# knights-lab/BURST

Measured on AMD Instinct MI355X. Metric: aligned reads/sec (node), 100-bp synthetic reads @0.98 id vs RefSeq stand-in .edx/.acx (DB15), -m BEST; 1 GPU, higher is better.
Workload: dtype u32 bit-vectors (u8 edit distances)

## Files before the change

burst_amd/csrc/bhip_align.hip:

```cpp
#include "bhip_handle.h"
#include "bhip_pf_select.h"

__global__ void k_hit_count(const BhipHit *__restrict__ hits, uint32_t n, const uint32_t *__restrict__ n_dev, uint32_t *__restrict__ cnt, uint32_t *__restrict__ rank) {
	if (n_dev) n = *n_dev < n ? *n_dev : n;
	for (uint32_t i = blockIdx.x * blockDim.x + threadIdx.x; i < n; i += gridDim.x * blockDim.x) rank[i] = atomicAdd(&cnt[hits[i].q], 1u);
}
__global__ void k_hit_scatter(const BhipHit *__restrict__ in, uint32_t n, const uint32_t *__restrict__ n_dev, const uint32_t *__restrict__ off, const uint32_t *__restrict__ rank,
                              BhipHit *__restrict__ out, const uint32_t *__restrict__ qmap) {
	if (n_dev) n = *n_dev < n ? *n_dev : n;
	for (uint32_t i = blockIdx.x * blockDim.x + threadIdx.x; i < n; i += gridDim.x * blockDim.x) {
		BhipHit h = in[i];
		const uint32_t dst = off[h.q] + rank[i];
		if (qmap) h.q = qmap[h.q];
		out[dst] = h;
	}
}
__global__ void k_junk_adjust_raw(BhipRawHit *__restrict__ raw, const uint32_t *__restrict__ n_raw_dev, uint32_t raw_cap, const uint8_t *__restrict__ nx) {
	uint32_t n = *n_raw_dev;
	if (n > raw_cap) n = raw_cap;
	for (uint32_t i = blockIdx.x * blockDim.x + threadIdx.x; i < n; i += gridDim.x * blockDim.x) { const uint32_t x = nx[raw[i].q]; raw[i].ed += x; raw[i].m += x; }
}
__global__ void k_junk_adjust_best(uint32_t *__restrict__ best, const uint8_t *__restrict__ nx_six, uint32_t s0, uint32_t s1) {
	for (uint32_t s = s0 + blockIdx.x * blockDim.x + threadIdx.x; s < s1; s += gridDim.x * blockDim.x)
		if (nx_six[s] && best[s] != 0xFFFFFFFFu) best[s] += nx_six[s];
}

__global__ __launch_bounds__(256) void k_hit_fix(BhipHit *__restrict__ out, const uint32_t *__restrict__ off, const uint32_t *__restrict__ cnt, uint32_t n_q,
                                               BhipHit *__restrict__ scratch, uint32_t scratch_cap) {
	const uint32_t lane = threadIdx.x & 63u;
	const uint32_t wave = (blockIdx.x * blockDim.x + threadIdx.x) >> 6, n_waves = (gridDim.x * blockDim.x) >> 6;
	struct Rec { uint32_t w[5]; };
	static_assert(sizeof(BhipHit) == 20, "BhipHit is five dwords");
	for (uint32_t q0 = wave * 64u; q0 < n_q; q0 += n_waves * 64u) {
		const uint32_t q = q0 + lane;
		const uint32_t n_mine = q < n_q ? cnt[q] : 0u, o_mine = q < n_q ? off[q] : 0u;
		unsigned long long todo = __ballot(n_mine >= 2u);
		while (todo) {
			const int b = __builtin_ctzll(todo);
			todo &= todo - 1ull;
			const uint32_t n = (uint32_t)__builtin_amdgcn_readlane((int)n_mine, b), o = (uint32_t)__builtin_amdgcn_readlane((int)o_mine, b);
			Rec *grp = (Rec *)(out + o);
			if (n <= 64u) {
				Rec r = {};
				if (lane < n) r = grp[lane];
				const uint32_t key = lane < n ? r.w[1] : 0xFFFFFFFFu;
				uint32_t rank = 0;
				for (uint32_t j = 0; j < n; ++j) { const uint32_t kj = (uint32_t)__builtin_amdgcn_readlane((int)key, (int)j); rank += (kj < key || (kj == key && j < lane)) ? 1u : 0u; }
				if (lane < n) grp[rank] = r;
			} else if ((uint64_t)o + n <= scratch_cap) {
				Rec *tmp = (Rec *)(scratch + o);
				for (uint32_t i = lane; i < n; i += 64u) tmp[i] = grp[i];
				__threadfence();
				for (uint32_t i0 = 0; i0 < n; i0 += 64u) {
					const uint32_t i = i0 + lane;
					Rec r = {};
					if (i < n) r = tmp[i];
					const uint32_t key = i < n ? r.w[1] : 0xFFFFFFFFu;
					uint32_t rank = 0;
					for (uint32_t j0 = 0; j0 < n; j0 += 64u) {
						const uint32_t kj = j0 + lane < n ? tmp[j0 + lane].w[1] : 0xFFFFFFFFu;
						const uint32_t m = n - j0 < 64u ? n - j0 : 64u;
						for (uint32_t j = 0; j < m; ++j) { const uint32_t kk = (uint32_t)__builtin_amdgcn_readlane((int)kj, (int)j); rank += (kk < key || (kk == key && j0 + j < i)) ? 1u : 0u; }
					}
					if (i < n) grp[rank] = r;
				}
			} else if (lane == 0) {
				BhipHit *a = out + o;
				uint32_t gap = 1;
				while (gap < n / 3) gap = 3 * gap + 1;
				for (; gap >= 1; gap /= 3)
					for (uint32_t i = gap; i < n; ++i) {
						const BhipHit v = a[i];
						uint32_t j = i;
						for (; j >= gap && a[j - gap].refIx > v.refIx; j -= gap) a[j] = a[j - gap];
						a[j] = v;
					}
			}
		}
	}
}
__global__ void k_set_rank_ptrs(SharedCtr *sc, uint32_t *cnt, uint32_t *rank) { sc->cnt = cnt; sc->rank = rank; }

__device__ __forceinline__ unsigned long long best_key_of(const BhipHit &h, const uint32_t *__restrict__ order) {
	return (unsigned long long)(~__float_as_uint(h.score)) << 32 | order[h.refIx];
}
__global__ void k_best_key(const BhipHit *__restrict__ hits, uint32_t n, const uint32_t *__restrict__ n_dev, const uint32_t *__restrict__ order, const uint32_t *__restrict__ cnt,
                           unsigned long long *__restrict__ key) {
	if (n_dev) n = *n_dev < n ? *n_dev : n;
	for (uint32_t i = blockIdx.x * blockDim.x + threadIdx.x; i < n; i += gridDim.x * blockDim.x) {
		const BhipHit h = hits[i];
		if (cnt[h.q] > 1u) atomicMin(&key[h.q], best_key_of(h, order));
	}
}
__global__ void k_best_flag(const uint32_t *__restrict__ cnt, uint32_t n_q, uint32_t *__restrict__ flag) {
	for (uint32_t i = blockIdx.x * blockDim.x + threadIdx.x; i <= n_q; i += gridDim.x * blockDim.x) flag[i] = i < n_q && cnt[i] ? 1u : 0u;
}
__global__ void k_best_emit(const BhipHit *__restrict__ hits, uint32_t n, const uint32_t *__restrict__ n_dev, const uint32_t *__restrict__ order, const uint32_t *__restrict__ cnt,
                            const unsigned long long *__restrict__ key, const uint32_t *__restrict__ off, BhipHit *__restrict__ out, const uint32_t *__restrict__ qmap) {
	if (n_dev) n = *n_dev < n ? *n_dev : n;
	for (uint32_t i = blockIdx.x * blockDim.x + threadIdx.x; i < n; i += gridDim.x * blockDim.x) {
		BhipHit h = hits[i];
		if (cnt[h.q] > 1u && best_key_of(h, order) != key[h.q]) continue;
		const uint32_t dst = off[h.q];
		if (qmap) h.q = qmap[h.q];
		out[dst] = h;
	}
}
extern "C" int bhip_set_ref_order(void *handle, const uint32_t *order, uint32_t n) {
	Handle *h = (Handle *)handle;
	if (!h) return fail(BHIP_E_ARG, "null handle");
	if (!order) return h->n_order ? 1 : 0;
	if (n < h->tot_refs) return fail(BHIP_E_ARG, "reference order table holds %u entries, the database has %u references", n, h->tot_refs);
	HIPCHK(hipSetDevice(h->device));
	int rc;
	h->n_order = 0;
	if ((rc = h->ref_order.reserve((size_t)h->tot_refs * 4 + 16))) return rc;
	HIPCHK(hipMemcpy(h->ref_order.p, order, (size_t)h->tot_refs * 4, hipMemcpyHostToDevice));
	h->n_order = h->tot_refs;
	return BHIP_OK;
}

static void launch_myers(Handle *h, Lane *L, hipStream_t st, int NW, uint32_t grid, const uint2 *pairs, const uint32_t *n_pairs_dev,
		uint64_t n_pairs_host, uint32_t li_base, const uint32_t *qlist, BhipRawHit *raw, uint32_t *n_raw, uint32_t raw_cap, uint32_t *best,
		uint8_t *mins, Counters *dc) {
	if (NW > 32) {
		hipLaunchKernelGGL(k_myers_long, dim3(grid * 4u), dim3(64), (size_t)NW * 512u, st, pairs, n_pairs_dev, n_pairs_host, h->n_clumps, li_base, qlist,
			L->peq.as<uint32_t>(), h->s_off(), h->s_emac(), (best && h->cur->st_has_six) ? h->cur->qsix.as<uint32_t>() : nullptr,
			h->ref_lane.as<uint4>(), h->ref_off.as<uint64_t>(), h->clump_len.as<uint32_t>(), h->tot_refs, raw, n_raw, raw_cap, best, mins, &dc->col_sum, &dc->qlen_sum, (uint32_t)NW);
		return;
	}
	#define LM(N) hipLaunchKernelGGL(k_myers<N>, dim3(grid), dim3(256), 0, st, pairs, n_pairs_dev, n_pairs_host, h->n_clumps, li_base, qlist, \
		L->peq.as<uint32_t>(), h->s_off(), h->s_emac(), (best && h->cur->st_has_six) ? h->cur->qsix.as<uint32_t>() : nullptr, \
		h->ref_lane.as<uint4>(), h->ref_off.as<uint64_t>(), h->clump_len.as<uint32_t>(), h->tot_refs, raw, n_raw, raw_cap, best, mins, &dc->col_sum, &dc->qlen_sum)
	switch (NW) { case 2: LM(2); break; case 4: LM(4); break; case 6: LM(6); break; case 8: LM(8); break; case 10: LM(10); break;
		case 16: LM(16); break; default: LM(32); break; }
	#undef LM
}
static void launch_prefix(Handle *h, Lane *L, hipStream_t st, int NWP, uint32_t grid, const uint2 *pairs, const uint32_t *n_pairs_dev,
		uint64_t n_pairs_host, uint32_t li_base, const uint32_t *qlist, uint32_t *n_wins, Counters *dc) {
	#define LP(N) hipLaunchKernelGGL(k_myers_prefix<N>, dim3(grid), dim3(256), 0, st, pairs, n_pairs_dev, n_pairs_host, h->n_clumps, li_base, qlist, \
		L->peqp.as<uint32_t>(), h->s_off(), h->s_emac(), h->ref_lane.as<uint4>(), h->ref_off.as<uint64_t>(), h->clump_len.as<uint32_t>(), \
		h->tot_refs, L->wins.as<BhipWin>(), n_wins, (uint32_t)L->win_cap, &dc->col_sum, &dc->qlen_sum, dc->win_class_seen, h->cur->st_has_six ? h->cur->qsix.as<uint32_t>() : nullptr)
	if (NWP == 1) LP(1); else if (NWP == 2) LP(2); else if (NWP == 3) LP(3); else if (NWP == 4) LP(4); else LP(6);
	#undef LP
}
static void launch_prefix_task(Handle *h, Lane *L, hipStream_t st, int NWP, uint32_t grid, const uint2 *tasks, const uint32_t *n_tasks_dev, const uint32_t *qlist,
		BhipWin *wins, uint32_t *n_wins, Counters *dc, const uint4 *qmeta) {
	#define LT(N) hipLaunchKernelGGL(k_myers_prefix_task<N>, dim3(grid), dim3(64), 0, st, tasks, n_tasks_dev, (uint32_t)L->task_cap, qlist, \
		L->peqp.as<uint32_t>(), h->s_off(), h->s_emac(), h->ref_lane.as<uint4>(), h->ref_off.as<uint64_t>(), h->clump_len.as<uint32_t>(), \
		wins, n_wins, (uint32_t)L->win_cap, &dc->tcol_sum, dc->win_class_seen, qmeta, h->cur->st_has_six ? h->cur->qsix.as<uint32_t>() : nullptr)
	if (NWP == 1) LT(1); else if (NWP == 2) LT(2); else if (NWP == 3) LT(3); else if (NWP == 4) LT(4); else LT(6);
	#undef LT
}
static uint32_t blocks_per_cu(const void *fn, uint32_t threads, size_t dyn_lds, hipFuncAttributes *fa_out = nullptr) {
	hipFuncAttributes fa_here, &fa = fa_out ? *fa_out : fa_here;
	memset(&fa, 0, sizeof fa);
	if (hipFuncGetAttributes(&fa, fn) != hipSuccess) return 4;
	const uint32_t waves_per_block = (threads + 63) / 64;
	const uint32_t by_reg = 4u * std::min(8u, 512u / (uint32_t)std::max(8, (fa.numRegs + 7) & ~7)) / waves_per_block;
	const size_t lds = fa.sharedSizeBytes + dyn_lds;
	const uint32_t by_lds = lds ? (uint32_t)((148u * 1024u) / std::max<size_t>(512, (lds + 511) & ~(size_t)511)) : 64u;
	return std::max(1u, std::min(by_reg, by_lds));
}

static void launch_window(Handle *h, Lane *L, hipStream_t wst, int cls, int NWP, uint32_t grid_cap, const BhipWin *wins, const uint32_t *n_wins, Counters *dc) {
	const uint32_t *six = h->cur->st_has_six ? h->cur->qsix.as<uint32_t>() : nullptr;
	const int NWc = kClasses[cls];
	const int min_class = h->opt_no_band ? 0 : NWc >= 8 ? 3 : NWc >= 6 ? 2 : NWc >= 4 ? 1 : 0;
	#define LB(BW) { uint32_t per_cu = blocks_per_cu((const void *)k_myers_window_band<BW>, 64u, 0); \
		if (h->opt_band_blocks > 0) per_cu = (uint32_t)h->opt_band_blocks; \
		const uint32_t grid = (uint32_t)h->n_cu * per_cu * (uint32_t)h->opt_oversub; \
		hipLaunchKernelGGL(k_myers_window_band<BW>, dim3(grid), dim3(64), 0, wst, wins, n_wins, (uint32_t)L->win_cap, NWP, NWc, L->peq.as<uint32_t>(), six, \
			h->ref_lane.as<uint4>(), L->raw.as<BhipRawHit>(), &dc->n_raw, (uint32_t)L->raw_cap, h->best.as<uint32_t>(), &dc->wcol_sum, dc->win_class_seen); }
	if (min_class >= 1) LB(2);
	if (min_class >= 2) LB(3);
	if (min_class >= 3) LB(4);
	#undef LB
	#define LW(N) { const uint32_t thr = (N) <= 8 ? 64u : 256u;       \
		const uint32_t grid = std::min<uint32_t>(grid_cap * (256u / thr), (uint32_t)h->n_cu * blocks_per_cu((const void *)k_myers_window<N>, thr, 0)); \
		hipLaunchKernelGGL(k_myers_window<N>, dim3(grid), dim3(thr), 0, wst, wins, n_wins, (uint32_t)L->win_cap, NWP, min_class, \
		L->peq.as<uint32_t>(), six, h->ref_lane.as<uint4>(), \
		L->raw.as<BhipRawHit>(), &dc->n_raw, (uint32_t)L->raw_cap, h->best.as<uint32_t>(), &dc->wcol_sum, dc->win_class_seen); }
	switch (NWc) { case 2: LW(2); break; case 4: LW(4); break; case 6: LW(6); break; case 8: LW(8); break; case 10: LW(10); break;
		case 16: LW(16); break; default: LW(32); break; }
	#undef LW
}


static int upload_queries(Handle *h, const uint8_t *q_codes, const uint64_t *q_off, const uint16_t *q_emac,
                          const uint32_t *q_six, const uint8_t *q_rc, uint32_t n_q) {
	const uint64_t nb = q_off[n_q];
	int rc;
	h->cur->st_has_junk = false;
	h->cur->st_maxlen = 0; h->cur->st_maxE = 0;
	for (uint32_t i = 0; i < n_q; ++i) {
		h->cur->st_maxlen = std::max<uint32_t>(h->cur->st_maxlen, (uint32_t)(q_off[i + 1] - q_off[i]));
		h->cur->st_maxE = std::max<uint32_t>(h->cur->st_maxE, q_emac[i]);
	}
	if ((rc = h->cur->qcodes.reserve(nb + 16))) return rc;
	if ((rc = h->cur->qoff.reserve((n_q + 1) * sizeof(uint64_t)))) return rc;
	if ((rc = h->cur->qemac.reserve((n_q + 1) * sizeof(uint16_t)))) return rc;
	if ((rc = h->cur->qsix.reserve((n_q + 1) * sizeof(uint32_t)))) return rc;
	if ((rc = h->cur->qrc.reserve(n_q + 1))) return rc;
	HIPCHK(hipMemcpyAsync(h->cur->qcodes.p, q_codes, nb, hipMemcpyHostToDevice, h->stream));
	HIPCHK(hipMemcpyAsync(h->cur->qoff.p, q_off, (n_q + 1) * sizeof(uint64_t), hipMemcpyHostToDevice, h->stream));
	HIPCHK(hipMemcpyAsync(h->cur->qemac.p, q_emac, n_q * sizeof(uint16_t), hipMemcpyHostToDevice, h->stream));
	if (q_six) HIPCHK(hipMemcpyAsync(h->cur->qsix.p, q_six, n_q * sizeof(uint32_t), hipMemcpyHostToDevice, h->stream));
	if (q_rc) HIPCHK(hipMemcpyAsync(h->cur->qrc.p, q_rc, n_q, hipMemcpyHostToDevice, h->stream));
	return 0;
}

static int upload_plan(Handle *h, const uint8_t *q_codes, const uint64_t *q_off, const uint16_t *q_emac, uint32_t n_q, std::vector<uint32_t> &plan) {
	int rc;
	if ((rc = h->cur->plan.reserve((size_t)n_q * 4 + 16))) return rc;
	(void)q_codes; (void)q_off; (void)q_emac;
	HIPCHK(hipMemcpyAsync(h->cur->plan.p, plan.data(), (size_t)n_q * 4, hipMemcpyHostToDevice, h->stream));
	HIPCHK(hipStreamSynchronize(h->stream));
	return 0;
}

struct PfOverflow {
	uint32_t *fb1 = nullptr, *n_fb1 = nullptr;
	uint32_t *fb2 = nullptr, *n_fb2 = nullptr;
	int begin(Lane *L, Counters *dc, hipStream_t st, uint32_t n_list, bool lane_resolved) {
		int rc;
		if ((rc = L->fb_list.reserve(lane_resolved ? (size_t)n_list * 8 + 64 : (size_t)n_list * 4 + 16))) return rc;
		fb1 = L->fb_list.as<uint32_t>(); n_fb1 = &dc->n_fb;
		if (lane_resolved) {
			fb2 = fb1 + n_list + 8; n_fb2 = &dc->n_fb2;
			if (L->pf_launches || L->fb_dirty) HIPCHK(hipMemsetAsync(&dc->n_fb, 0, 8, st));
			L->fb_dirty = false;
		} else {
			HIPCHK(hipMemsetAsync(&dc->n_fb, 0, 4, st));
			L->fb_dirty = true;
		}
		return 0;
	}
};

static int launch_dense_fallback(Handle *h, Lane *L, hipStream_t st, const uint32_t *d_qlist, uint32_t n_list, const uint32_t *bad, uint32_t n_bad,
                                 uint2 *cand, uint32_t *candcnt, uint32_t *n_cand_dev, uint32_t cand_cap, Counters *dc, const uint32_t *fb, const uint32_t *n_fb) {
	const uint32_t *plan = h->cur->plan.as<uint32_t>();
	const bool narrow = h->cur->st_maxlen < 255u + (uint32_t)h->K;
	const size_t lds_w = ((size_t)(h->n_clumps + (narrow ? 3 : 1)) / (narrow ? 4 : 2)) * 4 + 1536u * 4 + 512u * 8 + 512u * 4 + 16;
	const uint32_t nw32 = (h->n_clumps + 1) / 2;
	if (lds_w <= 64 * 1024) {
		const uint32_t per_cu = (uint32_t)std::max<size_t>(1, std::min<size_t>(16, (160 * 1024) / lds_w));
		const uint32_t grid = std::min<uint32_t>(n_list, (uint32_t)h->n_cu * per_cu);
		if (narrow) hipLaunchKernelGGL(k_prefilter_wave<uint8_t>, dim3(grid), dim3(64), lds_w, st, h->s_codes(), h->s_off(),
			h->s_emac(), d_qlist, n_list, h->acx_view(), h->K, h->n_clumps, bad, n_bad, cand, candcnt,
			n_cand_dev, cand_cap, &dc->ent_read, plan, fb, n_fb);
		else hipLaunchKernelGGL(k_prefilter_wave<uint16_t>, dim3(grid), dim3(64), lds_w, st, h->s_codes(), h->s_off(),
			h->s_emac(), d_qlist, n_list, h->acx_view(), h->K, h->n_clumps, bad, n_bad, cand, candcnt,
			n_cand_dev, cand_cap, &dc->ent_read, plan, fb, n_fb);
	} else {
		int rc;
		const uint32_t grid = std::min<uint32_t>(n_list, (uint32_t)h->n_cu * 2);
		if ((rc = L->gcnt.reserve((size_t)grid * nw32 * 4))) return rc;
		hipLaunchKernelGGL(k_prefilter<false>, dim3(grid), dim3(256), 0, st, h->s_codes(), h->s_off(),
			h->s_emac(), d_qlist, n_list, h->acx_view(), h->K, h->n_clumps,
			L->gcnt.as<uint32_t>(), bad, n_bad, cand, candcnt, n_cand_dev, cand_cap, &dc->ent_read, fb, n_fb, plan);
	}
	HIPCHK(hipGetLastError());
	return 0;
}

static int launch_prefilter(Handle *h, Lane *L, hipStream_t st, const uint32_t *d_qlist, uint32_t n_list, uint2 *cand, uint32_t *candcnt, uint32_t cand_cap,
                            bool with_bad, uint32_t *n_cand_dev, Counters *dc) {
	const uint32_t *bad = with_bad ? h->bad.as<uint32_t>() : nullptr;
	const uint32_t n_bad = with_bad ? h->n_bad : 0;
	int rc;
	PfOverflow ov;
	if ((rc = ov.begin(L, dc, st, n_list, false))) return rc;
	{
		const uint32_t n_quads = (n_list + 3) / 4;
		const uint32_t grid = std::min<uint32_t>(n_quads, (uint32_t)h->n_cu * 6);
		hipLaunchKernelGGL(k_prefilter_hash, dim3(grid), dim3(64), 0, st, h->s_codes(), h->s_off(), h->s_emac(),
			d_qlist, n_list, h->acx_view(), h->K, bad, n_bad, cand, candcnt, n_cand_dev, cand_cap, &dc->ent_read,
			h->cur->plan.as<uint32_t>(), ov.fb1, ov.n_fb1);
		HIPCHK(hipGetLastError());
	}
	return launch_dense_fallback(h, L, st, d_qlist, n_list, bad, n_bad, cand, candcnt, n_cand_dev, cand_cap, dc, ov.fb1, ov.n_fb1);
}

static uint32_t seed_row_words(uint32_t maxwords) { return maxwords <= 8 ? 8u : std::max<uint32_t>(16u, (maxwords + 15u) & ~15u); }
static int class_prefix_words(const Handle *h, uint32_t maxE, int NW) {
	if (!h->opt_two_stage || NW > 32) return 0;
	const uint32_t want = (6 * maxE + 31) / 32;
	int NWP = want <= 1 ? 1 : (want <= 2 ? 2 : (want <= 3 ? 3 : (want <= 4 ? 4 : (want <= 6 ? 6 : 0))));
	if (NWP >= NW) NWP = 0;
	return NWP;
}
static int launch_peq(Handle *h, hipStream_t st, StageSlot *S, const uint32_t *d_qlist, uint32_t n_list, int NW, int NWP, DBuf &peq, DBuf &peqp, uint32_t blocks_per_cu = 16) {
	int rc;
	if ((rc = peq.reserve((size_t)n_list * 16 * NW * 4))) return rc;
	if ((rc = peqp.reserve((size_t)n_list * 16 * 6 * 4))) return rc;
	const bool junk = S->st_has_junk;
	const uint8_t *codes = junk ? S->qcodes_s.as<uint8_t>() : S->qcodes.as<uint8_t>();
	const uint64_t *off = junk ? S->qoff_s.as<uint64_t>() : S->qoff.as<uint64_t>();
	const uint32_t *pack = junk ? S->qpack_s.as<uint32_t>() : S->qpack.as<uint32_t>();
	{
		const uint32_t qb = 256u / (uint32_t)NW;
		const uint32_t grid = (uint32_t)std::min<uint64_t>(((uint64_t)n_list + qb - 1) / qb, (uint64_t)h->n_cu * blocks_per_cu);
		hipLaunchKernelGGL(k_build_peq, dim3(grid), dim3(256), 0, st, codes, off, d_qlist, n_list, NW, 0, h->mm, peq.as<uint32_t>(), pack, (S->st_maxlen + 7) / 8, h->peq_rows);
		HIPCHK(hipGetLastError());
	}
	if (NWP) {
		const uint32_t qb = 256u / (uint32_t)NWP;
		const uint32_t grid = (uint32_t)std::min<uint64_t>(((uint64_t)n_list + qb - 1) / qb, (uint64_t)h->n_cu * blocks_per_cu);
		hipLaunchKernelGGL(k_build_peq, dim3(grid), dim3(256), 0, st, codes, off, d_qlist, n_list, NWP, 32 * NWP, h->mm, peqp.as<uint32_t>(), pack, (S->st_maxlen + 7) / 8, h->peq_rows);
		HIPCHK(hipGetLastError());
	}
	return 0;
}
static uint32_t seed_min_need_for(const Handle *h, double mean_words, uint32_t W16) {
	return bhip_seed_min_need(h->opt_seed_min_need, h->opt_pf_cw, h->opt_pf_table, h->opt_pf_bytes, h->acx_wmean, mean_words, W16);
}
static int launch_seed(Handle *h, Lane *L, hipStream_t st, StageSlot *S, int cls, const uint32_t *d_qlist, uint32_t n_list, uint32_t maxwords, double mean_words, bool ahead = false) {
	int rc;
	const uint32_t W16 = seed_row_words(maxwords);
	L->seeded_ok[cls] = false;
	if ((rc = L->ranges_c[cls].reserve((size_t)n_list * W16 * 8 + 16))) return rc;
	if ((rc = L->hdr_c[cls].reserve((size_t)n_list * 8 + 16))) return rc;
	DBuf &qm = L->qmeta_c[S->seq & 1][cls];
	if ((rc = qm.reserve((size_t)n_list * 16 + 16))) return rc;
	L->qmeta_seq[S->seq & 1][cls] = 0;
	const uint64_t n_thr = (uint64_t)n_list * W16;
	hipEvent_t *ev = L->ev_seed[S->seq & 1][cls];
	const bool junk = S->st_has_junk;
	HIPCHK(hipEventRecord(ev[0], st));
	const uint64_t full = (n_thr + 255) / 256;
	const uint32_t grid = (uint32_t)(ahead && h->opt_seed_ahead_blocks > 0 ? std::min<uint64_t>(full, (uint64_t)h->n_cu * (uint64_t)h->opt_seed_ahead_blocks) : full);
	hipLaunchKernelGGL(k_seed_ranges, dim3(grid), dim3(256), 0, st,
		junk ? S->qcodes_s.as<uint8_t>() : S->qcodes.as<uint8_t>(), junk ? S->qoff_s.as<uint64_t>() : S->qoff.as<uint64_t>(), d_qlist, n_list,
		h->acx_view(), h->K, S->plan.as<uint32_t>(), W16, L->ranges_c[cls].as<uint2>(), L->hdr_c[cls].as<uint2>(),
		junk ? S->qpack_s.as<uint32_t>() : S->qpack.as<uint32_t>(), (S->st_maxlen + 7) / 8, junk ? S->qemac_s.as<uint16_t>() : S->qemac.as<uint16_t>(), qm.as<uint4>(), S->st_has_six ? S->qsix.as<uint32_t>() : nullptr,
		seed_min_need_for(h, mean_words, W16), (uint32_t)h->opt_seed_drop_len, h->alt);
	HIPCHK(hipGetLastError());
	HIPCHK(hipEventRecord(ev[1], st));
	L->qmeta_seq[S->seq & 1][cls] = S->seq + 1;
	L->seeded_ok[cls] = true; L->seeded_seq[cls] = S->seq; L->seeded_n[cls] = n_list; L->seeded_W16[cls] = W16;
	return 0;
}

static bhip_pf_kernel_t pf_kernel(const BhipPfChoice &c, int big) {
	if (c.legacy) return bhip_legacy_pf_kernel ? bhip_legacy_pf_kernel(c.kind, big ? 11 : c.htb, big ? 4 : c.rb, c.cw_mode, big) : nullptr;
	if (c.kind == BHIP_PF_CQ) return c.cw_mode == 0 ? (big ? k_prefilter_cq<0, 1> : k_prefilter_cq<0, 0>) : (big ? k_prefilter_cq<1, 1> : k_prefilter_cq<1, 0>);
	return big ? k_prefilter_cw<2, 1> : k_prefilter_cw<2, 0>;
}

static int launch_prefilter_mask(Handle *h, Lane *L, hipStream_t st, int cls, const uint32_t *d_qlist, uint32_t n_list, uint32_t maxwords, uint32_t *n_tasks_dev,
                                 uint32_t *n_cand_dev, Counters *dc, int algo, int prune) {
	int rc;
	PfOverflow ov;
	if ((rc = ov.begin(L, dc, st, n_list, true))) return rc;
	const uint32_t W16 = seed_row_words(maxwords);
	const double mean_words = n_list ? (double)L->seed_words[cls] / (double)n_list : (double)maxwords;
	if (!(L->seeded_ok[cls] && L->seeded_seq[cls] == h->cur->seq && L->seeded_n[cls] == n_list && L->seeded_W16[cls] == W16))
		if ((rc = launch_seed(h, L, st, h->cur, cls, d_qlist, n_list, maxwords, mean_words))) return rc;
	const BhipPfChoice c = bhip_pf_choose(algo, h->opt_pf_cw, h->opt_pf_table, h->opt_pf_rb, W16, mean_words * h->acx_wmean);
	const bool filter = c.kind != BHIP_PF_MASK, cw = c.kind == BHIP_PF_CW || c.kind == BHIP_PF_CQ;
	const bhip_pf_kernel_t fp = filter ? pf_kernel(c, 0) : nullptr, fp2 = filter && c.two_pass ? pf_kernel(c, 1) : nullptr;
	if (filter && (!fp || (c.two_pass && !fp2)))
		return fail(BHIP_E_ARG, "option prefilter_cw = %d selects a superseded prefilter kernel that is not part of libburst_hip.so (tests: libburst_hip_legacy.so is loaded first)", h->opt_pf_cw);
	hipFuncAttributes fa;
	const void *fn = filter ? (const void *)fp : c.htb == 9 ? (const void *)k_prefilter_mask<9> : c.htb == 10 ? (const void *)k_prefilter_mask<10> : (const void *)k_prefilter_mask<11>;
	const uint32_t fit = std::min<uint32_t>(cw ? 32u : 12u, blocks_per_cu(fn, 64u, 0, &fa));
	if (getenv("BHIP_DEBUG")) {
		if (cw) fprintf(stderr, "[bhip] prefilter kernel: %s, slot mode %d, %zu B LDS, %d VGPRs -> %u blocks per CU\n", c.kind == BHIP_PF_CQ ? "four queries per wave, streams by the whole wave" : "one query per wave", c.cw_mode, fa.sharedSizeBytes, fa.numRegs, fit);
		else fprintf(stderr, "[bhip] prefilter kernel: table 2^%d, %d record blocks in registers, %zu B LDS, %d VGPRs -> %u blocks per CU\n", c.htb, c.rb, fa.sharedSizeBytes, fa.numRegs, fit);
	}
	const uint32_t waves = h->opt_pf_waves ? std::min<uint32_t>((uint32_t)h->opt_pf_waves, fit) : fit;
	const uint32_t grid = std::min<uint32_t>(c.kind == BHIP_PF_CW ? n_list : (n_list + 3) / 4, (uint32_t)h->n_cu * waves);
	HIPCHK(hipEventRecord(L->ev_pf[cls][1], st));
	const uint32_t *fb_dense = ov.fb1, *n_fb_dense = ov.n_fb1;
	if (filter) {
		auto launch = [&](bhip_pf_kernel_t k, uint32_t g, uint32_t *fb, uint32_t *n_fb, const uint32_t *sel, const uint32_t *n_sel) {
			hipLaunchKernelGGL(k, dim3(g), dim3(64), 0, st, L->ranges_c[cls].as<uint2>(), L->hdr_c[cls].as<uint2>(), W16, n_list,
				h->acx_view().rec, h->bad.as<uint32_t>(), h->n_bad,
				h->clump_len.as<uint32_t>(), h->tot_refs, L->tasks.as<uint2>(), n_tasks_dev, (uint32_t)L->task_cap, &dc->ent_read,
				fb, n_fb, &dc->unit_sum, &dc->col_sum, &dc->qlen_sum, &dc->surv_sum,
				L->tasks2.as<uint2>(), &dc->n_tasks2_cls[cls], prune, sel, n_sel, c.kind == BHIP_PF_CF ? h->opt_pf_bytes : 0);
		};
		launch(fp, grid, ov.fb1, ov.n_fb1, nullptr, nullptr);
		if (c.two_pass) {
			HIPCHK(hipGetLastError());
			const uint32_t g2 = (uint32_t)h->n_cu * (c.kind == BHIP_PF_CQ ? std::min<uint32_t>(4u, blocks_per_cu((const void *)fp2, 64u, 0)) : 1u);
			launch(fp2, g2, ov.fb2, ov.n_fb2, ov.fb1, ov.n_fb1);
			fb_dense = ov.fb2; n_fb_dense = ov.n_fb2;
		}
	} else {
#define PFM_LAUNCH(B) hipLaunchKernelGGL(k_prefilter_mask<B>, dim3(grid), dim3(64), 0, st, L->ranges_c[cls].as<uint2>(), L->hdr_c[cls].as<uint2>(), W16, n_list, \
		h->acx_view().rec, h->bad.as<uint32_t>(), h->n_bad, \
		h->clump_len.as<uint32_t>(), h->tot_refs, L->tasks.as<uint2>(), n_tasks_dev, (uint32_t)L->task_cap, &dc->ent_read, \
		ov.fb1, ov.n_fb1, &dc->unit_sum, &dc->col_sum, &dc->qlen_sum, L->cand.as<uint2>(), n_cand_dev, (uint32_t)L->cand_cap)
		if (c.htb == 9) PFM_LAUNCH(9); else if (c.htb == 10) PFM_LAUNCH(10); else PFM_LAUNCH(11);
#undef PFM_LAUNCH
	}
	HIPCHK(hipGetLastError());
	HIPCHK(hipEventRecord(L->ev_pf[cls][2], st));
	++L->pf_launches;
	L->pf_algo_used = c.kind;
	return launch_dense_fallback(h, L, st, d_qlist, n_list, h->bad.as<uint32_t>(), h->n_bad, L->cand.as<uint2>(), nullptr, n_cand_dev, (uint32_t)L->cand_cap, dc, fb_dense, n_fb_dense);
}

static int lane_reserve_work(Lane *L) {
	int rc;
	if ((rc = L->cand.reserve(L->cand_cap * sizeof(uint2))) || (rc = L->raw.reserve(L->raw_cap * sizeof(BhipRawHit))) || (rc = L->wide.reserve(L->raw_cap * sizeof(uint32_t))) ||
	    (rc = L->rs_lists.reserve(L->raw_cap * sizeof(uint32_t) * 10)) || (rc = L->scratch.reserve(L->scratch_cap * sizeof(uint32_t))) || (rc = L->wins.reserve(L->win_cap * sizeof(BhipWin))) ||
	    (rc = L->tasks.reserve(L->task_cap * sizeof(uint2))) || (rc = L->tasks2.reserve(L->task_cap * sizeof(uint2))) || (rc = L->tasks2k.reserve(L->task_cap * sizeof(uint2))) ||
	    (rc = L->wins2.reserve(L->win_cap * sizeof(BhipWin)))) return rc;
	return 0;
}
extern "C" int bhip_reserve(void *handle, uint32_t n_entries, uint32_t max_len) { return bhip_reserve_symbols(handle, n_entries, max_len, 0); }
extern "C" int bhip_reserve_symbols(void *handle, uint32_t n_entries, uint32_t max_len, uint64_t total_symbols) {
	Handle *h = (Handle *)handle;
	if (!h) return fail(BHIP_E_ARG, "null handle");
	if (!n_entries) return BHIP_OK;
	if (!max_len || max_len > BHIP_MAX_QLEN) max_len = BHIP_MAX_QLEN;
	HIPCHK(hipSetDevice(h->device));
	int rc;
	if (getenv("BHIP_DEBUG")) { size_t f_ = 0, t_ = 0; if (hipMemGetInfo(&f_, &t_) == hipSuccess) fprintf(stderr, "[bhip] reserve for %u entries of up to %u symbols: %.2f GB of the device's %.2f free\n", n_entries, max_len, f_ / 1e9, t_ / 1e9); }
	const size_t n = n_entries, nb = total_symbols ? (size_t)std::min<uint64_t>(total_symbols + 64, (uint64_t)n * max_len) : n * max_len, qw = (max_len + 7) / 8;
	const size_t cw = (size_t)class_words(class_of_len(max_len), max_len);
	const size_t peq_words = total_symbols ? std::min<size_t>(n * cw, 2 * (nb / 32 + n)) : n * cw;
	for (StageSlot &S : h->slots) {
		if ((rc = slot_init(&S))) return rc;
		if ((rc = S.qcodes4.reserve(nb / 2 + 128)) || (rc = S.qcodes.reserve(nb + 128)) || (rc = S.qoff.reserve((n + 1) * 8)) || (rc = S.qemac.reserve((n + 1) * 2)) ||
		    (rc = S.qsix.reserve((n + 1) * 4)) || (rc = S.qrc.reserve(n + 1)) || (rc = S.qflags.reserve(n + 1)) || (rc = S.qmap.reserve((n + 1) * 4)) ||
		    (rc = S.off_raw.reserve((n + 8) * 8)) || (rc = S.plan.reserve(n * 4 + 16)) || (rc = S.qpack.reserve(n * qw * 4 + 64)) || (rc = S.key.reserve(n + 16)) ||
		    (rc = S.key_sorted.reserve(n + 16)) || (rc = S.idx.reserve(n * 4 + 16)) || (rc = S.idx_sorted.reserve(n * 4 + 16))) return rc;
		size_t tb = 0;
		HIPCHK(hipcub::DeviceRadixSort::SortPairs(nullptr, tb, S.key.as<uint8_t>(), S.key_sorted.as<uint8_t>(), S.idx.as<uint32_t>(), S.idx_sorted.as<uint32_t>(), (int)n, 0, 8, h->stage_stream));
		if ((rc = S.sort_tmp.reserve(tb + 16))) return rc;
	}
	if (getenv("BHIP_DEBUG")) { size_t f_ = 0, t_ = 0; if (hipMemGetInfo(&f_, &t_) == hipSuccess) fprintf(stderr, "[bhip] ... staging slots reserved: %.2f GB free\n", f_ / 1e9); }
	if ((rc = ensure_lanes(h, 1))) return rc;
	Lane *L = h->lanes[0];
	lane_capacity_floor(h, L, n);
	const int cls = class_of_len(max_len);
	if ((rc = lane_reserve_work(L)) || (rc = L->peq.reserve(peq_words * 16 * 4)) || (rc = L->peqp.reserve(n * 16 * 6 * 4)) ||
	    (rc = L->peq_alt.reserve(peq_words * 16 * 4)) || (rc = L->peqp_alt.reserve(n * 16 * 6 * 4)) ||
	    (rc = L->fb_list.reserve(n * 8 + 64)) || (rc = L->ranges_c[cls].reserve(n * 16 * 8 + 16)) || (rc = L->hdr_c[cls].reserve(n * 8 + 16))) return rc;
	if (h->n_order) { if ((rc = h->best_key.reserve((n + 1) * 8)) || (rc = h->sort_idx.reserve(std::max<size_t>((size_t)h->out_cap, n + 1) * 4))) return rc; if (!h->nsel_pinned) HIPCHK(hipHostMalloc((void **)&h->nsel_pinned, 64, hipHostMallocDefault)); }
	if ((rc = h->best.reserve((n + 1) * 4)) || (rc = h->out.reserve(h->out_cap * sizeof(BhipHit))) || (rc = h->shared_ctr.reserve(sizeof(SharedCtr))) ||
	    (rc = h->sort_idx.reserve(h->out_cap * 4)) || (rc = h->sort_keys.reserve((n + 1) * 4)) || (rc = h->sort_keys2.reserve((n + 1) * 4)) ||
	    (rc = h->out_sorted.reserve(h->out_cap * sizeof(BhipHit))) || (rc = h->out_sorted2.reserve(h->out_cap * sizeof(BhipHit)))) return rc;
	{
		size_t tb = 0;
		HIPCHK(hipcub::DeviceScan::ExclusiveSum(nullptr, tb, h->sort_keys.as<uint32_t>(), h->sort_keys2.as<uint32_t>(), (int)(n + 1), h->stream));
		if ((rc = h->sort_tmp.reserve(tb))) return rc;
	}
	if (getenv("BHIP_DEBUG")) { size_t f_ = 0, t_ = 0; if (hipMemGetInfo(&f_, &t_) == hipSuccess) fprintf(stderr, "[bhip] ... lane and record buffers reserved: %.2f GB free\n", f_ / 1e9); }
	if (!h->copy_stream) { HIPCHK(hipStreamCreateWithFlags(&h->copy_stream, hipStreamNonBlocking)); HIPCHK(hipEventCreateWithFlags(&h->ev_sorted, hipEventDisableTiming));
		for (auto &e : h->ev_copied) HIPCHK(hipEventCreateWithFlags(&e, hipEventDisableTiming)); }
	{
		const uint32_t nw = std::min<uint32_t>(n_entries, 1u << 17), len = std::min<uint32_t>(max_len, 100u);
		const size_t nb_w = (size_t)nw * len + 16;
		uint8_t *pin = nullptr;
		const size_t bytes = nb_w + nb_w / 2 + 16 + ((size_t)nw + 1) * 8 + (size_t)nw * 2 + 64 + (size_t)nw * 4 * sizeof(BhipHit);
		HIPCHK(hipHostMalloc((void **)&pin, bytes, hipHostMallocPortable));
		uint8_t *codes = pin, *codes4 = pin + nb_w;
		uint64_t *off = (uint64_t *)(pin + ((nb_w + nb_w / 2 + 16 + 7) & ~(size_t)7));
		uint16_t *emac = (uint16_t *)(off + nw + 1);
		BhipHit *hbuf = (BhipHit *)(((uintptr_t)(emac + nw) + 63) & ~(uintptr_t)63);
		uint64_t x = 88172645463325252ull;
		for (size_t i = 0; i < nb_w; ++i) { x ^= x << 13; x ^= x >> 7; x ^= x << 17; codes[i] = (uint8_t)(1 + (x & 3)); }
		for (size_t i = 0; i < nb_w / 2; ++i) codes4[i] = (uint8_t)(codes[2 * i] | codes[2 * i + 1] << 4);
		for (uint32_t i = 0; i <= nw; ++i) off[i] = (uint64_t)i * len;
		for (uint32_t i = 0; i < nw; ++i) emac[i] = (uint16_t)(len / 40);
		BhipQuerySpan sp;
		memset(&sp, 0, sizeof sp);
		sp.codes = codes; sp.codes4 = codes4; sp.off = off; sp.emac = emac; sp.n = nw;
		uint64_t n_out = 0;
		const int async = h->opt_async_d2h;
		h->opt_async_d2h = 1;
		for (StageSlot &S : h->slots) { S.state = 0; S.st_valid = false; }
		rc = 0;
		for (int rep = 0; rep < 4 && !rc; ++rep) {
			rc = bhip_stage_spans(h, &sp, 1, nw, len);
			if (!rc) rc = bhip_align_staged(h, 0, hbuf, (uint64_t)nw * 4, &n_out);
		}
		(void)bhip_sync_hits(h);
		{
			const size_t big = std::min<size_t>(64u << 20, std::min(h->out_sorted.cap, h->out_sorted2.cap));
			void *tmp = nullptr;
			if (big && hipHostMalloc(&tmp, 2 * big, hipHostMallocPortable) == hipSuccess) {
				(void)hipMemcpyAsync(tmp, h->out_sorted.p, big, hipMemcpyDeviceToHost, h->copy_stream);
				(void)hipMemcpyAsync((char *)tmp + big, h->out_sorted2.p, big, hipMemcpyDeviceToHost, h->copy_stream);
				(void)hipMemcpyAsync(tmp, h->out_sorted.p, big, hipMemcpyDeviceToHost, h->copy_stream);
				(void)hipStreamSynchronize(h->copy_stream);
				(void)hipMemcpyAsync(h->out_sorted.p, tmp, big, hipMemcpyHostToDevice, h->stage_stream);
				(void)hipMemcpyAsync(h->out_sorted2.p, (char *)tmp + big, big, hipMemcpyHostToDevice, h->stage_stream);
				(void)hipMemcpyAsync(h->out_sorted.p, tmp, big, hipMemcpyHostToDevice, h->stage_stream);
				(void)hipStreamSynchronize(h->stage_stream);
				const size_t piece = big / 16;
				if (piece) {
					for (int i = 0; i < 12; ++i) (void)hipMemcpyAsync((char *)h->out_sorted.p + (size_t)i * piece, (char *)tmp + (size_t)i * piece, piece, hipMemcpyHostToDevice, h->stage_stream);
					(void)hipMemcpyAsync((char *)tmp + big, h->out_sorted2.p, big, hipMemcpyDeviceToHost, h->copy_stream);
					(void)hipStreamSynchronize(h->copy_stream);
					(void)hipStreamSynchronize(h->stage_stream);
				}
				(void)hipHostFree(tmp);
			}
			(void)hipGetLastError();
		}
		h->opt_async_d2h = async;
		for (StageSlot &S : h->slots) { S.state = 0; S.st_valid = false; S.spans.clear(); }
		h->res_valid = false;
		(void)hipHostFree(pin);
		if (rc) return rc;
	}
	return BHIP_OK;
}
static int enqueue_lane(Handle *h, Lane *L, int all_hits, hipEvent_t start, uint32_t band_rows, uint32_t qw, uint32_t rw) {
	int rc;
	if ((rc = lane_reserve_work(L))) return rc;
	hipStream_t pf = h->pf_stream, sw = h->sweep_stream, po = h->post_stream;
	HIPCHK(hipMemsetAsync(L->counters.p, 0, sizeof(Counters), pf));
	Counters *dc = L->counters.as<Counters>();
	SharedCtr *sc = h->shared_ctr.as<SharedCtr>();
	L->launches = 0; L->prefix_words = 0; L->n_pairs_ex = 0; L->pf_launches = 0; L->fb_dirty = false;
	for (int c = 0; c < kNumClasses; ++c) { L->pf_masked[c] = false; L->pruned[c] = false; }
	const uint32_t grid_my = (uint32_t)h->n_cu * (uint32_t)h->opt_sweep_blocks;
	(void)start;
	for (int cls = 0; cls < kNumClasses; ++cls) {
		const uint32_t n_pf = L->npf[cls], n_ex = L->nex[cls], n_list = n_pf + n_ex;
		if (!n_list) continue;
		const int NW = class_words(cls, L->maxlen);
		const uint32_t *qlist = L->qlist[cls];
		hipEvent_t *ce = L->ev_cls[cls];
		if (L->launches) { HIPCHK(hipStreamWaitEvent(pf, L->ev_rs[0], 0)); HIPCHK(hipStreamWaitEvent(sw, L->ev_rs[0], 0)); }
		const int NWP = class_prefix_words(h, L->maxE[cls], NW);
		HIPCHK(hipEventRecord(ce[0], sw));
		L->peq_ahead[cls] = false;
		if (L->alt_ok && L->alt_seq == h->cur->seq && L->alt_cls == cls && L->alt_n == n_list && L->alt_nwp == NWP && !L->launches) {
			std::swap(L->peq, L->peq_alt); std::swap(L->peqp, L->peqp_alt);
			std::swap(L->ev_peq_cur[0], L->ev_peq_alt[0]); std::swap(L->ev_peq_cur[1], L->ev_peq_alt[1]);
			L->alt_ok = false; L->peq_ahead[cls] = true;
		} else if ((rc = launch_peq(h, sw, h->cur, qlist, n_list, NW, NWP, L->peq, L->peqp))) return rc;
		L->prefix_words = (uint32_t)NWP;
		HIPCHK(hipEventRecord(ce[1], sw));
		HIPCHK(hipEventRecord(ce[7], pf));
		const bool masked = NWP && n_pf && h->has_masks && h->opt_lane_masks;
		const int pf_algo = bhip_pf_algo(h->opt_pf_algo, L->pf_algo);
		const int prune = masked && !all_hits && h->opt_prune && n_list < (1u << 24) && pf_algo == 0;
		if (n_pf) {
			if (masked) { if ((rc = launch_prefilter_mask(h, L, pf, cls, qlist, n_pf, L->maxwords[cls], &dc->n_tasks_cls[cls], &dc->n_cand_cls[cls], dc, pf_algo, prune))) return rc; }
			else if ((rc = launch_prefilter(h, L, pf, qlist, n_pf, L->cand.as<uint2>(), nullptr, (uint32_t)L->cand_cap, true, &dc->n_cand_cls[cls], dc))) return rc;
		}
		const uint4 *qmeta_cls = (masked && L->qmeta_seq[h->cur->seq & 1][cls] == h->cur->seq + 1) ? L->qmeta_c[h->cur->seq & 1][cls].as<uint4>() : nullptr;
		L->masked = masked;
		L->pf_masked[cls] = masked && n_pf;
		HIPCHK(hipEventRecord(ce[2], pf));
		HIPCHK(hipStreamWaitEvent(sw, ce[2], 0));
		HIPCHK(hipEventRecord(ce[6], sw));
		if (n_pf) {
			if (masked) launch_prefix_task(h, L, sw, NWP, (uint32_t)h->n_cu * 4u * (uint32_t)h->opt_sweep_blocks * (uint32_t)h->opt_oversub, L->tasks.as<uint2>(), &dc->n_tasks_cls[cls], qlist, L->wins.as<BhipWin>(), &dc->n_wins_cls[cls], dc, qmeta_cls);
			if (NWP) launch_prefix(h, L, sw, NWP, masked ? std::min<uint32_t>(grid_my, (uint32_t)h->n_cu) : grid_my, L->cand.as<uint2>(), &dc->n_cand_cls[cls], L->cand_cap, 0, qlist, &dc->n_wins_cls[cls], dc);
			else launch_myers(h, L, sw, NW, grid_my, L->cand.as<uint2>(), &dc->n_cand_cls[cls], L->cand_cap, 0, qlist, L->raw.as<BhipRawHit>(),
				&dc->n_raw, (uint32_t)L->raw_cap, h->best.as<uint32_t>(), nullptr, dc);
			HIPCHK(hipGetLastError());
			++L->launches;
		}
		HIPCHK(hipEventRecord(ce[3], sw));
		if (n_ex) {
			const uint64_t np = (uint64_t)n_ex * h->n_clumps;
			const uint32_t g = (uint32_t)std::min<uint64_t>((np + 15) / 16, grid_my);
			if (NWP) launch_prefix(h, L, sw, NWP, g, nullptr, nullptr, np, n_pf, qlist, &dc->n_wins_cls[cls], dc);
			else launch_myers(h, L, sw, NW, g, nullptr, nullptr, np, n_pf, qlist, L->raw.as<BhipRawHit>(), &dc->n_raw, (uint32_t)L->raw_cap,
				h->best.as<uint32_t>(), nullptr, dc);
			HIPCHK(hipGetLastError());
			++L->launches;
			L->n_pairs_ex += np;
		}
		HIPCHK(hipEventRecord(ce[4], sw));
		HIPCHK(hipStreamWaitEvent(po, ce[4], 0));
		if (NWP) { launch_window(h, L, po, cls, NWP, grid_my, L->wins.as<BhipWin>(), &dc->n_wins_cls[cls], dc); HIPCHK(hipGetLastError()); }
		L->pruned[cls] = masked && prune && n_pf;
		if (masked && prune && n_pf) {
			HIPCHK(hipEventRecord(L->ev_ph[cls][0], po));
			HIPCHK(hipStreamWaitEvent(sw, L->ev_ph[cls][0], 0));
			hipLaunchKernelGGL(k_task_filter, dim3((uint32_t)h->n_cu * 8), dim3(256), 0, sw, L->tasks2.as<uint2>(), &dc->n_tasks2_cls[cls], (uint32_t)L->task_cap, qlist,
				h->cur->st_has_six ? h->cur->qsix.as<uint32_t>() : nullptr, h->best.as<uint32_t>(), L->tasks2k.as<uint2>(), &dc->n_tasks2k_cls[cls]);
			launch_prefix_task(h, L, sw, NWP, (uint32_t)h->n_cu * 4u * (uint32_t)h->opt_sweep_blocks * (uint32_t)h->opt_oversub, L->tasks2k.as<uint2>(), &dc->n_tasks2k_cls[cls], qlist, L->wins2.as<BhipWin>(), &dc->n_wins2_cls[cls], dc, qmeta_cls);
			HIPCHK(hipGetLastError());
			HIPCHK(hipEventRecord(L->ev_ph[cls][1], sw));
			HIPCHK(hipStreamWaitEvent(po, L->ev_ph[cls][1], 0));
			launch_window(h, L, po, cls, NWP, grid_my, L->wins2.as<BhipWin>(), &dc->n_wins2_cls[cls], dc);
			HIPCHK(hipGetLastError());
		}
		HIPCHK(hipEventRecord(ce[5], po));
		HIPCHK(hipEventRecord(L->ev_rs[0], po));
	}
	HIPCHK(hipEventRecord(L->ev_rs[0], po));
	if (h->cur->st_has_junk) {
		const uint32_t nl_ = h->cur->st_lanes, nsh_ = h->cur->st_nshared;
		uint32_t li_ = 0;
		for (uint32_t l = 0; l < nl_; ++l) if (h->lanes[l] == L) li_ = l;
		const uint32_t s0 = (uint32_t)(((uint64_t)li_ * nsh_ + nl_ - 1) / nl_), s1 = (uint32_t)(((uint64_t)(li_ + 1) * nsh_ + nl_ - 1) / nl_);
		hipLaunchKernelGGL(k_junk_adjust_raw, dim3((uint32_t)h->n_cu * 4), dim3(256), 0, po, L->raw.as<BhipRawHit>(), &dc->n_raw, (uint32_t)L->raw_cap, h->cur->nx.as<uint8_t>());
		if (s1 > s0) hipLaunchKernelGGL(k_junk_adjust_best, dim3(std::min<uint32_t>((s1 - s0 + 255) / 256, (uint32_t)h->n_cu * 4)), dim3(256), 0, po, h->best.as<uint32_t>(), h->cur->nx_six.as<uint8_t>(), s0, s1);
		HIPCHK(hipGetLastError());
	}
	const uint32_t qw_g = (h->cur->st_maxlen + 7) / 8;
	hipLaunchKernelGGL(k_rescore_classify, dim3((uint32_t)h->n_cu * 8), dim3(256), 0, po, L->raw.as<BhipRawHit>(), &dc->n_raw, (uint32_t)L->raw_cap,
		h->best.as<uint32_t>(), all_hits, h->cur->qoff.as<uint64_t>(), h->cur->st_has_six ? h->cur->qsix.as<uint32_t>() : nullptr, h->cur->st_has_rc ? h->cur->qrc.as<uint8_t>() : nullptr,
		h->clump_len.as<uint32_t>(), h->out.as<BhipHit>(), &sc->n_out, (uint32_t)h->out_cap, L->rs_lists.as<uint32_t>(), dc->n_rs, L->wide.as<uint32_t>(), &dc->n_wide,
		band_rows, h->opt_rescore_reg);
	HIPCHK(hipGetLastError());
	if (h->opt_rescore_reg) {
#define RS_LAUNCH(SET, BLOCKS) hipLaunchKernelGGL(k_rescore_reg<SET>, dim3((uint32_t)h->n_cu * std::min<uint32_t>(32u, blocks_per_cu((const void *)k_rescore_reg<SET>, 64, 0)) * (uint32_t)h->opt_oversub), dim3(64), 0, po, L->raw.as<BhipRawHit>(), L->rs_lists.as<uint32_t>(), dc->n_rs, (uint32_t)L->raw_cap, \
			h->cur->qoff.as<uint64_t>(), h->cur->st_has_rc ? h->cur->qrc.as<uint8_t>() : nullptr, h->cur->qpack.as<uint32_t>(), qw_g, \
			h->ref_lane.as<uint8_t>(), h->ref_off.as<uint64_t>(), h->clump_len.as<uint32_t>(), h->lut.as<uint8_t>(), h->out.as<BhipHit>(), &sc->n_out, (uint32_t)h->out_cap, &sc->err)
		RS_LAUNCH(0, 16);
		HIPCHK(hipGetLastError());
		RS_LAUNCH(3, 16);
		HIPCHK(hipGetLastError());
		RS_LAUNCH(1, 12);
		HIPCHK(hipGetLastError());
		RS_LAUNCH(2, 8);
		HIPCHK(hipGetLastError());
#undef RS_LAUNCH
	}
	const uint32_t grid_rs = (uint32_t)h->n_cu * (h->opt_rescore_reg ? 4 : 16);
	const size_t lds_rs = (size_t)(band_rows + 1 + qw + rw) * 256;
	hipLaunchKernelGGL(k_rescore<false>, dim3(grid_rs), dim3(64), lds_rs, po, L->raw.as<BhipRawHit>(), &dc->n_raw, (uint32_t)L->raw_cap,
		L->rs_lists.as<uint32_t>() + (size_t)9 * L->raw_cap, &dc->n_rs[9], h->best.as<uint32_t>(), all_hits, h->cur->qcodes.as<uint8_t>(), h->cur->qoff.as<uint64_t>(),
		h->cur->st_has_six ? h->cur->qsix.as<uint32_t>() : nullptr, h->cur->st_has_rc ? h->cur->qrc.as<uint8_t>() : nullptr, h->ref_lane.as<uint8_t>(), h->ref_off.as<uint64_t>(),
		h->clump_len.as<uint32_t>(), h->lut.as<uint8_t>(), h->out.as<BhipHit>(), &sc->n_out, (uint32_t)h->out_cap, L->wide.as<uint32_t>(),
		&dc->n_wide, (uint32_t *)nullptr, &dc->scratch_used, 0ull, &sc->err, qw ? h->cur->qpack.as<uint32_t>() : nullptr, band_rows, qw, rw);
	HIPCHK(hipGetLastError());
	HIPCHK(hipEventRecord(L->ev_rs[1], po));
	HIPCHK(hipMemcpyAsync(L->hc_pinned, dc, sizeof(Counters), hipMemcpyDeviceToHost, po));
	return 0;
}

static void seed_next_batch(Handle *h, StageSlot *cur, hipEvent_t cur_done) {
	if (!h->opt_seed_ahead || !h->has_acx || !h->has_masks || !h->opt_lane_masks || h->opt_host_routing) return;
	StageSlot *N = nullptr;
	for (StageSlot &S : h->slots) if (&S != cur && S.state == 1 && (!N || S.seq < N->seq)) N = &S;
	if (!N || !N->st_nq) return;
	if (!N->resolved) {
		for (;;) {
			const hipError_t e = hipEventQuery(N->ev_done);
			if (e == hipSuccess) break;
			if (e != hipErrorNotReady) { (void)hipGetLastError(); return; }
			if (hipEventQuery(cur_done) != hipErrorNotReady) { (void)hipGetLastError(); return; }
			std::this_thread::yield();
		}
		(void)hipGetLastError();
		const BhipStageInfo &I = *N->info_pinned;
		if (I.err || I.junk) return;
		if (resolve_slot(h, N)) return;
	}
	if (N->st_has_junk || ensure_lanes(h, N->st_lanes)) return;
	for (uint32_t l = 0; l < N->st_lanes && l < h->lanes.size(); ++l) {
		Lane *L = h->lanes[l];
		for (int cls = 0; cls < kNumClasses; ++cls) {
			const uint32_t n_pf = N->npf[l][cls];
			if (!n_pf || !class_prefix_words(h, N->maxE[l][cls], class_words(cls, N->maxlen_lane[l]))) continue;
			if (L->seeded_ok[cls] && L->seeded_seq[cls] == N->seq) continue;
			if (launch_seed(h, L, h->pf_stream, N, cls, N->idx_sorted.as<uint32_t>() + N->qlist_off[l][cls], n_pf, N->maxwords[l][cls], (double)N->seed_words[l][cls] / (double)n_pf, true)) { (void)hipGetLastError(); return; }
		}
		int only = -1, n_cls = 0;
		for (int cls = 0; cls < kNumClasses; ++cls) if (N->npf[l][cls] + N->nex[l][cls]) { only = cls; ++n_cls; }
		if (n_cls == 1 && !(L->alt_ok && L->alt_seq == N->seq)) {
			const uint32_t n_list = N->npf[l][only] + N->nex[l][only];
			const int NW = class_words(only, N->maxlen_lane[l]), NWP = class_prefix_words(h, N->maxE[l][only], NW);
			L->alt_ok = false;
			if (hipEventRecord(L->ev_peq_alt[0], h->pf_stream) != hipSuccess ||
			    launch_peq(h, h->pf_stream, N, N->idx_sorted.as<uint32_t>() + N->qlist_off[l][only], n_list, NW, NWP, L->peq_alt, L->peqp_alt, (uint32_t)h->opt_peq_ahead_blocks) ||
			    hipEventRecord(L->ev_peq_alt[1], h->pf_stream) != hipSuccess) { (void)hipGetLastError(); return; }
			L->alt_ok = true; L->alt_seq = N->seq; L->alt_cls = only; L->alt_nwp = NWP; L->alt_n = n_list;
		}
	}
}

extern "C" int bhip_set_enqueued_hook(void *handle, void (*fn)(void *), void *ctx) {
	Handle *h = (Handle *)handle;
	if (!h) return fail(BHIP_E_ARG, "null handle");
	h->enqueued_hook = fn; h->enqueued_ctx = ctx;
	return BHIP_OK;
}

extern "C" int bhip_align_staged(void *handle, int all_hits_arg, BhipHit *hits, uint64_t cap, uint64_t *n_hits) {
	Handle *h = (Handle *)handle;
	if (!h || !n_hits) return fail(BHIP_E_ARG, "null argument");
	*n_hits = 0;
	if (all_hits_arg < 0 || all_hits_arg > BHIP_HITS_BEST) return fail(BHIP_E_ARG, "all_hits must be 0, 1 or 2 (BHIP_HITS_BEST)");
	const int all_hits = all_hits_arg == BHIP_HITS_ALL ? 1 : 0;
	const bool sel_best = all_hits_arg == BHIP_HITS_BEST;
	if (sel_best && !h->n_order) return fail(BHIP_E_ARG, "BHIP_HITS_BEST needs the reference order table (bhip_set_ref_order)");
	memset(&h->stats, 0, sizeof h->stats);
	HIPCHK(hipSetDevice(h->device));
	StageSlot *slot = nullptr;
	for (StageSlot &S : h->slots) if (S.state == 1 && (!slot || S.seq < slot->seq)) slot = &S;
	if (!slot) for (StageSlot &S : h->slots) if (S.state == 2 && (!slot || S.seq > slot->seq)) slot = &S;
	if (!slot) return fail(BHIP_E_ARG, "no staged queries (call bhip_stage_queries first)");
	{ int rcs = resolve_slot(h, slot); if (rcs) { slot->state = 0; return rcs; } }
	apply_slot(h, slot);
	const uint32_t n_q = h->cur->st_nq, n_shared = h->cur->st_nshared, nl = h->cur->st_lanes;
	if (!n_q) { slot->state = 2; return BHIP_OK; }
	const uint32_t band_rows = std::min<uint32_t>(BHIP_RESCORE_WMAX, 2 * h->cur->st_maxE + 1 + 9);
	uint32_t qw = (h->cur->st_maxlen + 7) / 8, rw = (h->cur->st_maxlen + band_rows + 24) / 8 + 2;
	if ((size_t)(band_rows + 1 + qw + rw) * 256 > 40 * 1024) { qw = 0; rw = 0; }
	SharedCtr hsc;
	uint32_t n_deliver = 0;
	bool sorted_ahead = false; int o_ahead = 0;
	if (sel_best) { int rcs; if ((rcs = h->best_key.reserve((size_t)(n_q + 1) * 8)) || (rcs = h->sort_idx.reserve(std::max<size_t>((size_t)h->out_cap, (size_t)n_q + 1) * 4))) return rcs;
		if (!h->nsel_pinned) HIPCHK(hipHostMalloc((void **)&h->nsel_pinned, 64, hipHostMallocDefault)); }
	auto enqueue_grouping = [&](hipStream_t st, uint32_t n_host, const uint32_t *n_dev, DBuf &sorted, uint32_t *cnt, uint32_t *off, uint32_t *rank, size_t tmp_bytes) -> int {
		const uint32_t g = (uint32_t)h->n_cu * 8;
		const uint32_t *qmap = h->cur->has_qmap ? h->cur->qmap.as<uint32_t>() : (const uint32_t *)nullptr;
		if (sel_best) {
			hipLaunchKernelGGL(k_best_key, dim3(g), dim3(256), 0, st, h->out.as<BhipHit>(), n_host, n_dev, h->ref_order.as<uint32_t>(), cnt, h->best_key.as<unsigned long long>());
			hipLaunchKernelGGL(k_best_flag, dim3(std::min<uint32_t>((n_q + 256) / 256, g)), dim3(256), 0, st, cnt, n_q, rank);
			HIPCHK(hipcub::DeviceScan::ExclusiveSum(h->sort_tmp.p, tmp_bytes, rank, off, (int)(n_q + 1), st));
			hipLaunchKernelGGL(k_best_emit, dim3(g), dim3(256), 0, st, h->out.as<BhipHit>(), n_host, n_dev, h->ref_order.as<uint32_t>(), cnt, h->best_key.as<unsigned long long>(), off, sorted.as<BhipHit>(), qmap);
			HIPCHK(hipGetLastError());
			HIPCHK(hipMemcpyAsync(h->nsel_pinned, off + n_q, 4, hipMemcpyDeviceToHost, st));
			return 0;
		}
		HIPCHK(hipcub::DeviceScan::ExclusiveSum(h->sort_tmp.p, tmp_bytes, cnt, off, (int)(n_q + 1), st));
		hipLaunchKernelGGL(k_hit_scatter, dim3(g), dim3(256), 0, st, h->out.as<BhipHit>(), n_host, n_dev, off, rank, sorted.as<BhipHit>(), qmap);
		hipLaunchKernelGGL(k_hit_fix, dim3(std::min<uint32_t>((n_q + 255) / 256, (uint32_t)h->n_cu * 8)), dim3(256), 0, st, sorted.as<BhipHit>(), off, cnt, n_q, h->sort_scratch.as<BhipHit>(), (uint32_t)(h->sort_scratch.cap / sizeof(BhipHit)));
		HIPCHK(hipGetLastError());
		return 0;
	};
	for (int attempt = 0; attempt < 24; ++attempt) {
		int rc;
		sorted_ahead = false;
		if (h->res_valid && h->res_seq == slot->seq && h->res_all_hits == all_hits_arg) { hsc.n_out = h->res_n_raw; hsc.err = 0; h->stats = h->res_stats; n_deliver = h->res_n; *n_hits = n_deliver; }
		else {
		h->res_valid = false;
		if ((rc = h->best.reserve((size_t)(n_shared + 1) * 4))) return rc;
		if ((rc = h->out.reserve(h->out_cap * sizeof(BhipHit)))) return rc;
		if ((rc = h->shared_ctr.reserve(sizeof(SharedCtr)))) return rc;
		HIPCHK(hipEventRecord(h->ev[0], h->stream));
		HIPCHK(hipMemsetAsync(h->best.p, 0xFF, (size_t)n_shared * 4, h->stream));
		HIPCHK(hipMemsetAsync(h->shared_ctr.p, 0, 2 * sizeof(uint32_t), h->stream));
		{
			if ((rc = h->sort_idx.reserve((size_t)h->out_cap * 4)) || (rc = h->sort_keys.reserve((size_t)(n_q + 1) * 4))) return rc;
			HIPCHK(hipMemsetAsync(h->sort_keys.p, 0, (size_t)(n_q + 1) * 4, h->stream));
			if (sel_best) HIPCHK(hipMemsetAsync(h->best_key.p, 0xFF, (size_t)(n_q + 1) * 8, h->stream));
			hipLaunchKernelGGL(k_set_rank_ptrs, dim3(1), dim3(1), 0, h->stream, h->shared_ctr.as<SharedCtr>(), h->sort_keys.as<uint32_t>(), h->sort_idx.as<uint32_t>());
		}
		HIPCHK(hipEventRecord(h->ev[1], h->stream));
		HIPCHK(hipStreamWaitEvent(h->sweep_stream, h->ev[1], 0));
		HIPCHK(hipStreamWaitEvent(h->post_stream, h->ev[1], 0));
		for (uint32_t l = 0; l < nl; ++l) if (h->lanes[l]->n_entries) if ((rc = enqueue_lane(h, h->lanes[l], all_hits, h->ev[1], band_rows, qw, rw))) return rc;
		HIPCHK(hipEventRecord(h->ev[2], h->pf_stream));
		sorted_ahead = false;
		{
			const bool async = h->opt_async_d2h && hits;
			o_ahead = async ? (h->out_idx ^ 1) : 0;
			DBuf &sorted = o_ahead ? h->out_sorted2 : h->out_sorted;
			size_t tmp_bytes = 0;
			uint32_t *cnt = nullptr, *off = nullptr, *rank = nullptr;
			if ((rc = h->sort_idx.reserve((size_t)h->out_cap * 4)) || (rc = h->sort_keys.reserve((size_t)(n_q + 1) * 4)) || (rc = h->sort_keys2.reserve((size_t)(n_q + 1) * 4)) ||
			    (rc = sorted.reserve((size_t)h->out_cap * sizeof(BhipHit))) || (rc = h->sort_scratch.reserve((size_t)h->out_cap * sizeof(BhipHit)))) return rc;
			cnt = h->sort_keys.as<uint32_t>(); off = h->sort_keys2.as<uint32_t>(); rank = h->sort_idx.as<uint32_t>();
			HIPCHK(hipcub::DeviceScan::ExclusiveSum(nullptr, tmp_bytes, cnt, off, (int)(n_q + 1), h->post_stream));
			if ((rc = h->sort_tmp.reserve(tmp_bytes))) return rc;
			SharedCtr *sc = h->shared_ctr.as<SharedCtr>();
			if (h->copy_pending[o_ahead]) HIPCHK(hipStreamWaitEvent(h->post_stream, h->ev_copied[o_ahead], 0));
			HIPCHK(hipEventRecord(h->ev[4], h->post_stream));
			if ((rc = enqueue_grouping(h->post_stream, (uint32_t)h->out_cap, &sc->n_out, sorted, cnt, off, rank, tmp_bytes))) return rc;
			HIPCHK(hipEventRecord(h->ev[5], h->post_stream));
			sorted_ahead = true;
		}
		if (!h->hsc_pinned) HIPCHK(hipHostMalloc((void **)&h->hsc_pinned, sizeof(SharedCtr), hipHostMallocDefault));
		HIPCHK(hipMemcpyAsync(h->hsc_pinned, h->shared_ctr.p, 2 * sizeof(uint32_t), hipMemcpyDeviceToHost, h->post_stream));
		HIPCHK(hipEventRecord(h->ev[3], h->post_stream));
		seed_next_batch(h, slot, h->ev[3]);
		if (h->enqueued_hook && attempt == 0) h->enqueued_hook(h->enqueued_ctx);
		HIPCHK(hipEventSynchronize(h->ev[2]));
		HIPCHK(hipStreamSynchronize(h->sweep_stream));
		HIPCHK(hipStreamSynchronize(h->post_stream));
		for (uint32_t l = 0; l < nl; ++l) if (h->lanes[l]->n_entries) h->lanes[l]->hc = *h->lanes[l]->hc_pinned;
		for (uint32_t l = 0; l < nl; ++l) {
			Lane *L = h->lanes[l];
			const bool cq_min_only = !all_hits && h->opt_pf_cw == 2 && L->pf_algo_used == 3;
			if (L->n_entries && L->pf_algo == 0 && !cq_min_only && L->hc.ent_read > 100000 && (double)L->hc.surv_sum > (all_hits ? 0.20 : 0.50) * (double)L->hc.ent_read) L->pf_algo = 1;
		}
		if (getenv("BHIP_DEBUG")) for (uint32_t l = 0; l < nl; ++l) {
			const Lane *L = h->lanes[l];
			if (!L->n_entries) continue;
			fprintf(stderr, "[bhip] lane %u: %llu list records, %llu survived the counting filter, next prefilter algorithm %d\n", l, (unsigned long long)L->hc.ent_read, (unsigned long long)L->hc.surv_sum, L->pf_algo);
			for (int cls = 0; cls < kNumClasses; ++cls) if (L->npf[cls] + L->nex[cls])
				fprintf(stderr, "[bhip] lane %u class NW=%d: prefiltered %u exhaustive %u maxE %u maxwords %u | tasks %u + deferred %u (kept %u) clump pairs %u windows %u + %u | fallback queries(last class) %u raw %u\n",
					l, kClasses[cls], L->npf[cls], L->nex[cls], L->maxE[cls], L->maxwords[cls], L->hc.n_tasks_cls[cls], L->hc.n_tasks2_cls[cls], L->hc.n_tasks2k_cls[cls], L->hc.n_cand_cls[cls], L->hc.n_wins_cls[cls], L->hc.n_wins2_cls[cls], L->hc.n_fb, L->hc.n_raw);
			if (L->hc.n_fb) fprintf(stderr, "[bhip] lane %u: %u queries overflowed the first prefilter pass, %u the second (dense fallback)\n", l, L->hc.n_fb, L->hc.n_fb2);
		}
		bool retry = false;
		for (uint32_t l = 0; l < nl; ++l) {
			Lane *L = h->lanes[l];
			if (!L->n_entries) continue;
			const Counters &c = L->hc;
			for (int cls = 0; cls < kNumClasses; ++cls) {
				if (c.n_cand_cls[cls] > L->cand_cap) { L->cand_cap = (uint64_t)c.n_cand_cls[cls] + c.n_cand_cls[cls] / 8 + 1024; retry = true; }
				if (c.n_tasks_cls[cls] > L->task_cap) { L->task_cap = (uint64_t)c.n_tasks_cls[cls] + c.n_tasks_cls[cls] / 8 + 1024; retry = true; }
				if (c.n_tasks2_cls[cls] > L->task_cap) { L->task_cap = (uint64_t)c.n_tasks2_cls[cls] + c.n_tasks2_cls[cls] / 8 + 1024; retry = true; }
				if (c.n_wins2_cls[cls] > L->win_cap) { L->win_cap = (uint64_t)c.n_wins2_cls[cls] + c.n_wins2_cls[cls] / 8 + 1024; retry = true; }
				if (c.n_wins_cls[cls] > L->win_cap) { L->win_cap = (uint64_t)c.n_wins_cls[cls] + c.n_wins_cls[cls] / 8 + 1024; retry = true; }
			}
			if (c.n_raw > L->raw_cap) { L->raw_cap = (uint64_t)c.n_raw + c.n_raw / 8 + 1024; retry = true; }
		}
		if (retry) continue;
		bool scratch_retry = false;
		for (uint32_t l = 0; l < nl; ++l) {
			Lane *L = h->lanes[l];
			if (!L->n_entries || !L->hc.n_wide) continue;
			sorted_ahead = false;
			Counters *dc = L->counters.as<Counters>();
			SharedCtr *sc = h->shared_ctr.as<SharedCtr>();
			hipLaunchKernelGGL(k_rescore<true>, dim3(std::min<uint32_t>((L->hc.n_wide + 63) / 64, (uint32_t)h->n_cu * 16)), dim3(64), 256, h->post_stream,
				L->raw.as<BhipRawHit>(), &dc->n_raw, (uint32_t)L->raw_cap, L->wide.as<uint32_t>(), &dc->n_wide, h->best.as<uint32_t>(), all_hits,
				h->cur->qcodes.as<uint8_t>(), h->cur->qoff.as<uint64_t>(), h->cur->st_has_six ? h->cur->qsix.as<uint32_t>() : nullptr, h->cur->st_has_rc ? h->cur->qrc.as<uint8_t>() : nullptr,
				h->ref_lane.as<uint8_t>(), h->ref_off.as<uint64_t>(), h->clump_len.as<uint32_t>(), h->lut.as<uint8_t>(), h->out.as<BhipHit>(),
				&sc->n_out, (uint32_t)h->out_cap, (uint32_t *)nullptr, (uint32_t *)nullptr, L->scratch.as<uint32_t>(), &dc->scratch_used,
				(unsigned long long)L->scratch_cap, &sc->err, (const uint32_t *)nullptr, 0u, 0u, 0u);
			HIPCHK(hipGetLastError());
			HIPCHK(hipMemcpyAsync(&L->hc, dc, sizeof(Counters), hipMemcpyDeviceToHost, h->post_stream));
			HIPCHK(hipStreamSynchronize(h->post_stream));
			if (L->hc.scratch_used > L->scratch_cap) { L->scratch_cap = (uint64_t)L->hc.scratch_used + 1024; scratch_retry = true; }
		}
		if (sorted_ahead) hsc = *h->hsc_pinned;
		else HIPCHK(hipMemcpy(&hsc, h->shared_ctr.p, 2 * sizeof(uint32_t), hipMemcpyDeviceToHost));
		if (scratch_retry || (hsc.err & 2u)) continue;
		if (hsc.err & 1u) return fail(BHIP_E_RESCORE, "re-scoring could not reproduce a hit found by the edit-distance kernel (a query starting with a symbol outside the alphabet? the reference stops here as well: CRITICAL ERROR: Truncation within known good path, burst.c:812-816)");
		if (hsc.n_out > h->out_cap) { h->out_cap = (uint64_t)hsc.n_out + hsc.n_out / 8 + 1024; continue; }
		n_deliver = sel_best ? (sorted_ahead ? *h->nsel_pinned : std::min<uint32_t>(hsc.n_out, n_q)) : hsc.n_out;
		*n_hits = n_deliver;
		h->last_n_out = 0;
		BhipStats &S = h->stats;
		S.n_queries = n_q; S.n_hits = n_deliver;
		uint64_t qlen_sum = 0;
		for (uint32_t l = 0; l < nl; ++l) {
			Lane *L = h->lanes[l];
			if (!L->n_entries) continue;
			const Counters &c = L->hc;
			S.n_pairs += L->n_pairs_ex + c.unit_sum; S.n_columns += c.col_sum; S.n_task_columns += c.tcol_sum; S.n_raw_hits += c.n_raw; S.acx_entries_read += c.ent_read;
			S.myers_launches += L->launches; S.prefilter_launches += L->pf_launches; if (L->pf_launches) S.prefilter_algo = (uint32_t)L->pf_algo_used; S.n_window_columns += c.wcol_sum; qlen_sum += c.qlen_sum;
			if (L->prefix_words) S.prefix_words = L->prefix_words;
			for (int cls = 0; cls < kNumClasses; ++cls) {
				S.n_pairs += c.n_cand_cls[cls]; S.n_windows += c.n_wins_cls[cls] + c.n_wins2_cls[cls]; S.n_lane_tasks += c.n_tasks_cls[cls] + c.n_tasks2k_cls[cls];
				if (!(L->npf[cls] + L->nex[cls])) continue;
				hipEvent_t *ce = L->ev_cls[cls];
				S.ms_peq += L->peq_ahead[cls] ? ev_ms(L->ev_peq_cur[0], L->ev_peq_cur[1]) : ev_ms(ce[0], ce[1]);
				if (L->npf[cls]) S.ms_prefilter += ev_ms(ce[7], ce[2]);
				if (L->npf[cls] && L->pf_masked[cls]) { { hipEvent_t *es = L->ev_seed[h->cur->seq & 1][cls]; S.ms_seed += ev_ms(es[0], es[1]); } S.ms_prefilter_hash += ev_ms(L->ev_pf[cls][1], L->ev_pf[cls][2]); S.n_seed_words += L->seed_words[cls]; }
				float sweep = ev_ms(ce[6], ce[4]), win = ev_ms(ce[4], ce[5]);
				if (L->pruned[cls]) { const float second = ev_ms(L->ev_ph[cls][0], L->ev_ph[cls][1]); sweep += second; win -= second; }
				S.ms_myers += sweep + win;
				if (L->prefix_words) { S.ms_myers_prefix += sweep; S.ms_myers_window += win; }
			}
			S.ms_rescore += ev_ms(L->ev_rs[0], L->ev_rs[1]);
		}
		S.bytes_algorithmic = 8ull * S.n_columns + qlen_sum / 2 + 192ull * S.n_pairs;
		h->res_valid = true; h->res_seq = slot->seq; h->res_all_hits = all_hits_arg; h->res_n = n_deliver; h->res_n_raw = hsc.n_out; h->res_stats = h->stats;
		}
		BhipStats &S = h->stats;
		if (hits && n_deliver > cap) return fail(BHIP_E_CAPACITY, "hit buffer holds %llu records, %u needed", (unsigned long long)cap, n_deliver);
		HIPCHK(hipEventRecord(h->ev[8], h->stream));
		const bool dbg_t = getenv("BHIP_DEBUG_TIMES") != nullptr;
		const auto tq0 = std::chrono::steady_clock::now();
		auto tq = [&]() { return std::chrono::duration<double, std::milli>(std::chrono::steady_clock::now() - tq0).count(); };
		double tq1 = 0, tq2 = 0, tq3 = 0, tq4 = 0;
		if (hsc.n_out) {
			const uint32_t n = hsc.n_out;
			if ((rc = h->sort_idx.reserve(std::max<size_t>((size_t)n, sel_best ? (size_t)n_q + 1 : 0) * 4)) || (rc = h->sort_keys.reserve((size_t)(n_q + 1) * 4)) || (rc = h->sort_keys2.reserve((size_t)(n_q + 1) * 4)) ||
			    0) return rc;
			const bool async = h->opt_async_d2h && hits;
			const int o = async ? (h->out_idx ^= 1) : 0;
			DBuf &sorted = o ? h->out_sorted2 : h->out_sorted;
			if (sorted_ahead && o == o_ahead) tq1 = tq();
			else {
			if (h->copy_pending[o]) { HIPCHK(hipEventSynchronize(h->ev_copied[o])); h->copy_pending[o] = false; }
			if ((rc = sorted.reserve((size_t)n * sizeof(BhipHit))) || (rc = h->sort_scratch.reserve((size_t)n * sizeof(BhipHit)))) return rc;
			uint32_t *cnt = h->sort_keys.as<uint32_t>(), *off = h->sort_keys2.as<uint32_t>(), *rank = h->sort_idx.as<uint32_t>();
			const uint32_t g = std::min<uint32_t>((n + 255) / 256, (uint32_t)h->n_cu * 8);
			HIPCHK(hipMemsetAsync(cnt, 0, (size_t)(n_q + 1) * 4, h->stream));
			if (sel_best) HIPCHK(hipMemsetAsync(h->best_key.p, 0xFF, (size_t)(n_q + 1) * 8, h->stream));
			tq1 = tq();
			hipLaunchKernelGGL(k_hit_count, dim3(g), dim3(256), 0, h->stream, h->out.as<BhipHit>(), n, (const uint32_t *)nullptr, cnt, rank);
			size_t tmp_bytes = 0;
			HIPCHK(hipcub::DeviceScan::ExclusiveSum(nullptr, tmp_bytes, cnt, off, (int)(n_q + 1), h->stream));
			if ((rc = h->sort_tmp.reserve(tmp_bytes))) return rc;
			if ((rc = enqueue_grouping(h->stream, n, (const uint32_t *)nullptr, sorted, cnt, off, rank, tmp_bytes))) return rc;
			if (sel_best) {
				HIPCHK(hipStreamSynchronize(h->stream));
				n_deliver = *h->nsel_pinned; *n_hits = n_deliver; S.n_hits = n_deliver; h->res_n = n_deliver;
				if (hits && n_deliver > cap) return fail(BHIP_E_CAPACITY, "hit buffer holds %llu records, %u needed", (unsigned long long)cap, n_deliver);
			}
			}
			tq2 = tq();
			const size_t bytes = (size_t)n_deliver * sizeof(BhipHit);
			bool queued = false;
			if (async) {
				if (!h->copy_stream) { HIPCHK(hipStreamCreateWithFlags(&h->copy_stream, hipStreamNonBlocking)); HIPCHK(hipEventCreateWithFlags(&h->ev_sorted, hipEventDisableTiming));
					for (auto &e : h->ev_copied) HIPCHK(hipEventCreateWithFlags(&e, hipEventDisableTiming)); }
				const size_t want = (size_t)cap * sizeof(BhipHit);
				bool reg_ok = h->reg_ptr[o] == (void *)hits && h->reg_bytes[o] >= bytes;
				if (!reg_ok) {
					hipPointerAttribute_t at;
					memset(&at, 0, sizeof at);
					if (hipPointerGetAttributes(&at, (const void *)hits) == hipSuccess && at.type == hipMemoryTypeHost) reg_ok = true;
					else (void)hipGetLastError();
				}
				if (!reg_ok) {
					if (h->reg_ptr[o]) { (void)hipHostUnregister(h->reg_ptr[o]); h->reg_ptr[o] = nullptr; }
					if (h->reg_ptr[o ^ 1] == (void *)hits) { if (h->copy_pending[o ^ 1]) { HIPCHK(hipEventSynchronize(h->ev_copied[o ^ 1])); h->copy_pending[o ^ 1] = false; }
						(void)hipHostUnregister(h->reg_ptr[o ^ 1]); h->reg_ptr[o ^ 1] = nullptr; }
					if (hipHostRegister((void *)hits, want, hipHostRegisterDefault) == hipSuccess) { h->reg_ptr[o] = (void *)hits; h->reg_bytes[o] = want; reg_ok = true; }
					else (void)hipGetLastError();
				}
				tq3 = tq();
				if (reg_ok) {
					HIPCHK(hipEventRecord(h->ev_sorted, h->stream));
					HIPCHK(hipStreamWaitEvent(h->copy_stream, h->ev_sorted, 0));
					HIPCHK(hipMemcpyAsync(hits, sorted.p, bytes, hipMemcpyDeviceToHost, h->copy_stream));
					HIPCHK(hipEventRecord(h->ev_copied[o], h->copy_stream));
					h->copy_pending[o] = true;
					queued = true;
				}
			}
			if (hits && !queued) HIPCHK(hipMemcpyAsync(hits, sorted.p, bytes, hipMemcpyDeviceToHost, h->stream));
			h->last_n_out = n_deliver; h->last_out = o;
		}
		tq4 = tq();
		HIPCHK(hipEventRecord(h->ev[9], h->stream));
		HIPCHK(hipStreamSynchronize(h->stream));
		if (dbg_t) fprintf(stderr, "[bhip] delivery host ms: reserve+memset %.3f, sort launches %.3f, pointer check %.3f, copy enqueue %.3f, sync %.3f\n", tq1, tq2 - tq1, tq3 - tq2, tq4 - tq3, tq() - tq4);
		S.ms_h2d = h->cur->st_ms_h2d; S.ms_stage_copy = h->cur->st_ms_copy; S.ms_stage_route = h->cur->st_ms_route; S.ms_d2h = ev_ms(h->ev[8], h->ev[9]) + (sorted_ahead ? ev_ms(h->ev[4], h->ev[5]) : 0.0f); S.ms_total = ev_ms(h->ev[0], h->ev[9]);
		slot->state = 2;
		h->res_valid = false;
		return BHIP_OK;
	}
	return fail(BHIP_E_INTERNAL, "buffers kept overflowing");
}

extern "C" int bhip_align_batch(void *handle, const uint8_t *q_codes, const uint64_t *q_off, const uint16_t *q_emac,
                                const uint32_t *q_six, const uint8_t *q_rc, const uint8_t *q_flags,
                                uint32_t n_q, uint32_t n_shared, int all_hits,
                                BhipHit *hits, uint64_t cap, uint64_t *n_hits) {
	if (!n_hits) return fail(BHIP_E_ARG, "null argument");
	*n_hits = 0;
	int rc = bhip_stage_queries(handle, q_codes, q_off, q_emac, q_six, q_rc, q_flags, n_q, n_shared);
	if (rc) return rc;
	return bhip_align_staged(handle, all_hits, hits, cap, n_hits);
}

extern "C" int bhip_align_pairs(void *handle, const uint8_t *q_codes, const uint64_t *q_off, const uint16_t *q_emac,
                                uint32_t n_q, const uint32_t *pair_q, const uint32_t *pair_clump, uint64_t n_pairs, uint8_t *mins) {
	Handle *h = (Handle *)handle;
	if (!h || !q_codes || !q_off || !q_emac || !pair_q || !pair_clump || !mins) return fail(BHIP_E_ARG, "null argument");
	memset(&h->stats, 0, sizeof h->stats);
	for (StageSlot &S : h->slots) { S.state = 0; S.st_valid = false; }
	h->cur = &h->slots[0];
	if (!n_pairs || !n_q) return BHIP_OK;
	HIPCHK(hipSetDevice(h->device));
	int rc;
	if ((rc = ensure_lanes(h, 1))) return rc;
	Lane *L = h->lanes[0];
	uint32_t maxlen = 0;
	for (uint32_t i = 0; i < n_q; ++i) maxlen = std::max<uint32_t>(maxlen, (uint32_t)(q_off[i + 1] - q_off[i]));
	if (maxlen > BHIP_MAX_QLEN) return fail(BHIP_E_QUERYLEN, "query longer than %d", BHIP_MAX_QLEN);
	const int cls = class_of_len(std::max<uint32_t>(maxlen, 1)), NW = class_words(cls, maxlen);
	std::vector<uint2> pr(n_pairs);
	for (uint64_t p = 0; p < n_pairs; ++p) {
		if (pair_q[p] >= n_q || pair_clump[p] >= h->n_clumps) return fail(BHIP_E_ARG, "pair %llu out of range", (unsigned long long)p);
		pr[p] = make_uint2(pair_q[p], pair_clump[p]);
	}
	h->cur->st_has_six = false; h->cur->st_has_rc = false;
	if ((rc = upload_queries(h, q_codes, q_off, q_emac, nullptr, nullptr, n_q))) return rc;
	if ((rc = L->peq.reserve((size_t)n_q * 16 * NW * 4))) return rc;
	if ((rc = h->pairs.reserve(n_pairs * sizeof(uint2)))) return rc;
	if ((rc = h->mins.reserve(n_pairs * 16))) return rc;
	hipStream_t st = h->stream;
	HIPCHK(hipMemcpyAsync(h->pairs.p, pr.data(), n_pairs * sizeof(uint2), hipMemcpyHostToDevice, st));
	HIPCHK(hipMemsetAsync(L->counters.p, 0, sizeof(Counters), st));
	Counters *dc = L->counters.as<Counters>();
	const uint32_t qb = 256u / (uint32_t)NW;
	hipLaunchKernelGGL(k_build_peq, dim3((uint32_t)std::min<uint64_t>(((uint64_t)n_q + qb - 1) / qb, (uint64_t)h->n_cu * 16)), dim3(256), 0, st,
		h->cur->qcodes.as<uint8_t>(), h->cur->qoff.as<uint64_t>(), (const uint32_t *)nullptr, n_q, NW, 0, h->mm, L->peq.as<uint32_t>(), (const uint32_t *)nullptr, 0u, h->peq_rows);
	HIPCHK(hipGetLastError());
	HIPCHK(hipEventRecord(h->ev[0], st));
	launch_myers(h, L, st, NW, (uint32_t)std::min<uint64_t>((n_pairs + 15) / 16, (uint64_t)h->n_cu * 8), h->pairs.as<uint2>(), nullptr, n_pairs, 0, nullptr,
		nullptr, nullptr, 0, nullptr, h->mins.as<uint8_t>(), dc);
	HIPCHK(hipGetLastError());
	HIPCHK(hipEventRecord(h->ev[1], st));
	HIPCHK(hipMemcpyAsync(mins, h->mins.p, n_pairs * 16, hipMemcpyDeviceToHost, st));
	Counters hc;
	HIPCHK(hipMemcpyAsync(&hc, dc, sizeof hc, hipMemcpyDeviceToHost, st));
	HIPCHK(hipStreamSynchronize(st));
	h->stats.n_queries = n_q; h->stats.n_pairs = n_pairs; h->stats.n_columns = hc.col_sum; h->stats.myers_launches = 1;
	h->stats.bytes_algorithmic = 8ull * hc.col_sum + hc.qlen_sum / 2 + 192ull * n_pairs;
	h->stats.ms_myers = ev_ms(h->ev[0], h->ev[1]); h->stats.ms_total = h->stats.ms_myers;
	return BHIP_OK;
}

extern "C" int bhip_prefilter(void *handle, const uint8_t *q_codes, const uint64_t *q_off, const uint16_t *q_emac, uint32_t n_q,
                              uint32_t *out_q, uint32_t *out_clump, uint32_t *out_count, uint64_t cap, uint64_t *n_out) {
	Handle *h = (Handle *)handle;
	if (!h || !q_codes || !q_off || !q_emac || !n_out) return fail(BHIP_E_ARG, "null argument");
	if (!h->has_acx) return fail(BHIP_E_ARG, "handle has no accelerator");
	*n_out = 0;
	for (StageSlot &S : h->slots) { S.state = 0; S.st_valid = false; }
	h->cur = &h->slots[0];
	if (!n_q) return BHIP_OK;
	HIPCHK(hipSetDevice(h->device));
	int rc;
	if ((rc = ensure_lanes(h, 1))) return rc;
	Lane *L = h->lanes[0];
	for (int attempt = 0; attempt < 4; ++attempt) {
		if ((rc = upload_queries(h, q_codes, q_off, q_emac, nullptr, nullptr, n_q))) return rc;
		{
			std::vector<uint32_t> plan(n_q, 1u);
			for (uint32_t i = 0; i < n_q; ++i) plan[i] = make_seed_plan(q_codes + q_off[i], (uint32_t)(q_off[i + 1] - q_off[i]), q_emac[i], (uint32_t)h->K, h->opt_prefilter_stride, h->alt);
			if ((rc = upload_plan(h, q_codes, q_off, q_emac, n_q, plan))) return rc;
	{
		const uint32_t qw_g = (h->cur->st_maxlen + 7) / 8;
		if ((rc = h->cur->qpack.reserve((size_t)n_q * qw_g * 4 + 16))) return rc;
		const uint64_t total = (uint64_t)n_q * qw_g;
		if (total) hipLaunchKernelGGL(k_pack_queries, dim3((uint32_t)std::min<uint64_t>((total + 255) / 256, (uint64_t)h->n_cu * 16)), dim3(256), 0, h->stream,
			h->cur->qcodes.as<uint8_t>(), h->cur->qoff.as<uint64_t>(), n_q, qw_g, h->cur->qpack.as<uint32_t>());
		HIPCHK(hipGetLastError());
	}
		}
		if ((rc = L->cand.reserve(L->cand_cap * sizeof(uint2)))) return rc;
		if ((rc = L->candcnt.reserve(L->cand_cap * sizeof(uint32_t)))) return rc;
		HIPCHK(hipStreamSynchronize(h->stream));
		HIPCHK(hipMemsetAsync(L->counters.p, 0, sizeof(Counters), L->stream));
		Counters *dc = L->counters.as<Counters>();
		HIPCHK(hipEventRecord(h->ev[0], L->stream));
		if ((rc = launch_prefilter(h, L, L->stream, nullptr, n_q, L->cand.as<uint2>(), L->candcnt.as<uint32_t>(), (uint32_t)L->cand_cap, false, &dc->n_cand, dc))) return rc;
		HIPCHK(hipEventRecord(h->ev[1], L->stream));
		Counters hc;
		HIPCHK(hipMemcpyAsync(&hc, dc, sizeof hc, hipMemcpyDeviceToHost, L->stream));
		HIPCHK(hipStreamSynchronize(L->stream));
		if (hc.n_cand > L->cand_cap) { L->cand_cap = (uint64_t)hc.n_cand + 1024; continue; }
		*n_out = hc.n_cand;
		memset(&h->stats, 0, sizeof h->stats);
		h->stats.n_queries = n_q; h->stats.n_pairs = hc.n_cand; h->stats.acx_entries_read = hc.ent_read; h->stats.ms_prefilter = ev_ms(h->ev[0], h->ev[1]);
		if (hc.n_cand > cap) return fail(BHIP_E_CAPACITY, "candidate buffer holds %llu, %u needed", (unsigned long long)cap, hc.n_cand);
		std::vector<uint2> c(hc.n_cand); std::vector<uint32_t> cc(hc.n_cand);
		if (hc.n_cand) {
			HIPCHK(hipMemcpy(c.data(), L->cand.p, hc.n_cand * sizeof(uint2), hipMemcpyDeviceToHost));
			HIPCHK(hipMemcpy(cc.data(), L->candcnt.p, hc.n_cand * sizeof(uint32_t), hipMemcpyDeviceToHost));
		}
		std::vector<uint32_t> ord(hc.n_cand);
		for (uint32_t i = 0; i < hc.n_cand; ++i) ord[i] = i;
		std::sort(ord.begin(), ord.end(), [&](uint32_t a, uint32_t b) { return c[a].x != c[b].x ? c[a].x < c[b].x : c[a].y < c[b].y; });
		for (uint32_t i = 0; i < hc.n_cand; ++i) {
			if (out_q) out_q[i] = c[ord[i]].x;
			if (out_clump) out_clump[i] = c[ord[i]].y;
			if (out_count) out_count[i] = cc[ord[i]];
		}
		return BHIP_OK;
	}
	return fail(BHIP_E_INTERNAL, "candidate buffer kept overflowing");
}

extern "C" int bhip_copy_hits_device(void *handle, void *dst_device, uint64_t cap_records, uint64_t *n_records) {
	Handle *h = (Handle *)handle;
	if (!h || !n_records) return fail(BHIP_E_ARG, "null argument");
	*n_records = h->last_n_out;
	if (!h->last_n_out) return BHIP_OK;
	if (!dst_device && cap_records) return fail(BHIP_E_ARG, "null destination");
	if (h->last_n_out > cap_records) return fail(BHIP_E_CAPACITY, "device buffer holds %llu records, %llu needed", (unsigned long long)cap_records, (unsigned long long)h->last_n_out);
	HIPCHK(hipSetDevice(h->device));
	HIPCHK(hipMemcpyAsync(dst_device, (h->last_out ? h->out_sorted2 : h->out_sorted).p, (size_t)h->last_n_out * sizeof(BhipHit), hipMemcpyDeviceToDevice, h->stream));
	HIPCHK(hipStreamSynchronize(h->stream));
	return BHIP_OK;
}

extern "C" int bhip_sync_hits(void *handle) {
	Handle *h = (Handle *)handle;
	if (!h) return fail(BHIP_E_ARG, "null handle");
	HIPCHK(hipSetDevice(h->device));
	for (int o = 0; o < 2; ++o) if (h->copy_pending[o]) { HIPCHK(hipEventSynchronize(h->ev_copied[o])); h->copy_pending[o] = false; }
	return BHIP_OK;
}
```

burst_amd/csrc/bhip_handle.h:

```cpp
#ifndef BHIP_HANDLE_H
#define BHIP_HANDLE_H
#include <hip/hip_runtime.h>
#include <hipcub/hipcub.hpp>
#include <string>
#include <stdint.h>
#include <stdio.h>
#include <stdarg.h>
#include <stdlib.h>
#include <string.h>
#include <algorithm>
#include <vector>
#include <mutex>
#include <atomic>
#include <chrono>
#include <thread>
#include "burst_hip.h"
#include "bhip_internal.h"

__global__ void k_acx_offsets(const uint32_t *, uint64_t, int, uint32_t *, unsigned long long *);
__global__ void k_acx_lines(const uint32_t *, uint64_t, int, unsigned long long *, uint4 *);
__global__ void k_acx_decode(const uint8_t *, const unsigned long long *, const uint32_t *, BhipAcxView, uint64_t, int, uint32_t, uint32_t *, uint32_t *);
__global__ void k_transpose_refs(const uint8_t *, const uint64_t *, const uint32_t *, const uint64_t *, uint32_t, uint4 *);
__global__ void k_build_peq(const uint8_t *, const uint64_t *, const uint32_t *, uint32_t, int, int, BhipMatchMask, uint32_t *, const uint32_t *, uint32_t, uint32_t);
template <bool LDS_CNT> __global__ void k_prefilter(const uint8_t *, const uint64_t *, const uint16_t *, const uint32_t *, uint32_t,
	BhipAcxView, int, uint32_t, uint32_t *, const uint32_t *, uint32_t, uint2 *, uint32_t *, uint32_t *, uint32_t,
	unsigned long long *, const uint32_t *, const uint32_t *, const uint32_t *);
__global__ void k_prefilter_hash(const uint8_t *, const uint64_t *, const uint16_t *, const uint32_t *, uint32_t, BhipAcxView, int,
	const uint32_t *, uint32_t, uint2 *, uint32_t *, uint32_t *, uint32_t, unsigned long long *, const uint32_t *, uint32_t *, uint32_t *);
template <typename CNT> __global__ void k_prefilter_wave(const uint8_t *, const uint64_t *, const uint16_t *, const uint32_t *, uint32_t,
	BhipAcxView, int, uint32_t, const uint32_t *, uint32_t, uint2 *, uint32_t *, uint32_t *, uint32_t, unsigned long long *, const uint32_t *,
	const uint32_t *, const uint32_t *);
template <int NW> __global__ void k_myers(const uint2 *, const uint32_t *, uint64_t, uint32_t, uint32_t, const uint32_t *, const uint32_t *,
	const uint64_t *, const uint16_t *, const uint32_t *, const uint4 *, const uint64_t *, const uint32_t *, uint32_t,
	BhipRawHit *, uint32_t *, uint32_t, uint32_t *, uint8_t *, unsigned long long *, unsigned long long *);
__global__ void k_myers_long(const uint2 *, const uint32_t *, uint64_t, uint32_t, uint32_t, const uint32_t *, const uint32_t *,
	const uint64_t *, const uint16_t *, const uint32_t *, const uint4 *, const uint64_t *, const uint32_t *, uint32_t,
	BhipRawHit *, uint32_t *, uint32_t, uint32_t *, uint8_t *, unsigned long long *, unsigned long long *, uint32_t);
template <int NWP> __global__ void k_myers_prefix(const uint2 *, const uint32_t *, uint64_t, uint32_t, uint32_t, const uint32_t *, const uint32_t *,
	const uint64_t *, const uint16_t *, const uint4 *, const uint64_t *, const uint32_t *, uint32_t, BhipWin *, uint32_t *, uint32_t,
	unsigned long long *, unsigned long long *, uint32_t *, const uint32_t *);
template <int NW> __global__ void k_myers_window(const BhipWin *, const uint32_t *, uint32_t, int, int, const uint32_t *, const uint32_t *,
	const uint4 *, BhipRawHit *, uint32_t *, uint32_t, uint32_t *, unsigned long long *, const uint32_t *);
template <int BW> __global__ void k_myers_window_band(const BhipWin *, const uint32_t *, uint32_t, int, int, const uint32_t *, const uint32_t *,
	const uint4 *, BhipRawHit *, uint32_t *, uint32_t, uint32_t *, unsigned long long *, const uint32_t *);
__global__ void k_extract_kmers(const uint4 *, const uint64_t *, const uint32_t *, const uint64_t *, uint32_t, uint32_t, int, unsigned long long *, uint16_t *, uint32_t *);
__global__ void k_attach_masks(BhipAcxView, uint64_t, const unsigned long long *, const uint16_t *, uint32_t, const uint32_t *, uint32_t *, uint32_t, uint32_t);
template <int HTB> __global__ void k_prefilter_mask(const uint2 *, const uint2 *, uint32_t, uint32_t, const uint32_t *, const uint32_t *, uint32_t, const uint32_t *, uint32_t,
	uint2 *, uint32_t *, uint32_t, unsigned long long *, uint32_t *, uint32_t *, unsigned long long *, unsigned long long *, unsigned long long *,
	uint2 *, uint32_t *, uint32_t);
template <int MODE, int BIG> __global__ void k_prefilter_cq(const uint2 *, const uint2 *, uint32_t, uint32_t, const uint32_t *, const uint32_t *, uint32_t, const uint32_t *, uint32_t,
	uint2 *, uint32_t *, uint32_t, unsigned long long *, uint32_t *, uint32_t *, unsigned long long *, unsigned long long *, unsigned long long *, unsigned long long *,
	uint2 *, uint32_t *, int, const uint32_t *, const uint32_t *, int);
template <int MODE, int BIG> __global__ void k_prefilter_cw(const uint2 *, const uint2 *, uint32_t, uint32_t, const uint32_t *, const uint32_t *, uint32_t, const uint32_t *, uint32_t,
	uint2 *, uint32_t *, uint32_t, unsigned long long *, uint32_t *, uint32_t *, unsigned long long *, unsigned long long *, unsigned long long *, unsigned long long *,
	uint2 *, uint32_t *, int, const uint32_t *, const uint32_t *, int);
__global__ void k_task_filter(const uint2 *, const uint32_t *, uint32_t, const uint32_t *, const uint32_t *, const uint32_t *, uint2 *, uint32_t *);
__global__ void k_seed_ranges(const uint8_t *, const uint64_t *, const uint32_t *, uint32_t, BhipAcxView, int, const uint32_t *, uint32_t, uint2 *, uint2 *, const uint32_t *, uint32_t, const uint16_t *, uint4 *, const uint32_t *, uint32_t, uint32_t, BhipAlt);
template <int NWP> __global__ void k_myers_prefix_task(const uint2 *, const uint32_t *, uint32_t, const uint32_t *, const uint32_t *, const uint64_t *,
	const uint16_t *, const uint4 *, const uint64_t *, const uint32_t *, BhipWin *, uint32_t *, uint32_t, unsigned long long *, uint32_t *, const uint4 *, const uint32_t *);
template <bool WIDE> __global__ void k_rescore(const BhipRawHit *, const uint32_t *, uint32_t, const uint32_t *, const uint32_t *,
	const uint32_t *, int, const uint8_t *, const uint64_t *, const uint32_t *, const uint8_t *, const uint8_t *, const uint64_t *,
	const uint32_t *, const uint8_t *, BhipHit *, uint32_t *, uint32_t, uint32_t *, uint32_t *, uint32_t *, unsigned long long *,
	unsigned long long, uint32_t *, const uint32_t *, uint32_t, uint32_t, uint32_t);
__global__ void k_pack_queries(const uint8_t *, const uint64_t *, uint32_t, uint32_t, uint32_t *);
__global__ void k_unpack4(const uint8_t *, uint64_t, uint64_t, uint8_t *);
__global__ void k_unpack2(const uint8_t *, uint64_t, uint64_t, uint8_t *);
__global__ void k_span_fill(const uint64_t *, uint32_t, uint32_t, uint64_t, uint32_t, uint64_t *, uint32_t *, uint32_t *);
__global__ void k_route(const uint64_t *, const uint32_t *, uint32_t, const uint16_t *, const uint32_t *, const uint8_t *, uint32_t, uint32_t, uint32_t, int, int, int,
	uint32_t *, uint8_t *, uint32_t *, BhipStageInfo *, BhipAlt);
__global__ void k_rescore_classify(const BhipRawHit *, const uint32_t *, uint32_t, const uint32_t *, int, const uint64_t *, const uint32_t *, const uint8_t *,
	const uint32_t *, BhipHit *, uint32_t *, uint32_t, uint32_t *, uint32_t *, uint32_t *, uint32_t *, uint32_t, int);
template <int SET> __global__ void k_rescore_reg(const BhipRawHit *, const uint32_t *, const uint32_t *, uint32_t, const uint64_t *, const uint8_t *, const uint32_t *, uint32_t,
	const uint8_t *, const uint64_t *, const uint32_t *, const uint8_t *, BhipHit *, uint32_t *, uint32_t, uint32_t *);
int bhip_fail_msg(int code, const char *fmt, ...) __attribute__((format(printf, 2, 3)));
#define fail(...) bhip_fail_msg(__VA_ARGS__)
inline bool bhip_trace_sync() { static const bool on = getenv("BHIP_TRACE_SYNC") != nullptr; return on; }
#define HIPCHK(x) do { hipError_t e_ = (x); if (e_ != hipSuccess) \
	return fail(BHIP_E_DEVICE, "%s:%d %s: %s", __FILE__, __LINE__, #x, hipGetErrorString(e_)); \
	if (bhip_trace_sync()) { fprintf(stderr, "[bhip sync] %s:%d\n", __FILE__, __LINE__); (void)hipDeviceSynchronize(); } } while (0)

inline std::mutex &bhip_vmm_mutex() { static std::mutex m; return m; }
inline std::atomic<int> &bhip_vmm_peer_access() { static std::atomic<int> f(0); return f; }
struct DBuf {
	void *p = nullptr; size_t cap = 0;
	bool vmm = false; size_t va_size = 0; int vmm_device = 0;
	std::vector<hipMemGenericAllocationHandle_t> chunks;
	size_t n_mapped = 0;
	static constexpr size_t kChunk = 1ull << 30;
	static hipError_t malloc_patiently(void **q, size_t want) {
		hipError_t e = hipMalloc(q, want);
		if (e != hipErrorOutOfMemory) return e;
		(void)hipGetLastError();
		size_t last_free = 0, total = 0;
		(void)hipMemGetInfo(&last_free, &total);
		const bool dbg = getenv("BHIP_DEBUG") != nullptr;
		if (dbg) fprintf(stderr, "[bhip] hipMalloc(%zu) found no memory with %.2f GB reported free: waiting for memory that is on its way back\n", want, last_free / 1e9);
		for (int tries = 0; tries < 80; ++tries) {
			std::this_thread::sleep_for(std::chrono::milliseconds(100));
			e = hipMalloc(q, want);
			if (e != hipErrorOutOfMemory) { if (dbg) fprintf(stderr, "[bhip] ... there after %d ms\n", 100 * (tries + 1)); return e; }
			(void)hipGetLastError();
			if (dbg && tries % 10 == 9) { size_t f = 0; (void)hipMemGetInfo(&f, &total); fprintf(stderr, "[bhip] ... %d ms: %.2f GB reported free\n", 100 * (tries + 1), f / 1e9); }
		}
		return e;
	}
	static void poison(void *q, size_t n) {
		static const char *ev = getenv("BHIP_POISON");
		if (ev && q) { (void)hipMemset(q, atoi(ev) & 255, n); (void)hipDeviceSynchronize(); if (getenv("BHIP_DEBUG")) fprintf(stderr, "[bhip] buffer %p .. %p (%zu bytes)\n", q, (void *)((char *)q + n), n); }
	}
	int reserve(size_t bytes) {
		if (bytes <= cap) return 0;
		release();
		size_t want = bytes + bytes / 4 + 256;
		hipError_t e = malloc_patiently(&p, want);
		if (e != hipSuccess) { p = nullptr; return fail(BHIP_E_DEVICE, "hipMalloc(%zu): %s", want, hipGetErrorString(e)); }
		poison(p, want);
		cap = want; return 0;
	}
	int reserve_exact(size_t bytes) {
		if (bytes <= cap) return 0;
		release();
		hipError_t e = malloc_patiently(&p, bytes);
		if (e != hipSuccess) { p = nullptr; return fail(BHIP_E_DEVICE, "hipMalloc(%zu): %s", bytes, hipGetErrorString(e)); }
		poison(p, bytes);
		cap = bytes; return 0;
	}
	int reserve_growable(size_t max_bytes, int device) {
		release();
		std::lock_guard<std::mutex> lk(bhip_vmm_mutex());
		int ok = 0;
		if (hipDeviceGetAttribute(&ok, hipDeviceAttributeVirtualMemoryManagementSupported, device) != hipSuccess || !ok) { (void)hipGetLastError(); return 1; }
		const size_t sz = ((max_bytes + kChunk - 1) / kChunk + 1) * kChunk;
		if (hipMemAddressReserve(&p, sz, kChunk, nullptr, 0) != hipSuccess) { (void)hipGetLastError(); p = nullptr; return 1; }
		vmm = true; va_size = sz; vmm_device = device; cap = 0; n_mapped = 0;
		chunks.assign(sz / kChunk, nullptr);
		peers.clear();
		int n_dev = 0;
		if (bhip_vmm_peer_access().load() && hipGetDeviceCount(&n_dev) == hipSuccess) for (int d = 0; d < n_dev; ++d) { int can = 0; if (d != device && hipDeviceCanAccessPeer(&can, d, device) == hipSuccess && can) peers.push_back(d); }
		(void)hipGetLastError();
		return 0;
	}
	std::vector<int> peers;
	int map_chunks(size_t c0, size_t c1) {
		if (!vmm) return fail(BHIP_E_INTERNAL, "map_chunks on a fixed buffer");
		if (c1 > chunks.size()) return fail(BHIP_E_DEVICE, "record area: chunk %zu wanted, %zu reserved", c1, chunks.size());
		hipMemAllocationProp prop = {};
		prop.type = hipMemAllocationTypePinned; prop.location.type = hipMemLocationTypeDevice; prop.location.id = vmm_device;
		hipMemAccessDesc acc = {};
		acc.location.type = hipMemLocationTypeDevice; acc.location.id = vmm_device; acc.flags = hipMemAccessFlagsProtReadWrite;
		for (size_t c = c0; c < c1; ++c) {
			if (chunks[c]) continue;
			std::lock_guard<std::mutex> lk(bhip_vmm_mutex());
			hipMemGenericAllocationHandle_t hnd;
			hipError_t e = hipMemCreate(&hnd, kChunk, &prop, 0);
			if (e != hipSuccess) return fail(BHIP_E_DEVICE, "hipMemCreate(%zu) with %zu chunks mapped: %s", kChunk, n_mapped, hipGetErrorString(e));
			e = hipMemMap((char *)p + c * kChunk, kChunk, 0, hnd, 0);
			if (e == hipSuccess && !peers.empty()) {
				std::vector<hipMemAccessDesc> all(1 + peers.size(), acc);
				for (size_t k = 0; k < peers.size(); ++k) all[1 + k].location.id = peers[k];
				if (hipMemSetAccess((char *)p + c * kChunk, kChunk, all.data(), all.size()) != hipSuccess) { (void)hipGetLastError(); peers.clear(); }
			}
			if (e == hipSuccess && peers.empty()) e = hipMemSetAccess((char *)p + c * kChunk, kChunk, &acc, 1);
			if (e != hipSuccess) { (void)hipMemRelease(hnd); return fail(BHIP_E_DEVICE, "hipMemMap with %zu chunks mapped: %s", n_mapped, hipGetErrorString(e)); }
			chunks[c] = hnd; ++n_mapped;
		}
		size_t pre = cap / kChunk;
		while (pre < chunks.size() && chunks[pre]) ++pre;
		cap = pre * kChunk;
		return 0;
	}
	int grow_to(size_t bytes) {
		if (!vmm) return fail(BHIP_E_INTERNAL, "grow_to on a fixed buffer");
		if (bytes > va_size) return fail(BHIP_E_DEVICE, "record area: %zu bytes wanted, %zu reserved", bytes, va_size);
		return map_chunks(0, (bytes + kChunk - 1) / kChunk);
	}
	int grow_top_to(size_t bytes) {
		if (!vmm) return fail(BHIP_E_INTERNAL, "grow_top_to on a fixed buffer");
		if (bytes > va_size) return fail(BHIP_E_DEVICE, "record area: %zu bytes wanted at its top, %zu reserved", bytes, va_size);
		return map_chunks(chunks.size() - (bytes + kChunk - 1) / kChunk, chunks.size());
	}
	void shrink_to(size_t bytes) {
		if (!vmm) return;
		const size_t keep = (bytes + kChunk - 1) / kChunk;
		std::lock_guard<std::mutex> lk(bhip_vmm_mutex());
		for (size_t c = keep; c < chunks.size(); ++c) if (chunks[c]) {
			(void)hipMemUnmap((char *)p + c * kChunk, kChunk); (void)hipMemRelease(chunks[c]);
			chunks[c] = nullptr; --n_mapped;
		}
		if (cap > keep * kChunk) cap = keep * kChunk;
	}
	void release() {
		if (vmm) {
			std::lock_guard<std::mutex> lk(bhip_vmm_mutex());
			for (size_t c = 0; c < chunks.size(); ++c) if (chunks[c]) { (void)hipMemUnmap((char *)p + c * kChunk, kChunk); (void)hipMemRelease(chunks[c]); }
			chunks.clear(); n_mapped = 0;
			if (p) (void)hipMemAddressFree(p, va_size);
			vmm = false; va_size = 0;
		} else if (p) (void)hipFree(p);
		p = nullptr; cap = 0;
	}
	template <class T> T *as() const { return (T *)p; }
};

static const int kClasses[] = {2, 4, 6, 8, 10, 16, 32, 128};
static const int kNumClasses = BHIP_N_CLASSES;
static inline int class_of_len(uint32_t len) {
	for (int i = 0; i < kNumClasses - 1; ++i) if (len <= 32u * kClasses[i]) return i;
	return kNumClasses - 1;
}
static inline int class_words(int cls, uint32_t maxlen) { return cls == kNumClasses - 1 ? (int)((std::max<uint32_t>(maxlen, 1025u) + 31u) / 32u) : kClasses[cls]; }

struct Counters {
	uint32_t n_cand, n_raw, n_out, n_wide, err, pad0;
	uint32_t n_cand_cls[8];
	uint32_t n_wins_cls[8];
	uint32_t n_fb, n_fb2;
	uint32_t n_tasks_cls[8];
	uint32_t n_tasks2_cls[8];
	uint32_t n_tasks2k_cls[8];
	uint32_t n_wins2_cls[8];
	uint32_t n_rs[12];
	unsigned long long wcol_sum, tcol_sum, unit_sum;
	unsigned long long col_sum, qlen_sum, ent_read, scratch_used;
	unsigned long long surv_sum;
	uint32_t win_class_seen[4];
};

struct StageSlot {
	DBuf qcodes, qcodes4, qlen16, qoff, qemac, qsix, qrc, qflags, qmap, off_raw, plan, qpack, key, key_sorted, idx, idx_sorted, sort_tmp, info;
	DBuf qcodes_s, qoff_s, qemac_s, qpack_s, nx, nx_six;
	BhipStageInfo *info_pinned = nullptr;
	hipEvent_t ev_begin = nullptr, ev_done = nullptr, ev_copied = nullptr;
	int state = 0;
	uint64_t seq = 0;
	bool resolved = false;
	bool st_valid = false, st_has_six = false, st_has_rc = false, st_has_junk = false, has_flags = false, has_qmap = false;
	uint32_t st_nq = 0, st_nshared = 0, st_maxlen = 0, st_maxE = 0, st_lanes = 1;
	float st_ms_h2d = 0, st_ms_copy = 0, st_ms_route = 0;
	std::vector<BhipQuerySpan> spans;
	const uint32_t *six_explicit = nullptr;
	uint32_t npf[16][BHIP_N_CLASSES], nex[16][BHIP_N_CLASSES], maxE[16][BHIP_N_CLASSES], maxwords[16][BHIP_N_CLASSES], qlist_off[16][BHIP_N_CLASSES], maxlen_lane[16], n_entries_lane[16];
	uint64_t seed_words[16][BHIP_N_CLASSES];
	void release_all() {
		DBuf *b[] = {&qcodes, &qcodes4, &qlen16, &qoff, &qemac, &qsix, &qrc, &qflags, &qmap, &off_raw, &plan, &qpack, &key, &key_sorted, &idx, &idx_sorted,
			&sort_tmp, &info, &qcodes_s, &qoff_s, &qemac_s, &qpack_s, &nx, &nx_six};
		for (DBuf *x : b) x->release();
		if (info_pinned) { (void)hipHostFree(info_pinned); info_pinned = nullptr; }
		if (ev_begin) { (void)hipEventDestroy(ev_begin); ev_begin = nullptr; }
		if (ev_done) { (void)hipEventDestroy(ev_done); ev_done = nullptr; }
		if (ev_copied) { (void)hipEventDestroy(ev_copied); ev_copied = nullptr; }
	}
};

struct Lane {
	hipStream_t stream = nullptr;
	hipEvent_t ev_cls[kNumClasses][8];
	hipEvent_t ev_rs[2];
	hipEvent_t ev_ph[kNumClasses][2];
	hipEvent_t ev_pf[kNumClasses][3];
	uint64_t seed_words[kNumClasses] = {0};
	uint32_t pf_launches = 0;
	bool fb_dirty = false;
	bool pf_masked[kNumClasses] = {false};
	bool pruned[kNumClasses] = {false};
	int pf_algo_used = 0;
	int pf_algo = 0;
	const uint32_t *qlist[kNumClasses] = {nullptr};
	DBuf peq, peqp, cand, candcnt, wins, raw, wide, scratch, fb_list, gcnt, counters, tasks, tasks2, tasks2k, wins2, rs_lists;
	DBuf ranges_c[kNumClasses], hdr_c[kNumClasses];
	DBuf qmeta_c[2][kNumClasses];
	uint64_t qmeta_seq[2][kNumClasses] = {};
	bool seeded_ok[kNumClasses] = {false};
	uint64_t seeded_seq[kNumClasses] = {0};
	uint32_t seeded_n[kNumClasses] = {0}, seeded_W16[kNumClasses] = {0};
	hipEvent_t ev_seed[2][kNumClasses][2];
	DBuf peq_alt, peqp_alt;
	bool alt_ok = false; uint64_t alt_seq = 0; int alt_cls = 0, alt_nwp = 0; uint32_t alt_n = 0;
	hipEvent_t ev_peq_alt[2], ev_peq_cur[2];
	bool peq_ahead[kNumClasses] = {false};
	uint64_t task_cap = 1 << 20;
	uint64_t cand_cap = 1 << 18, raw_cap = 1 << 18, win_cap = 1 << 20, scratch_cap = 1 << 18;
	uint32_t npf[kNumClasses] = {0}, nex[kNumClasses] = {0}, maxE[kNumClasses] = {0}, maxwords[kNumClasses] = {0}, maxlen = 0, n_entries = 0;
	Counters *hc_pinned = nullptr;
	Counters hc;
	uint32_t launches = 0, prefix_words = 0;
	uint64_t n_pairs_ex = 0;
	bool masked = false;
};

struct SharedCtr { uint32_t n_out, err; uint32_t *cnt; uint32_t *rank; };
__global__ void k_set_rank_ptrs(SharedCtr *sc, uint32_t *cnt, uint32_t *rank);
struct Handle {
	int device = 0, n_cu = 0;
	char dev_name[256];
	uint64_t hbm = 0;
	hipStream_t stream = nullptr;
	hipStream_t pf_stream = nullptr;
	hipStream_t sweep_stream = nullptr;
	hipStream_t post_stream = nullptr;
	hipEvent_t ev[10];
	uint32_t n_clumps = 0, tot_refs = 0, max_clump_len = 0;
	DBuf ref_lane, ref_off, clump_len, lut;
	BhipMatchMask mm;
	BhipAlt alt;
	bool has_acx = false; int K = 0;
	int acx_z = 0;
	DBuf acx_lines, acx_rec, bad; uint32_t n_bad = 0; uint64_t n_ent = 0, acx_bias = 0;
	BhipAcxView acx_view() const {
		BhipAcxView v; v.lines = acx_lines.as<uint4>();
		v.rec = acx_rec.as<uint32_t>() - acx_bias; return v;
	}
	bool has_masks = false;
	int opt_lane_masks = 1;
	StageSlot slots[3];
	StageSlot *cur = &slots[0];
	uint64_t stage_seq = 0;
	hipStream_t stage_stream = nullptr;
	bool res_valid = false; uint64_t res_seq = 0; int res_all_hits = 0; uint32_t res_n = 0; BhipStats res_stats;
	int opt_host_routing = 0;
	DBuf best, out, shared_ctr, mins, pairs;
	DBuf ref_order, best_key; uint32_t n_order = 0;
	uint32_t *nsel_pinned = nullptr;
	bool res_sel = false; uint32_t res_n_raw = 0;
	SharedCtr *hsc_pinned = nullptr;
	const uint8_t *s_codes() const { return cur->st_has_junk ? cur->qcodes_s.as<uint8_t>() : cur->qcodes.as<uint8_t>(); }
	const uint64_t *s_off() const { return cur->st_has_junk ? cur->qoff_s.as<uint64_t>() : cur->qoff.as<uint64_t>(); }
	const uint16_t *s_emac() const { return cur->st_has_junk ? cur->qemac_s.as<uint16_t>() : cur->qemac.as<uint16_t>(); }
	const uint32_t *s_pack() const { return cur->st_has_junk ? cur->qpack_s.as<uint32_t>() : cur->qpack.as<uint32_t>(); }
	DBuf sort_keys, sort_keys2, sort_idx, sort_tmp, out_sorted, out_sorted2, sort_scratch;
	uint64_t out_cap = 1 << 20;
	std::vector<uint32_t> h_clump_len;
	BhipStats stats;
	std::vector<Lane *> lanes;
	int opt_two_stage = 1;
	int opt_prefilter_stride = 0;
	int opt_lanes = 1;
	int opt_sweep_blocks = 8;
	uint32_t peq_rows = 16;
	int opt_oversub = 2;
	int opt_band_blocks = 0;
	int opt_no_band = 0;
	int opt_async_d2h = 0, out_idx = 0;
	hipStream_t copy_stream = nullptr;
	hipEvent_t ev_sorted = nullptr, ev_copied[2] = {nullptr, nullptr};
	bool copy_pending[2] = {false, false};
	void *reg_ptr[2] = {nullptr, nullptr}; size_t reg_bytes[2] = {0, 0};
	int last_out = 0;
	uint64_t last_n_out = 0;
	int opt_prune = 1;
	int opt_lane_min = 32768;
	int opt_rescore_reg = 1;
	int opt_pf_waves = 0;
	int opt_pf_algo = -1;
	int opt_pf_table = 0;
	int opt_pf_cw = 2;
	int opt_pf_bytes = 1;
	int opt_pf_rb = 0;
	int opt_seed_ahead = 1;
	int opt_seed_ahead_blocks = 2;
	int opt_peq_ahead_blocks = 16;
	void (*enqueued_hook)(void *) = nullptr; void *enqueued_ctx = nullptr;
	int opt_seed_min_need = -1;
	int opt_seed_drop_len = 8;
	double acx_wmean = 0.0;
};

static inline float ev_ms(hipEvent_t a, hipEvent_t b) { float ms = 0; (void)hipEventElapsedTime(&ms, a, b); return ms; }

int  ensure_lanes(Handle *h, uint32_t n);
uint32_t make_seed_plan(const uint8_t *s, uint32_t len, uint32_t E, uint32_t K, int stride_opt, const BhipAlt &A);
int  slot_init(StageSlot *S);
int  resolve_slot(Handle *h, StageSlot *S);
void apply_slot(Handle *h, StageSlot *S);
void lane_capacity_floor(Handle *h, Lane *L, uint64_t n);
int  bhip_load_accelerator(Handle *h, const uint32_t *acx_lens, const void *acx_lists, int acx_fmt, int K, const uint32_t *badlist, uint32_t n_bad);
int  bhip_build_accelerator(Handle *h, int K, int z);
#endif
```

burst_amd/csrc/bhip_init.hip:

```cpp
#include "bhip_handle.h"

static thread_local char g_err[512] = "";

__global__ void k_ref_symbol_scan(const uint32_t *__restrict__ w, uint64_t n_words, uint32_t *__restrict__ flag) {
	uint32_t any = 0;
	for (uint64_t i = blockIdx.x * (uint64_t)blockDim.x + threadIdx.x; i < n_words; i += (uint64_t)gridDim.x * blockDim.x) {
		const uint32_t d = w[i];
		any |= (d | ((d << 1) & ((d << 2) | (d << 3)))) & 0x88888888u;
	}
	if (any) *flag = 1u;
}
int bhip_fail_msg(int code, const char *fmt, ...) {
	va_list ap; va_start(ap, fmt); vsnprintf(g_err, sizeof g_err, fmt, ap); va_end(ap);
	return code;
}

extern "C" const char *bhip_last_error(void) { return g_err; }
extern "C" int bhip_abi_version(void) { return BHIP_ABI_VERSION; }
std::atomic<int> &bhip_vmm_peer_access_flag() { return bhip_vmm_peer_access(); }

static void lane_destroy(Lane *L) {
	if (!L) return;
	DBuf *all[] = {&L->peq, &L->peqp, &L->cand, &L->candcnt, &L->wins, &L->raw, &L->wide, &L->scratch, &L->fb_list, &L->gcnt, &L->counters, &L->tasks, &L->tasks2, &L->tasks2k, &L->wins2, &L->rs_lists};
	for (DBuf *b : all) b->release();
	L->peq_alt.release(); L->peqp_alt.release();
	for (auto &e : L->ev_peq_alt) if (e) (void)hipEventDestroy(e);
	for (auto &e : L->ev_peq_cur) if (e) (void)hipEventDestroy(e);
	for (DBuf &b : L->ranges_c) b.release();
	for (DBuf &b : L->hdr_c) b.release();
	for (auto &pb : L->qmeta_c) for (DBuf &b : pb) b.release();
	for (auto &pe : L->ev_seed) for (auto &ce : pe) for (auto &e : ce) if (e) (void)hipEventDestroy(e);
	for (auto &ce : L->ev_cls) for (auto &e : ce) if (e) (void)hipEventDestroy(e);
	for (auto &e : L->ev_rs) if (e) (void)hipEventDestroy(e);
	for (auto &ce : L->ev_pf) for (auto &e : ce) if (e) (void)hipEventDestroy(e);
	for (auto &ce : L->ev_ph) for (auto &e : ce) if (e) (void)hipEventDestroy(e);
	if (L->hc_pinned) (void)hipHostFree(L->hc_pinned);
	delete L;
}

static int lane_create(Handle *h, Lane **out) {
	Lane *L = new Lane();
	memset(L->ev_cls, 0, sizeof L->ev_cls); memset(L->ev_rs, 0, sizeof L->ev_rs); memset(L->ev_pf, 0, sizeof L->ev_pf); memset(L->ev_ph, 0, sizeof L->ev_ph); memset(L->ev_seed, 0, sizeof L->ev_seed); memset(L->ev_peq_alt, 0, sizeof L->ev_peq_alt); memset(L->ev_peq_cur, 0, sizeof L->ev_peq_cur);
	L->stream = h->stream;
	for (auto &ce : L->ev_cls) for (auto &e : ce) if (hipEventCreate(&e) != hipSuccess) { lane_destroy(L); return fail(BHIP_E_DEVICE, "hipEventCreate failed"); }
	for (auto &e : L->ev_rs) if (hipEventCreate(&e) != hipSuccess) { lane_destroy(L); return fail(BHIP_E_DEVICE, "hipEventCreate failed"); }
	for (auto &ce : L->ev_pf) for (auto &e : ce) if (hipEventCreate(&e) != hipSuccess) { lane_destroy(L); return fail(BHIP_E_DEVICE, "hipEventCreate failed"); }
	for (auto &ce : L->ev_ph) for (auto &e : ce) if (hipEventCreate(&e) != hipSuccess) { lane_destroy(L); return fail(BHIP_E_DEVICE, "hipEventCreate failed"); }
	for (auto &pe : L->ev_seed) for (auto &ce : pe) for (auto &e : ce) if (hipEventCreate(&e) != hipSuccess) { lane_destroy(L); return fail(BHIP_E_DEVICE, "hipEventCreate failed"); }
	for (auto &e : L->ev_peq_alt) if (hipEventCreate(&e) != hipSuccess) { lane_destroy(L); return fail(BHIP_E_DEVICE, "hipEventCreate failed"); }
	for (auto &e : L->ev_peq_cur) if (hipEventCreate(&e) != hipSuccess) { lane_destroy(L); return fail(BHIP_E_DEVICE, "hipEventCreate failed"); }
	int rc = L->counters.reserve(sizeof(Counters));
	if (rc) { lane_destroy(L); return rc; }
	if (hipHostMalloc((void **)&L->hc_pinned, sizeof(Counters), hipHostMallocDefault) != hipSuccess) { lane_destroy(L); return fail(BHIP_E_DEVICE, "hipHostMalloc failed"); }
	(void)h;
	*out = L;
	return 0;
}

extern "C" void bhip_destroy(void *handle) {
	Handle *h = (Handle *)handle;
	if (!h) return;
	(void)hipSetDevice(h->device);
	if (h->stream) (void)hipStreamSynchronize(h->stream);
	if (h->sweep_stream) (void)hipStreamSynchronize(h->sweep_stream);
	if (h->pf_stream) (void)hipStreamSynchronize(h->pf_stream);
	if (h->post_stream) (void)hipStreamSynchronize(h->post_stream);
	if (h->stage_stream) (void)hipStreamSynchronize(h->stage_stream);
	for (StageSlot &S : h->slots) S.release_all();
	if (h->hsc_pinned) (void)hipHostFree(h->hsc_pinned);
	if (h->nsel_pinned) (void)hipHostFree(h->nsel_pinned);
	for (Lane *L : h->lanes) lane_destroy(L);
	DBuf *all[] = {&h->ref_lane, &h->ref_off, &h->clump_len, &h->lut, &h->acx_lines, &h->acx_rec, &h->bad,
		&h->best, &h->out, &h->shared_ctr, &h->mins, &h->pairs, &h->sort_keys, &h->sort_keys2, &h->sort_idx,
		&h->sort_tmp, &h->out_sorted, &h->out_sorted2, &h->sort_scratch, &h->ref_order, &h->best_key};
	for (int o = 0; o < 2; ++o) {
		if (h->copy_pending[o] && h->ev_copied[o]) (void)hipEventSynchronize(h->ev_copied[o]);
		if (h->reg_ptr[o]) (void)hipHostUnregister(h->reg_ptr[o]);
		if (h->ev_copied[o]) (void)hipEventDestroy(h->ev_copied[o]);
	}
	if (h->ev_sorted) (void)hipEventDestroy(h->ev_sorted);
	if (h->copy_stream) (void)hipStreamDestroy(h->copy_stream);
	for (DBuf *b : all) b->release();
	for (auto &e : h->ev) if (e) (void)hipEventDestroy(e);
	if (h->stream) (void)hipStreamDestroy(h->stream);
	if (h->pf_stream) (void)hipStreamDestroy(h->pf_stream);
	if (h->stage_stream) (void)hipStreamDestroy(h->stage_stream);
	delete h;
}


extern "C" int bhip_init(int device, const void *edx_packed, const uint32_t *clump_len, uint32_t n_clumps, uint32_t tot_refs,
                         const uint32_t *acx_lens, const void *acx_lists, int acx_fmt, int K,
                         const uint32_t *badlist, uint32_t n_bad, const uint8_t score_lut[256], int xalpha, void **handle) {
	if (!handle) return fail(BHIP_E_ARG, "handle is NULL");
	*handle = nullptr;
	if (xalpha) return fail(BHIP_E_ARG, "xalpha (-x) databases are not supported on the device");
	if (!edx_packed || !clump_len || !n_clumps || !score_lut) return fail(BHIP_E_ARG, "empty database");
	if (acx_lens && (K < 4 || K > 15 || !acx_lists || (acx_fmt != 0 && acx_fmt != 1)))
		return fail(BHIP_E_ARG, "bad accelerator arguments (K=%d fmt=%d)", K, acx_fmt);
	if (!acx_lens && K && (K < 4 || K > 15)) return fail(BHIP_E_ARG, "bad accelerator word length K=%d", K);
	int ndev = 0;
	HIPCHK(hipGetDeviceCount(&ndev));
	if (device < 0 || device >= ndev) return fail(BHIP_E_DEVICE, "device %d not present (%d visible)", device, ndev);
	HIPCHK(hipSetDevice(device));
	Handle *h = new Handle();
	memset(h->ev, 0, sizeof h->ev);
	memset(&h->stats, 0, sizeof h->stats);
	h->device = device;
	hipDeviceProp_t prop;
	if (hipGetDeviceProperties(&prop, device) == hipSuccess) {
		h->n_cu = prop.multiProcessorCount; h->hbm = prop.totalGlobalMem;
		snprintf(h->dev_name, sizeof h->dev_name, "%s (%s)", prop.name, prop.gcnArchName);
	}
	if (h->n_cu <= 0) h->n_cu = 256;
	#define INITCHK(x) do { hipError_t e_ = (x); if (e_ != hipSuccess) { \
		fail(BHIP_E_DEVICE, "%s:%d %s: %s", __FILE__, __LINE__, #x, hipGetErrorString(e_)); bhip_destroy(h); return BHIP_E_DEVICE; } } while (0)
	#define INITRC(x) do { int rc_ = (x); if (rc_) { bhip_destroy(h); return rc_; } } while (0)
	INITCHK(hipStreamCreateWithFlags(&h->stream, hipStreamNonBlocking));
	h->sweep_stream = h->stream; h->post_stream = h->stream;
	INITCHK(hipStreamCreateWithFlags(&h->pf_stream, hipStreamNonBlocking));
	INITCHK(hipStreamCreateWithFlags(&h->stage_stream, hipStreamNonBlocking));
	for (auto &e : h->ev) INITCHK(hipEventCreate(&e));
	h->n_clumps = n_clumps; h->tot_refs = tot_refs;
	h->h_clump_len.assign(clump_len, clump_len + n_clumps);
	for (int a = 0; a < 16; ++a) {
		uint16_t m = 0;
		for (int b = 0; b < 16; ++b) if (score_lut[16 * a + b] == 0) m |= (uint16_t)(1u << b);
		h->mm.m[a] = m;
		uint8_t n = 0, bases = 0;
		for (int b = 1; b <= 4; ++b) if (m & (1u << b)) { bases |= (uint8_t)((b - 1) << (2 * n)); ++n; }
		h->alt.n[a] = n; h->alt.base[a] = bases;
	}
	std::vector<uint64_t> src_off(n_clumps + 1), dst_off(n_clumps + 1);
	src_off[0] = dst_off[0] = 0;
	for (uint32_t c = 0; c < n_clumps; ++c) {
		src_off[c + 1] = src_off[c] + clump_len[c] / 2u + (clump_len[c] & 1);
		dst_off[c + 1] = dst_off[c] + (clump_len[c] + 31) / 32u;
		if (clump_len[c] > h->max_clump_len) h->max_clump_len = clump_len[c];
	}
	{
		DBuf d_src, d_srcoff;
		INITRC(d_src.reserve(src_off[n_clumps] * 16 + 16));
		INITRC(d_srcoff.reserve((n_clumps + 1) * sizeof(uint64_t)));
		INITRC(h->ref_lane.reserve_exact(dst_off[n_clumps] * 256 + 256));
		INITRC(h->ref_off.reserve((n_clumps + 1) * sizeof(uint64_t)));
		INITRC(h->clump_len.reserve(n_clumps * sizeof(uint32_t)));
		INITRC(h->lut.reserve(256));
		INITCHK(hipMemcpyAsync(d_src.p, edx_packed, src_off[n_clumps] * 16, hipMemcpyHostToDevice, h->stream));
		INITCHK(hipMemcpyAsync(d_srcoff.p, src_off.data(), (n_clumps + 1) * sizeof(uint64_t), hipMemcpyHostToDevice, h->stream));
		INITCHK(hipMemcpyAsync(h->ref_off.p, dst_off.data(), (n_clumps + 1) * sizeof(uint64_t), hipMemcpyHostToDevice, h->stream));
		INITCHK(hipMemcpyAsync(h->clump_len.p, clump_len, n_clumps * sizeof(uint32_t), hipMemcpyHostToDevice, h->stream));
		INITCHK(hipMemcpyAsync(h->lut.p, score_lut, 256, hipMemcpyHostToDevice, h->stream));
		const uint32_t grid = std::min<uint32_t>(n_clumps, (uint32_t)h->n_cu * 8);
		hipLaunchKernelGGL(k_transpose_refs, dim3(grid), dim3(256), 0, h->stream, d_src.as<uint8_t>(), d_srcoff.as<uint64_t>(),
			h->clump_len.as<uint32_t>(), h->ref_off.as<uint64_t>(), n_clumps, h->ref_lane.as<uint4>());
		INITCHK(hipGetLastError());
		DBuf d_flag;
		INITRC(d_flag.reserve(sizeof(uint32_t)));
		INITCHK(hipMemsetAsync(d_flag.p, 0, sizeof(uint32_t), h->stream));
		hipLaunchKernelGGL(k_ref_symbol_scan, dim3((uint32_t)h->n_cu * 8), dim3(256), 0, h->stream, d_src.as<uint32_t>(), src_off[n_clumps] * 4, d_flag.as<uint32_t>());
		INITCHK(hipGetLastError());
		uint32_t any_other = 1;
		INITCHK(hipMemcpyAsync(&any_other, d_flag.p, sizeof(uint32_t), hipMemcpyDeviceToHost, h->stream));
		INITCHK(hipStreamSynchronize(h->stream));
		h->peq_rows = any_other ? 16u : 5u;
		d_src.release(); d_srcoff.release(); d_flag.release();
	}
	if (getenv("BHIP_DEBUG")) { size_t f_ = 0, t_ = 0; if (hipMemGetInfo(&f_, &t_) == hipSuccess) fprintf(stderr, "[bhip] references on the device (%.2f GB, upload buffer released): %.2f GB of the device's %.2f free\n", h->ref_lane.cap / 1e9, f_ / 1e9, t_ / 1e9); }
	h->acx_z = score_lut[16 * 5 + 5] != 0;
	if (acx_lens) INITRC(bhip_load_accelerator(h, acx_lens, acx_lists, acx_fmt, K, badlist, n_bad));
	else if (K) INITRC(bhip_build_accelerator(h, K, h->acx_z));
	INITRC(ensure_lanes(h, 1));
	if (const char *ev = getenv("BHIP_OPTS")) {
		std::string all(ev);
		for (size_t a = 0; a < all.size();) {
			size_t b = all.find(',', a); if (b == std::string::npos) b = all.size();
			const std::string kv = all.substr(a, b - a); a = b + 1;
			const size_t eq = kv.find('=');
			char *end = nullptr;
			const long long v = eq == std::string::npos ? 0 : strtoll(kv.c_str() + eq + 1, &end, 0);
			if (eq == std::string::npos || eq == 0 || !end || end == kv.c_str() + eq + 1 || *end) { fprintf(stderr, "[bhip] BHIP_OPTS: '%s' is not name=<integer>: ignored\n", kv.c_str()); continue; }
			if (bhip_set_option(h, kv.substr(0, eq).c_str(), v)) fprintf(stderr, "[bhip] BHIP_OPTS: %s: ignored\n", bhip_last_error());
		}
	}
	*handle = h;
	return BHIP_OK;
}


extern "C" int bhip_device_info(void *handle, char *name, int name_cap, int *n_cu, uint64_t *hbm_bytes) {
	Handle *h = (Handle *)handle;
	if (!h) return fail(BHIP_E_ARG, "null handle");
	if (name && name_cap > 0) snprintf(name, (size_t)name_cap, "%s", h->dev_name);
	if (n_cu) *n_cu = h->n_cu;
	if (hbm_bytes) *hbm_bytes = h->hbm;
	return BHIP_OK;
}

extern "C" int bhip_set_option(void *handle, const char *name, long long value) {
	Handle *h = (Handle *)handle;
	if (!h || !name) return fail(BHIP_E_ARG, "null argument");
	if (!strcmp(name, "prefilter_stride")) {
		if (value < 0 || value > 64) return fail(BHIP_E_ARG, "prefilter_stride must be 0 (auto) .. 64");
		h->opt_prefilter_stride = (int)value; return BHIP_OK;
	}
	if (!strcmp(name, "two_stage")) { h->opt_two_stage = value != 0; return BHIP_OK; }
	if (!strcmp(name, "host_routing")) { h->opt_host_routing = value != 0; return BHIP_OK; }
	if (!strcmp(name, "discard_staged")) { for (StageSlot &S : h->slots) if (S.state == 1) S.state = 0; h->res_valid = false; return BHIP_OK; }
	if (!strcmp(name, "lane_masks")) { h->opt_lane_masks = value != 0; return BHIP_OK; }
	if (!strcmp(name, "sweep_blocks")) { if (value < 1 || value > 8) return fail(BHIP_E_ARG, "sweep_blocks must be 1 .. 8"); h->opt_sweep_blocks = (int)value; return BHIP_OK; }
	if (!strcmp(name, "lane_min_entries")) { if (value < 1) return fail(BHIP_E_ARG, "lane_min_entries must be >= 1"); h->opt_lane_min = (int)value; return BHIP_OK; }
	if (!strcmp(name, "async_d2h")) { h->opt_async_d2h = value != 0; return BHIP_OK; }
	if (!strcmp(name, "seed_ahead")) { h->opt_seed_ahead = value != 0; return BHIP_OK; }
	if (!strcmp(name, "peq_ahead_blocks")) { if (value < 1 || value > 16) return fail(BHIP_E_ARG, "peq_ahead_blocks must be 1 .. 16"); h->opt_peq_ahead_blocks = (int)value; return BHIP_OK; }
	if (!strcmp(name, "seed_ahead_blocks")) { if (value < 0 || value > 64) return fail(BHIP_E_ARG, "seed_ahead_blocks must be 0 .. 64"); h->opt_seed_ahead_blocks = (int)value; return BHIP_OK; }
	if (!strcmp(name, "band_blocks")) { if (value < 0 || value > 1024) return fail(BHIP_E_ARG, "band_blocks must be 0 .. 1024"); h->opt_band_blocks = (int)value; return BHIP_OK; }
	if (!strcmp(name, "oversub")) { if (value < 1 || value > 16) return fail(BHIP_E_ARG, "oversub must be 1 .. 16"); h->opt_oversub = (int)value; return BHIP_OK; }
	if (!strcmp(name, "band")) { h->opt_no_band = value == 0; return BHIP_OK; }
	if (!strcmp(name, "prune")) { h->opt_prune = value != 0; return BHIP_OK; }
	if (!strcmp(name, "rescore_reg")) { h->opt_rescore_reg = value != 0; return BHIP_OK; }
	if (!strcmp(name, "seed_min_need")) { if (value < -1 || value > 255) return fail(BHIP_E_ARG, "seed_min_need must be -1 (by rule) or 0 .. 255"); h->opt_seed_min_need = (int)value; return BHIP_OK; }
	if (!strcmp(name, "seed_drop_len")) { if (value < 0 || value > (1 << 24)) return fail(BHIP_E_ARG, "seed_drop_len must be 0 .. 2^24"); h->opt_seed_drop_len = (int)value; return BHIP_OK; }
	if (!strcmp(name, "prefilter_waves")) { if (value < 0 || value > 16) return fail(BHIP_E_ARG, "prefilter_waves must be 0 .. 16"); h->opt_pf_waves = (int)value; return BHIP_OK; }
	if (!strcmp(name, "prefilter_algo")) { if (value < -1 || value > 1) return fail(BHIP_E_ARG, "prefilter_algo must be -1, 0 or 1"); h->opt_pf_algo = (int)value; return BHIP_OK; }
	if (!strcmp(name, "prefilter_table")) { if (value != 0 && (value < 9 || value > 11)) return fail(BHIP_E_ARG, "prefilter_table must be 0, 9, 10 or 11"); h->opt_pf_table = (int)value; return BHIP_OK; }
	if (!strcmp(name, "prefilter_cw")) { if (value < 0 || value > 2) return fail(BHIP_E_ARG, "prefilter_cw must be 0, 1 or 2"); h->opt_pf_cw = (int)value; return BHIP_OK; }
	if (!strcmp(name, "prefilter_bytes")) { h->opt_pf_bytes = value != 0; return BHIP_OK; }
	if (!strcmp(name, "prefilter_rb")) { if (value != 0 && (value < 2 || value > 4)) return fail(BHIP_E_ARG, "prefilter_rb must be 0, 2, 3 or 4"); h->opt_pf_rb = (int)value; return BHIP_OK; }
	if (!strcmp(name, "lanes")) {
		if (value < 1 || value > BHIP_MAX_LANES) return fail(BHIP_E_ARG, "lanes must be 1 .. %d", BHIP_MAX_LANES);
		h->opt_lanes = (int)value; for (StageSlot &S : h->slots) { S.state = 0; S.st_valid = false; } return BHIP_OK;
	}
	return fail(BHIP_E_ARG, "unknown option '%s'", name);
}

extern "C" int bhip_get_stats(void *handle, BhipStats *out) {
	Handle *h = (Handle *)handle;
	if (!h || !out) return fail(BHIP_E_ARG, "null argument");
	*out = h->stats;
	return BHIP_OK;
}

int ensure_lanes(Handle *h, uint32_t n) {
	while (h->lanes.size() < n) { Lane *L = nullptr; int rc = lane_create(h, &L); if (rc) return rc; h->lanes.push_back(L); }
	return 0;
}
```

burst_amd/csrc/bhip_stage.hip:

```cpp
#include "bhip_handle.h"

uint32_t make_seed_plan(const uint8_t *s, uint32_t len, uint32_t E, uint32_t K, int stride_opt, const BhipAlt &A) {
	if (len < K) return 1u;
	const uint32_t npos = len - K + 1;
	bool clean = true;
	for (uint32_t i = 0; i < len; ++i) if ((uint32_t)(s[i] - 1u) >= 4u) { clean = false; break; }
	std::vector<uint8_t> valid;
	if (!clean) {
		valid.assign(npos, 0);
		uint32_t run = 0;
		for (uint32_t i = 0; i < len; ++i) { run = ((uint32_t)(s[i] - 1u) < 4u) ? run + 1 : 0; if (i + 1 >= K && run >= K) valid[i + 1 - K] = 1; }
	}
	uint32_t xk = 0, usedk = 0;
	auto sym = [&](uint32_t i) -> uint32_t { return s[i]; };
	auto need_of = [&](uint32_t st) -> int {
		uint32_t W = 0;
		if (clean) W = (len - K) / st + 1;
		else if (st == K) { uint32_t ws; bhip_expand_walk(sym, K, (len - K) / K + 1, A, ws, xk, usedk); W = ws + xk; }
		else for (uint32_t p = 0; p < npos; p += st) W += valid[p];
		return (int)W - (int)(E * ((K + st - 1) / st));
	};
	const uint32_t smin = (len - K) / 254 + 1;
	uint32_t best_s = 0; int best_n = 0;
	if (stride_opt > 0) { best_s = std::max<uint32_t>((uint32_t)stride_opt, smin); best_n = need_of(best_s); }
// ... 162 lines not shown
	for (uint32_t k = 0; k < S->spans.size(); ++k) if (S->spans[k].n) { if (!n_live) first = k; ++n_live; }
	const bool share_by_position = S->st_has_six && !S->six_explicit;
	if (n_live == 1 && S->spans[first].off[0] == 0 && !share_by_position) {
		q_codes = S->spans[first].codes; q_off = S->spans[first].off; q_emac = S->spans[first].emac; q_flags = S->spans[first].flags;
	} else {
		f_off.assign(1, 0);
		for (const BhipQuerySpan &sp : S->spans) {
			if (!sp.n) continue;
			f_codes.insert(f_codes.end(), sp.codes + sp.off[0], sp.codes + sp.off[sp.n]);
			const uint64_t base = f_off.back() - sp.off[0];
			for (uint32_t j = 0; j < sp.n; ++j) { f_off.push_back(sp.off[j + 1] + base); if (share_by_position) f_six.push_back(j); }
			f_emac.insert(f_emac.end(), sp.emac, sp.emac + sp.n);
			if (S->has_flags) f_flags.insert(f_flags.end(), sp.flags, sp.flags + sp.n);
		}
		f_codes.resize(f_codes.size() + 16, 0);
		q_codes = f_codes.data(); q_off = f_off.data(); q_emac = f_emac.data();
		if (share_by_position) q_six = f_six.data();
		if (S->has_flags) q_flags = f_flags.data();
	}
	const size_t n_keys = (size_t)nl * kNumClasses * 2;
	std::vector<uint32_t> plan(n_q, 1u);
	std::vector<uint8_t> nxv(n_q, 0);
	struct Part {
		std::vector<std::vector<uint32_t>> lists;
		std::vector<uint32_t> maxE, maxwords, maxlen, n_entries;
		std::vector<uint64_t> seed_words;
		int err = 0; uint32_t err_i = 0; uint64_t err_len = 0;
		bool junk = false;
	};
	uint32_t n_thr = n_q < 65536 ? 1u : std::max(1u, std::min(32u, std::thread::hardware_concurrency()));
	if (const char *ev = getenv("BHIP_STAGE_THREADS")) { const int v = atoi(ev); if (v > 0 && n_q >= 65536) n_thr = (uint32_t)std::min(v, 64); }
	std::vector<Part> parts(n_thr);
	auto work = [&](uint32_t t) {
		Part &P = parts[t];
		P.lists.resize(n_keys); P.maxE.assign((size_t)nl * kNumClasses, 0); P.maxwords.assign((size_t)nl * kNumClasses, 0);
		P.seed_words.assign((size_t)nl * kNumClasses, 0); P.maxlen.assign(nl, 0); P.n_entries.assign(nl, 0);
		const uint32_t i0 = (uint32_t)((uint64_t)n_q * t / n_thr), i1 = (uint32_t)((uint64_t)n_q * (t + 1) / n_thr);
		std::vector<uint8_t> clean;
		for (uint32_t i = i0; i < i1; ++i) {
			const uint64_t len_all = q_off[i + 1] - q_off[i];
			if (len_all == 0) continue;
			if (len_all > BHIP_MAX_QLEN) { P.err = 1; P.err_i = i; P.err_len = len_all; return; }
			if (q_six && q_six[i] >= nsh) { P.err = 2; P.err_i = i; return; }
			const uint8_t *codes_i = q_codes + q_off[i];
			uint64_t len = len_all;
			uint32_t E_i = q_emac[i];
			if (memchr(codes_i, 0, len_all)) {
				clean.clear();
				for (uint64_t k = 0; k < len_all; ++k) if (codes_i[k]) clean.push_back(codes_i[k]);
				const uint64_t nx_i = len_all - clean.size();
				P.junk = true;
				nxv[i] = (uint8_t)std::min<uint64_t>(nx_i, 255);
				if (nx_i > E_i || clean.empty()) { nxv[i] = 255; continue; }
				E_i -= (uint32_t)nx_i; len = clean.size(); codes_i = clean.data();
			}
			const uint32_t six = q_six ? q_six[i] : i;
			const uint32_t l = (uint32_t)(((uint64_t)six * nl) / nsh);
			const int cls = class_of_len((uint32_t)len);
			int ex = q_flags ? (q_flags[i] == BHIP_Q_EXHAUSTIVE) : !h->has_acx;
			if (!h->has_acx) ex = 1;
			if (!ex) {
				plan[i] = make_seed_plan(codes_i, (uint32_t)len, E_i, (uint32_t)h->K, h->opt_prefilter_stride, h->alt);
				if (BHIP_PLAN_NEED(plan[i]) == 0) ex = 1;
			}
			const size_t lc = (size_t)l * kNumClasses + cls;
			P.lists[lc * 2 + ex].push_back(i);
			P.maxE[lc] = std::max<uint32_t>(P.maxE[lc], E_i);
			if (!ex && len >= (uint64_t)h->K) {
				const uint32_t nwd = (uint32_t)((len - h->K) / (plan[i] & 255u) + 1) + BHIP_PLAN_USED(plan[i]);
				P.maxwords[lc] = std::max<uint32_t>(P.maxwords[lc], nwd);
				P.seed_words[lc] += nwd;
			}
			P.maxlen[l] = std::max<uint32_t>(P.maxlen[l], (uint32_t)len_all);
			++P.n_entries[l];
		}
	};
	if (n_thr == 1) work(0);
	else {
		std::vector<std::thread> th;
		for (uint32_t t = 0; t < n_thr; ++t) th.emplace_back(work, t);
		for (auto &x : th) x.join();
	}
	for (const Part &P : parts) {
		if (P.err == 1) return fail(BHIP_E_QUERYLEN, "query %u has %llu symbols (max %d)", P.err_i, (unsigned long long)P.err_len, BHIP_MAX_QLEN);
		if (P.err == 2) return fail(BHIP_E_ARG, "q_six[%u] out of range", P.err_i);
	}
	BhipStageInfo I;
	memset(&I, 0, sizeof I);
	std::vector<uint32_t> sorted; sorted.reserve(n_q);
	for (uint32_t l = 0; l < nl; ++l) for (int c = 0; c < kNumClasses; ++c) for (int ex = 0; ex < 2; ++ex) {
		const size_t lc = (size_t)l * kNumClasses + c, k = lc * 2 + ex;
		for (const Part &P : parts) { sorted.insert(sorted.end(), P.lists[k].begin(), P.lists[k].end()); I.count[(l * BHIP_N_CLASSES + c) * 2 + ex] += (uint32_t)P.lists[k].size(); }
		if (!ex) for (const Part &P : parts) {
			I.maxE[l * BHIP_N_CLASSES + c] = std::max(I.maxE[l * BHIP_N_CLASSES + c], P.maxE[lc]); I.maxwords[l * BHIP_N_CLASSES + c] = std::max(I.maxwords[l * BHIP_N_CLASSES + c], P.maxwords[lc]);
			I.seed_words[l * BHIP_N_CLASSES + c] += P.seed_words[lc];
		}
	}
	for (uint32_t l = 0; l < nl; ++l) for (const Part &P : parts) { I.maxlen_lane[l] = std::max(I.maxlen_lane[l], P.maxlen[l]); I.n_entries_lane[l] += P.n_entries[l]; }
	for (uint32_t i = 0; i < n_q; ++i) I.maxE_all = std::max<uint32_t>(I.maxE_all, q_emac[i]);
	slot_take_info(S, I);
	hipStream_t st = h->stage_stream;
	HIPCHK(hipMemcpyAsync(S->plan.p, plan.data(), (size_t)n_q * 4, hipMemcpyHostToDevice, st));
	if (!sorted.empty()) HIPCHK(hipMemcpyAsync(S->idx_sorted.p, sorted.data(), sorted.size() * 4, hipMemcpyHostToDevice, st));
	S->st_has_junk = false;
	for (const Part &P : parts) S->st_has_junk |= P.junk;
	if (S->st_has_junk) {
		std::vector<uint64_t> off_s((size_t)n_q + 1, 0);
		std::vector<uint16_t> emac_s(n_q);
		std::vector<uint8_t> codes_s; codes_s.reserve(q_off[n_q] + 16);
		std::vector<uint8_t> nxs(nsh + 1, 0);
		for (uint32_t i = 0; i < n_q; ++i) {
			const uint8_t *c = q_codes + q_off[i]; const uint64_t len = q_off[i + 1] - q_off[i];
			if (!nxv[i]) codes_s.insert(codes_s.end(), c, c + len);
			else if (nxv[i] != 255) for (uint64_t k = 0; k < len; ++k) { if (c[k]) codes_s.push_back(c[k]); }
			off_s[i + 1] = codes_s.size();
			emac_s[i] = (uint16_t)(nxv[i] == 255 ? 0 : q_emac[i] - nxv[i]);
			if (nxv[i] == 255) nxv[i] = 0;
			nxs[q_six ? q_six[i] : i] = nxv[i];
		}
		codes_s.resize(codes_s.size() + 16, 0);
		if ((rc = S->qcodes_s.reserve(codes_s.size()))) return rc;
		if ((rc = S->qoff_s.reserve(((size_t)n_q + 1) * 8))) return rc;
		if ((rc = S->qemac_s.reserve(((size_t)n_q + 1) * 2))) return rc;
		if ((rc = S->nx.reserve((size_t)n_q + 16))) return rc;
		if ((rc = S->nx_six.reserve((size_t)nsh + 16))) return rc;
		HIPCHK(hipMemcpyAsync(S->qcodes_s.p, codes_s.data(), codes_s.size(), hipMemcpyHostToDevice, st));
		HIPCHK(hipMemcpyAsync(S->qoff_s.p, off_s.data(), ((size_t)n_q + 1) * 8, hipMemcpyHostToDevice, st));
		HIPCHK(hipMemcpyAsync(S->qemac_s.p, emac_s.data(), (size_t)n_q * 2, hipMemcpyHostToDevice, st));
		HIPCHK(hipMemcpyAsync(S->nx.p, nxv.data(), n_q, hipMemcpyHostToDevice, st));
		HIPCHK(hipMemcpyAsync(S->nx_six.p, nxs.data(), nsh, hipMemcpyHostToDevice, st));
		const uint32_t qw_g = (S->st_maxlen + 7) / 8;
		if ((rc = S->qpack_s.reserve((size_t)n_q * qw_g * 4 + 64))) return rc;
		const uint64_t total = (uint64_t)n_q * qw_g;
		if (total) hipLaunchKernelGGL(k_pack_queries, dim3((uint32_t)std::min<uint64_t>((total + 255) / 256, (uint64_t)h->n_cu * 16)), dim3(256), 0, st,
			S->qcodes_s.as<uint8_t>(), S->qoff_s.as<uint64_t>(), n_q, qw_g, S->qpack_s.as<uint32_t>());
		HIPCHK(hipGetLastError());
	}
	HIPCHK(hipStreamSynchronize(st));
	return 0;
}

int resolve_slot(Handle *h, StageSlot *S) {
	if (S->resolved) return 0;
	if (!S->st_nq) { S->resolved = true; S->st_valid = true; S->st_lanes = 0; return 0; }
	HIPCHK(hipEventSynchronize(S->ev_done));
	const BhipStageInfo &I = *S->info_pinned;
	if (I.err == 1) return fail(BHIP_E_QUERYLEN, "query %u has %u symbols (max %d)", I.err_i, I.err_len, BHIP_MAX_QLEN);
	if (I.err == 2) return fail(BHIP_E_ARG, "q_six[%u] out of range", I.err_i);
	S->st_ms_h2d = ev_ms(S->ev_begin, S->ev_done);
	S->st_ms_copy = ev_ms(S->ev_begin, S->ev_copied); S->st_ms_route = ev_ms(S->ev_copied, S->ev_done);
	if (I.junk || h->opt_host_routing) { int rc = host_route(h, S); if (rc) return rc; }
	else slot_take_info(S, I);
	S->resolved = true; S->st_valid = true;
	if (getenv("BHIP_DEBUG")) fprintf(stderr, "[bhip] stage: %u entries, %s routing, copies + routing %.2f ms on the staging stream\n", S->st_nq,
		(I.junk || h->opt_host_routing) ? "host" : "device", S->st_ms_h2d);
	return 0;
}

void lane_capacity_floor(Handle *h, Lane *L, uint64_t n) {
	L->task_cap = std::max<uint64_t>(L->task_cap, 3 * n + 4096); L->win_cap = std::max<uint64_t>(L->win_cap, 2 * n + 4096);
	L->raw_cap = std::max<uint64_t>(L->raw_cap, 2 * n + 4096); L->cand_cap = std::max<uint64_t>(L->cand_cap, n / 4 + 4096);
	h->out_cap = std::max<uint64_t>(h->out_cap, 2 * n + 4096);
}

void apply_slot(Handle *h, StageSlot *S) {
	h->cur = S;
	for (uint32_t l = 0; l < S->st_lanes && l < h->lanes.size(); ++l) {
		Lane *L = h->lanes[l];
		for (int c = 0; c < kNumClasses; ++c) {
			L->npf[c] = S->npf[l][c]; L->nex[c] = S->nex[l][c]; L->maxE[c] = S->maxE[l][c]; L->maxwords[c] = S->maxwords[l][c]; L->seed_words[c] = S->seed_words[l][c];
			L->qlist[c] = S->idx_sorted.as<uint32_t>() + S->qlist_off[l][c];
		}
		L->maxlen = S->maxlen_lane[l]; L->n_entries = S->n_entries_lane[l];
		lane_capacity_floor(h, L, L->n_entries);
	}
}

static StageSlot *free_slot(Handle *h) {
	for (StageSlot &S : h->slots) if (S.state == 0) return &S;
	for (StageSlot &S : h->slots) if (S.state == 2) return &S;
	return nullptr;
}

extern "C" int bhip_stage_spans(void *handle, const BhipQuerySpan *spans, uint32_t n_spans, uint32_t n_shared, uint32_t max_len) {
	Handle *h = (Handle *)handle;
	if (!h || (!spans && n_spans)) return fail(BHIP_E_ARG, "null argument");
	HIPCHK(hipSetDevice(h->device));
	StageSlot *S = free_slot(h);
	if (!S) return fail(BHIP_E_ARG, "every staging slot holds a batch that has not been aligned yet: align one first");
	S->state = 0;
	int rc = stage_enqueue(h, S, spans, n_spans, nullptr, true, n_shared, max_len);
	if (rc) return rc;
	S->state = 1;
	return BHIP_OK;
}

extern "C" int bhip_stage_queries(void *handle, const uint8_t *q_codes, const uint64_t *q_off, const uint16_t *q_emac,
                                  const uint32_t *q_six, const uint8_t *q_rc, const uint8_t *q_flags, uint32_t n_q, uint32_t n_shared) {
	Handle *h = (Handle *)handle;
	if (!h) return fail(BHIP_E_ARG, "null handle");
	if (n_q && (!q_codes || !q_off || !q_emac)) return fail(BHIP_E_ARG, "null query arrays");
	HIPCHK(hipSetDevice(h->device));
	for (StageSlot &S : h->slots) if (S.state == 1) S.state = 0;
	StageSlot *S = free_slot(h);
	S->state = 0;
	BhipQuerySpan sp;
	memset(&sp, 0, sizeof sp);
	sp.codes = q_codes; sp.off = q_off; sp.emac = q_emac; sp.rc = q_rc; sp.flags = q_flags; sp.n = n_q; sp.q_base = 0;
	int rc = stage_enqueue(h, S, &sp, n_q ? 1u : 0u, q_six, false, n_shared, 0);
	if (rc) return rc;
	if ((rc = resolve_slot(h, S))) return rc;
	S->spans.clear(); S->six_explicit = nullptr;
	S->state = 1;
	return BHIP_OK;
}
extern "C" void *bhip_alloc_host(uint64_t bytes) {
	void *p = nullptr;
	if (hipHostMalloc(&p, bytes ? bytes : 1, hipHostMallocPortable) != hipSuccess) { (void)hipGetLastError(); return nullptr; }
	void *d = nullptr; hipStream_t st = nullptr;
	if (hipMalloc(&d, 256) == hipSuccess && hipStreamCreateWithFlags(&st, hipStreamNonBlocking) == hipSuccess) {
		(void)hipMemcpyAsync(p, d, bytes < 64 ? bytes : 64, hipMemcpyDeviceToHost, st);
		(void)hipMemcpyAsync(d, p, bytes < 64 ? bytes : 64, hipMemcpyHostToDevice, st);
		(void)hipStreamSynchronize(st);
		hipPointerAttribute_t at;
		memset(&at, 0, sizeof at);
		(void)hipPointerGetAttributes(&at, p);
		if (bytes > 4096) {
			char *mid = (char *)p + ((bytes / 2) & ~(uint64_t)63);
			(void)hipPointerGetAttributes(&at, mid);
			(void)hipMemcpyAsync(mid, d, 64, hipMemcpyDeviceToHost, st);
			(void)hipMemcpyAsync(d, mid, 64, hipMemcpyHostToDevice, st);
			(void)hipStreamSynchronize(st);
		}
	}
	(void)hipGetLastError();
	if (st) (void)hipStreamDestroy(st);
	if (d) (void)hipFree(d);
	return p;
}
extern "C" void bhip_free_host(void *p) { if (p) (void)hipHostFree(p); }
extern "C" int bhip_host_register(void *p, uint64_t bytes) {
	if (!p || !bytes) return BHIP_OK;
	if (hipHostRegister(p, bytes, hipHostRegisterPortable) != hipSuccess) { (void)hipGetLastError(); return fail(BHIP_E_DEVICE, "hipHostRegister(%llu bytes) failed", (unsigned long long)bytes); }
	return BHIP_OK;
}
extern "C" int bhip_host_unregister(void *p) {
	if (p && hipHostUnregister(p) != hipSuccess) { (void)hipGetLastError(); return fail(BHIP_E_DEVICE, "hipHostUnregister failed"); }
	return BHIP_OK;
}
```

Measured before the change: 605.6 million.

## Launch next batch's prefilter ahead on the prefilter stream with double-buffered counters

Adds a run-ahead path that launches the prefilter for the next staged batch while the current batch is still aligning. Counters and prefilter events are double-buffered by batch sequence parity, and a stamp check reuses the early launch only when its class, choice and capacities match. The aim is to hide prefilter latency behind the rest of the pipeline. It also caches hipFuncGetAttributes results and replaces repeated getenv calls with cached flags, at the cost of drain synchronisations when buffers grow or options change.

```diff
diff --git a/burst_amd/csrc/bhip_align.hip b/burst_amd/csrc/bhip_align.hip
--- a/burst_amd/csrc/bhip_align.hip
+++ b/burst_amd/csrc/bhip_align.hip
@@ -152,10 +152,20 @@
 	if (NWP == 1) LT(1); else if (NWP == 2) LT(2); else if (NWP == 3) LT(3); else if (NWP == 4) LT(4); else LT(6);
 	#undef LT
 }
+static bool func_attributes(const void *fn, hipFuncAttributes &fa) {
+	struct Known { const void *fn; hipFuncAttributes fa; };
+	static std::mutex m;
+	static std::vector<Known> known;
+	std::lock_guard<std::mutex> lk(m);
+	for (const Known &k : known) if (k.fn == fn) { fa = k.fa; return true; }
+	memset(&fa, 0, sizeof fa);
+	if (hipFuncGetAttributes(&fa, fn) != hipSuccess) { (void)hipGetLastError(); return false; }
+	known.push_back({fn, fa});
+	return true;
+}
 static uint32_t blocks_per_cu(const void *fn, uint32_t threads, size_t dyn_lds, hipFuncAttributes *fa_out = nullptr) {
 	hipFuncAttributes fa_here, &fa = fa_out ? *fa_out : fa_here;
-	memset(&fa, 0, sizeof fa);
-	if (hipFuncGetAttributes(&fa, fn) != hipSuccess) return 4;
+	if (!func_attributes(fn, fa)) return 4;
 	const uint32_t waves_per_block = (threads + 63) / 64;
 	const uint32_t by_reg = 4u * std::min(8u, 512u / (uint32_t)std::max(8, (fa.numRegs + 7) & ~7)) / waves_per_block;
 	const size_t lds = fa.sharedSizeBytes + dyn_lds;
@@ -222,12 +232,13 @@
 struct PfOverflow {
 	uint32_t *fb1 = nullptr, *n_fb1 = nullptr;
 	uint32_t *fb2 = nullptr, *n_fb2 = nullptr;
-	int begin(Lane *L, Counters *dc, hipStream_t st, uint32_t n_list, bool lane_resolved) {
+	int begin(Lane *L, Counters *dc, hipStream_t st, uint32_t n_list, bool lane_resolved, bool ahead = false) {
 		int rc;
 		if ((rc = L->fb_list.reserve(lane_resolved ? (size_t)n_list * 8 + 64 : (size_t)n_list * 4 + 16))) return rc;
 		fb1 = L->fb_list.as<uint32_t>(); n_fb1 = &dc->n_fb;
 		if (lane_resolved) {
 			fb2 = fb1 + n_list + 8; n_fb2 = &dc->n_fb2;
+			if (ahead) return 0;
 			if (L->pf_launches || L->fb_dirty) HIPCHK(hipMemsetAsync(&dc->n_fb, 0, 8, st));
 			L->fb_dirty = false;
 		} else {
@@ -238,27 +249,40 @@
 	}
 };
 
-static int launch_dense_fallback(Handle *h, Lane *L, hipStream_t st, const uint32_t *d_qlist, uint32_t n_list, const uint32_t *bad, uint32_t n_bad,
+static size_t dense_lds_bytes(const Handle *h, const StageSlot *S, bool *narrow_out = nullptr) {
+	const bool narrow = S->st_maxlen < 255u + (uint32_t)h->K;
+	if (narrow_out) *narrow_out = narrow;
+	return ((size_t)(h->n_clumps + (narrow ? 3 : 1)) / (narrow ? 4 : 2)) * 4 + 1536u * 4 + 512u * 8 + 512u * 4 + 16;
+}
+static size_t dense_gcnt_bytes(const Handle *h, const StageSlot *S, uint32_t n_list) {
+	if (dense_lds_bytes(h, S) <= 64 * 1024) return 0;
+	return (size_t)std::min<uint32_t>(n_list, (uint32_t)h->n_cu * 2) * ((h->n_clumps + 1) / 2) * 4;
+}
+static int launch_dense_fallback(Handle *h, Lane *L, hipStream_t st, const StageSlot *S, const uint32_t *d_qlist, uint32_t n_list, const uint32_t *bad, uint32_t n_bad,
                                  uint2 *cand, uint32_t *candcnt, uint32_t *n_cand_dev, uint32_t cand_cap, Counters *dc, const uint32_t *fb, const uint32_t *n_fb) {
-	const uint32_t *plan = h->cur->plan.as<uint32_t>();
-	const bool narrow = h->cur->st_maxlen < 255u + (uint32_t)h->K;
-	const size_t lds_w = ((size_t)(h->n_clumps + (narrow ? 3 : 1)) / (narrow ? 4 : 2)) * 4 + 1536u * 4 + 512u * 8 + 512u * 4 + 16;
+	const uint32_t *plan = S->plan.as<uint32_t>();
+	const bool junk = S->st_has_junk;
+	const uint8_t *s_codes = junk ? S->qcodes_s.as<uint8_t>() : S->qcodes.as<uint8_t>();
+	const uint64_t *s_off = junk ? S->qoff_s.as<uint64_t>() : S->qoff.as<uint64_t>();
+	const uint16_t *s_emac = junk ? S->qemac_s.as<uint16_t>() : S->qemac.as<uint16_t>();
+	bool narrow;
+	const size_t lds_w = dense_lds_bytes(h, S, &narrow);
 	const uint32_t nw32 = (h->n_clumps + 1) / 2;
 	if (lds_w <= 64 * 1024) {
 		const uint32_t per_cu = (uint32_t)std::max<size_t>(1, std::min<size_t>(16, (160 * 1024) / lds_w));
 		const uint32_t grid = std::min<uint32_t>(n_list, (uint32_t)h->n_cu * per_cu);
-		if (narrow) hipLaunchKernelGGL(k_prefilter_wave<uint8_t>, dim3(grid), dim3(64), lds_w, st, h->s_codes(), h->s_off(),
-			h->s_emac(), d_qlist, n_list, h->acx_view(), h->K, h->n_clumps, bad, n_bad, cand, candcnt,
+		if (narrow) hipLaunchKernelGGL(k_prefilter_wave<uint8_t>, dim3(grid), dim3(64), lds_w, st, s_codes, s_off,
+			s_emac, d_qlist, n_list, h->acx_view(), h->K, h->n_clumps, bad, n_bad, cand, candcnt,
 			n_cand_dev, cand_cap, &dc->ent_read, plan, fb, n_fb);
-		else hipLaunchKernelGGL(k_prefilter_wave<uint16_t>, dim3(grid), dim3(64), lds_w, st, h->s_codes(), h->s_off(),
-			h->s_emac(), d_qlist, n_list, h->acx_view(), h->K, h->n_clumps, bad, n_bad, cand, candcnt,
+		else hipLaunchKernelGGL(k_prefilter_wave<uint16_t>, dim3(grid), dim3(64), lds_w, st, s_codes, s_off,
+			s_emac, d_qlist, n_list, h->acx_view(), h->K, h->n_clumps, bad, n_bad, cand, candcnt,
 			n_cand_dev, cand_cap, &dc->ent_read, plan, fb, n_fb);
 	} else {
 		int rc;
 		const uint32_t grid = std::min<uint32_t>(n_list, (uint32_t)h->n_cu * 2);
 		if ((rc = L->gcnt.reserve((size_t)grid * nw32 * 4))) return rc;
-		hipLaunchKernelGGL(k_prefilter<false>, dim3(grid), dim3(256), 0, st, h->s_codes(), h->s_off(),
-			h->s_emac(), d_qlist, n_list, h->acx_view(), h->K, h->n_clumps,
+		hipLaunchKernelGGL(k_prefilter<false>, dim3(grid), dim3(256), 0, st, s_codes, s_off,
+			s_emac, d_qlist, n_list, h->acx_view(), h->K, h->n_clumps,
 			L->gcnt.as<uint32_t>(), bad, n_bad, cand, candcnt, n_cand_dev, cand_cap, &dc->ent_read, fb, n_fb, plan);
 	}
 	HIPCHK(hipGetLastError());
@@ -280,7 +304,7 @@
 			h->cur->plan.as<uint32_t>(), ov.fb1, ov.n_fb1);
 		HIPCHK(hipGetLastError());
 	}
-	return launch_dense_fallback(h, L, st, d_qlist, n_list, bad, n_bad, cand, candcnt, n_cand_dev, cand_cap, dc, ov.fb1, ov.n_fb1);
+	return launch_dense_fallback(h, L, st, h->cur, d_qlist, n_list, bad, n_bad, cand, candcnt, n_cand_dev, cand_cap, dc, ov.fb1, ov.n_fb1);
 }
 
 static uint32_t seed_row_words(uint32_t maxwords) { return maxwords <= 8 ? 8u : std::max<uint32_t>(16u, (maxwords + 15u) & ~15u); }
@@ -349,16 +373,23 @@
 	return big ? k_prefilter_cw<2, 1> : k_prefilter_cw<2, 0>;
 }
 
-static int launch_prefilter_mask(Handle *h, Lane *L, hipStream_t st, int cls, const uint32_t *d_qlist, uint32_t n_list, uint32_t maxwords, uint32_t *n_tasks_dev,
-                                 uint32_t *n_cand_dev, Counters *dc, int algo, int prune) {
+static BhipPfChoice pf_choice_for(const Handle *h, int algo, uint32_t n_list, uint32_t maxwords, uint64_t seed_words) {
+	const double mean_words = n_list ? (double)seed_words / (double)n_list : (double)maxwords;
+	return bhip_pf_choose(algo, h->opt_pf_cw, h->opt_pf_table, h->opt_pf_rb, seed_row_words(maxwords), mean_words * h->acx_wmean);
+}
+static int launch_prefilter_mask(Handle *h, Lane *L, hipStream_t st, StageSlot *S, int cls, const uint32_t *d_qlist, uint32_t n_list, uint32_t maxwords, uint64_t seed_words,
+                                 Counters *dc, int algo, int prune, bool ahead, int *kind_out) {
 	int rc;
+	uint32_t *n_tasks_dev = &dc->n_tasks_cls[cls], *n_cand_dev = &dc->n_cand_cls[cls];
 	PfOverflow ov;
-	if ((rc = ov.begin(L, dc, st, n_list, true))) return rc;
+	if ((rc = ov.begin(L, dc, st, n_list, true, ahead))) return rc;
 	const uint32_t W16 = seed_row_words(maxwords);
-	const double mean_words = n_list ? (double)L->seed_words[cls] / (double)n_list : (double)maxwords;
-	if (!(L->seeded_ok[cls] && L->seeded_seq[cls] == h->cur->seq && L->seeded_n[cls] == n_list && L->seeded_W16[cls] == W16))
-		if ((rc = launch_seed(h, L, st, h->cur, cls, d_qlist, n_list, maxwords, mean_words))) return rc;
-	const BhipPfChoice c = bhip_pf_choose(algo, h->opt_pf_cw, h->opt_pf_table, h->opt_pf_rb, W16, mean_words * h->acx_wmean);
+	const double mean_words = n_list ? (double)seed_words / (double)n_list : (double)maxwords;
+	if (!(L->seeded_ok[cls] && L->seeded_seq[cls] == S->seq && L->seeded_n[cls] == n_list && L->seeded_W16[cls] == W16)) {
+		if (ahead) return BHIP_E_INTERNAL;
+		if ((rc = launch_seed(h, L, st, S, cls, d_qlist, n_list, maxwords, mean_words))) return rc;
+	}
+	const BhipPfChoice c = pf_choice_for(h, algo, n_list, maxwords, seed_words);
 	const bool filter = c.kind != BHIP_PF_MASK, cw = c.kind == BHIP_PF_CW || c.kind == BHIP_PF_CQ;
 	const bhip_pf_kernel_t fp = filter ? pf_kernel(c, 0) : nullptr, fp2 = filter && c.two_pass ? pf_kernel(c, 1) : nullptr;
 	if (filter && (!fp || (c.two_pass && !fp2)))
@@ -366,13 +397,14 @@
 	hipFuncAttributes fa;
 	const void *fn = filter ? (const void *)fp : c.htb == 9 ? (const void *)k_prefilter_mask<9> : c.htb == 10 ? (const void *)k_prefilter_mask<10> : (const void *)k_prefilter_mask<11>;
 	const uint32_t fit = std::min<uint32_t>(cw ? 32u : 12u, blocks_per_cu(fn, 64u, 0, &fa));
-	if (getenv("BHIP_DEBUG")) {
+	if (h->dbg) {
 		if (cw) fprintf(stderr, "[bhip] prefilter kernel: %s, slot mode %d, %zu B LDS, %d VGPRs -> %u blocks per CU\n", c.kind == BHIP_PF_CQ ? "four queries per wave, streams by the whole wave" : "one query per wave", c.cw_mode, fa.sharedSizeBytes, fa.numRegs, fit);
 		else fprintf(stderr, "[bhip] prefilter kernel: table 2^%d, %d record blocks in registers, %zu B LDS, %d VGPRs -> %u blocks per CU\n", c.htb, c.rb, fa.sharedSizeBytes, fa.numRegs, fit);
 	}
 	const uint32_t waves = h->opt_pf_waves ? std::min<uint32_t>((uint32_t)h->opt_pf_waves, fit) : fit;
 	const uint32_t grid = std::min<uint32_t>(c.kind == BHIP_PF_CW ? n_list : (n_list + 3) / 4, (uint32_t)h->n_cu * waves);
-	HIPCHK(hipEventRecord(L->ev_pf[cls][1], st));
+	hipEvent_t *pe = L->ev_pfx[S->seq & 1][cls];
+	HIPCHK(hipEventRecord(pe[1], st));
 	const uint32_t *fb_dense = ov.fb1, *n_fb_dense = ov.n_fb1;
 	if (filter) {
 		auto launch = [&](bhip_pf_kernel_t k, uint32_t g, uint32_t *fb, uint32_t *n_fb, const uint32_t *sel, const uint32_t *n_sel) {
@@ -398,14 +430,22 @@
 #undef PFM_LAUNCH
 	}
 	HIPCHK(hipGetLastError());
-	HIPCHK(hipEventRecord(L->ev_pf[cls][2], st));
-	++L->pf_launches;
-	L->pf_algo_used = c.kind;
-	return launch_dense_fallback(h, L, st, d_qlist, n_list, h->bad.as<uint32_t>(), h->n_bad, L->cand.as<uint2>(), nullptr, n_cand_dev, (uint32_t)L->cand_cap, dc, fb_dense, n_fb_dense);
-}
-
-static int lane_reserve_work(Lane *L) {
+	HIPCHK(hipEventRecord(pe[2], st));
+	if (!ahead) { ++L->pf_launches; L->pf_algo_used = c.kind; }
+	if (kind_out) *kind_out = c.kind;
+	return launch_dense_fallback(h, L, st, S, d_qlist, n_list, h->bad.as<uint32_t>(), h->n_bad, L->cand.as<uint2>(), nullptr, n_cand_dev, (uint32_t)L->cand_cap, dc, fb_dense, n_fb_dense);
+}
+
+static int lane_reserve_work(Handle *h, Lane *L) {
 	int rc;
+	{
+		const struct { const DBuf *b; size_t bytes; } want[] = {{&L->cand, L->cand_cap * sizeof(uint2)}, {&L->raw, L->raw_cap * sizeof(BhipRawHit)}, {&L->wide, L->raw_cap * sizeof(uint32_t)},
+			{&L->rs_lists, L->raw_cap * sizeof(uint32_t) * 10}, {&L->scratch, L->scratch_cap * sizeof(uint32_t)}, {&L->wins, L->win_cap * sizeof(BhipWin)}, {&L->tasks, L->task_cap * sizeof(uint2)},
+			{&L->tasks2, L->task_cap * sizeof(uint2)}, {&L->tasks2k, L->task_cap * sizeof(uint2)}, {&L->wins2, L->win_cap * sizeof(BhipWin)}};
+		bool grows = false;
+		for (const auto &w : want) grows |= w.bytes > w.b->cap;
+		if (grows) ahead_drain(h);
+	}
 	if ((rc = L->cand.reserve(L->cand_cap * sizeof(uint2))) || (rc = L->raw.reserve(L->raw_cap * sizeof(BhipRawHit))) || (rc = L->wide.reserve(L->raw_cap * sizeof(uint32_t))) ||
 	    (rc = L->rs_lists.reserve(L->raw_cap * sizeof(uint32_t) * 10)) || (rc = L->scratch.reserve(L->scratch_cap * sizeof(uint32_t))) || (rc = L->wins.reserve(L->win_cap * sizeof(BhipWin))) ||
 	    (rc = L->tasks.reserve(L->task_cap * sizeof(uint2))) || (rc = L->tasks2.reserve(L->task_cap * sizeof(uint2))) || (rc = L->tasks2k.reserve(L->task_cap * sizeof(uint2))) ||
@@ -419,8 +459,9 @@
 	if (!n_entries) return BHIP_OK;
 	if (!max_len || max_len > BHIP_MAX_QLEN) max_len = BHIP_MAX_QLEN;
 	HIPCHK(hipSetDevice(h->device));
+	ahead_drain(h);
 	int rc;
-	if (getenv("BHIP_DEBUG")) { size_t f_ = 0, t_ = 0; if (hipMemGetInfo(&f_, &t_) == hipSuccess) fprintf(stderr, "[bhip] reserve for %u entries of up to %u symbols: %.2f GB of the device's %.2f free\n", n_entries, max_len, f_ / 1e9, t_ / 1e9); }
+	if (h->dbg) { size_t f_ = 0, t_ = 0; if (hipMemGetInfo(&f_, &t_) == hipSuccess) fprintf(stderr, "[bhip] reserve for %u entries of up to %u symbols: %.2f GB of the device's %.2f free\n", n_entries, max_len, f_ / 1e9, t_ / 1e9); }
 	const size_t n = n_entries, nb = total_symbols ? (size_t)std::min<uint64_t>(total_symbols + 64, (uint64_t)n * max_len) : n * max_len, qw = (max_len + 7) / 8;
 	const size_t cw = (size_t)class_words(class_of_len(max_len), max_len);
 	const size_t peq_words = total_symbols ? std::min<size_t>(n * cw, 2 * (nb / 32 + n)) : n * cw;
@@ -434,12 +475,12 @@
 		HIPCHK(hipcub::DeviceRadixSort::SortPairs(nullptr, tb, S.key.as<uint8_t>(), S.key_sorted.as<uint8_t>(), S.idx.as<uint32_t>(), S.idx_sorted.as<uint32_t>(), (int)n, 0, 8, h->stage_stream));
 		if ((rc = S.sort_tmp.reserve(tb + 16))) return rc;
 	}
-	if (getenv("BHIP_DEBUG")) { size_t f_ = 0, t_ = 0; if (hipMemGetInfo(&f_, &t_) == hipSuccess) fprintf(stderr, "[bhip] ... staging slots reserved: %.2f GB free\n", f_ / 1e9); }
+	if (h->dbg) { size_t f_ = 0, t_ = 0; if (hipMemGetInfo(&f_, &t_) == hipSuccess) fprintf(stderr, "[bhip] ... staging slots reserved: %.2f GB free\n", f_ / 1e9); }
 	if ((rc = ensure_lanes(h, 1))) return rc;
 	Lane *L = h->lanes[0];
 	lane_capacity_floor(h, L, n);
 	const int cls = class_of_len(max_len);
-	if ((rc = lane_reserve_work(L)) || (rc = L->peq.reserve(peq_words * 16 * 4)) || (rc = L->peqp.reserve(n * 16 * 6 * 4)) ||
+	if ((rc = lane_reserve_work(h, L)) || (rc = L->peq.reserve(peq_words * 16 * 4)) || (rc = L->peqp.reserve(n * 16 * 6 * 4)) ||
 	    (rc = L->peq_alt.reserve(peq_words * 16 * 4)) || (rc = L->peqp_alt.reserve(n * 16 * 6 * 4)) ||
 	    (rc = L->fb_list.reserve(n * 8 + 64)) || (rc = L->ranges_c[cls].reserve(n * 16 * 8 + 16)) || (rc = L->hdr_c[cls].reserve(n * 8 + 16))) return rc;
 	if (h->n_order) { if ((rc = h->best_key.reserve((n + 1) * 8)) || (rc = h->sort_idx.reserve(std::max<size_t>((size_t)h->out_cap, n + 1) * 4))) return rc; if (!h->nsel_pinned) HIPCHK(hipHostMalloc((void **)&h->nsel_pinned, 64, hipHostMallocDefault)); }
@@ -451,7 +492,7 @@
 		HIPCHK(hipcub::DeviceScan::ExclusiveSum(nullptr, tb, h->sort_keys.as<uint32_t>(), h->sort_keys2.as<uint32_t>(), (int)(n + 1), h->stream));
 		if ((rc = h->sort_tmp.reserve(tb))) return rc;
 	}
-	if (getenv("BHIP_DEBUG")) { size_t f_ = 0, t_ = 0; if (hipMemGetInfo(&f_, &t_) == hipSuccess) fprintf(stderr, "[bhip] ... lane and record buffers reserved: %.2f GB free\n", f_ / 1e9); }
+	if (h->dbg) { size_t f_ = 0, t_ = 0; if (hipMemGetInfo(&f_, &t_) == hipSuccess) fprintf(stderr, "[bhip] ... lane and record buffers reserved: %.2f GB free\n", f_ / 1e9); }
 	if (!h->copy_stream) { HIPCHK(hipStreamCreateWithFlags(&h->copy_stream, hipStreamNonBlocking)); HIPCHK(hipEventCreateWithFlags(&h->ev_sorted, hipEventDisableTiming));
 		for (auto &e : h->ev_copied) HIPCHK(hipEventCreateWithFlags(&e, hipEventDisableTiming)); }
 	{
@@ -513,12 +554,32 @@
 	}
 	return BHIP_OK;
 }
+static bool pf_stamp_for(const Handle *h, const Lane *L, uint64_t seq, const uint32_t *npf, const uint32_t *nex, const uint32_t *maxE, const uint32_t *maxwords,
+                         const uint64_t *seed_words, uint32_t maxlen, int all_hits, PfAhead *out) {
+	int cls = -1, n_cls = 0;
+	for (int c = 0; c < kNumClasses; ++c) if (npf[c] + nex[c]) { cls = c; ++n_cls; }
+	if (n_cls != 1 || !npf[cls] || !h->has_masks || !h->opt_lane_masks) return false;
+	if (!class_prefix_words(h, maxE[cls], class_words(cls, maxlen))) return false;
+	const int pf_algo = bhip_pf_algo(h->opt_pf_algo, L->pf_algo);
+	out->ok = false; out->seq = seq; out->cls = cls; out->n_list = npf[cls]; out->W16 = seed_row_words(maxwords[cls]);
+	out->choice = pf_choice_for(h, pf_algo, npf[cls], maxwords[cls], seed_words[cls]);
+	out->prune = !all_hits && h->opt_prune && npf[cls] + nex[cls] < (1u << 24) && pf_algo == 0;
+	out->task_cap = L->task_cap; out->cand_cap = L->cand_cap; out->raw_cap = L->raw_cap; out->win_cap = L->win_cap; out->scratch_cap = L->scratch_cap;
+	return true;
+}
 static int enqueue_lane(Handle *h, Lane *L, int all_hits, hipEvent_t start, uint32_t band_rows, uint32_t qw, uint32_t rw) {
 	int rc;
-	if ((rc = lane_reserve_work(L))) return rc;
+	if ((rc = lane_reserve_work(h, L))) return rc;
 	hipStream_t pf = h->pf_stream, sw = h->sweep_stream, po = h->post_stream;
-	HIPCHK(hipMemsetAsync(L->counters.p, 0, sizeof(Counters), pf));
-	Counters *dc = L->counters.as<Counters>();
+	Counters *dc = L->ctr(h->cur->seq);
+	bool ran_ahead = false;
+	if (L->ahead.ok) {
+		PfAhead now;
+		ran_ahead = h->opt_pf_ahead && h->cur->st_lanes == 1 && !h->cur->st_has_junk &&
+			pf_stamp_for(h, L, h->cur->seq, L->npf, L->nex, L->maxE, L->maxwords, L->seed_words, L->maxlen, all_hits, &now) && L->ahead.same(now);
+		L->ahead.ok = false;
+	}
+	if (!ran_ahead) HIPCHK(hipMemsetAsync(dc, 0, sizeof(Counters), pf));
 	SharedCtr *sc = h->shared_ctr.as<SharedCtr>();
 	L->launches = 0; L->prefix_words = 0; L->n_pairs_ex = 0; L->pf_launches = 0; L->fb_dirty = false;
 	for (int c = 0; c < kNumClasses; ++c) { L->pf_masked[c] = false; L->pruned[c] = false; }
@@ -541,19 +602,22 @@
 		} else if ((rc = launch_peq(h, sw, h->cur, qlist, n_list, NW, NWP, L->peq, L->peqp))) return rc;
 		L->prefix_words = (uint32_t)NWP;
 		HIPCHK(hipEventRecord(ce[1], sw));
-		HIPCHK(hipEventRecord(ce[7], pf));
+		hipEvent_t *pe = L->ev_pfx[h->cur->seq & 1][cls];
+		if (!ran_ahead) HIPCHK(hipEventRecord(pe[0], pf));
 		const bool masked = NWP && n_pf && h->has_masks && h->opt_lane_masks;
 		const int pf_algo = bhip_pf_algo(h->opt_pf_algo, L->pf_algo);
 		const int prune = masked && !all_hits && h->opt_prune && n_list < (1u << 24) && pf_algo == 0;
+		if (h->dbg && masked) fprintf(stderr, "[bhip] batch %llu (class of %d words): prefilter %s\n", (unsigned long long)h->cur->seq, kClasses[cls], ran_ahead ? "ran ahead, behind the chain of the batch before" : "in place");
 		if (n_pf) {
-			if (masked) { if ((rc = launch_prefilter_mask(h, L, pf, cls, qlist, n_pf, L->maxwords[cls], &dc->n_tasks_cls[cls], &dc->n_cand_cls[cls], dc, pf_algo, prune))) return rc; }
+			if (masked && ran_ahead) { L->pf_launches = 1; L->pf_algo_used = L->ahead_kind; }
+			else if (masked) { if ((rc = launch_prefilter_mask(h, L, pf, h->cur, cls, qlist, n_pf, L->maxwords[cls], L->seed_words[cls], dc, pf_algo, prune, false, nullptr))) return rc; }
 			else if ((rc = launch_prefilter(h, L, pf, qlist, n_pf, L->cand.as<uint2>(), nullptr, (uint32_t)L->cand_cap, true, &dc->n_cand_cls[cls], dc))) return rc;
 		}
 		const uint4 *qmeta_cls = (masked && L->qmeta_seq[h->cur->seq & 1][cls] == h->cur->seq + 1) ? L->qmeta_c[h->cur->seq & 1][cls].as<uint4>() : nullptr;
 		L->masked = masked;
 		L->pf_masked[cls] = masked && n_pf;
-		HIPCHK(hipEventRecord(ce[2], pf));
-		HIPCHK(hipStreamWaitEvent(sw, ce[2], 0));
+		if (!ran_ahead) HIPCHK(hipEventRecord(pe[3], pf));
+		HIPCHK(hipStreamWaitEvent(sw, pe[3], 0));
 		HIPCHK(hipEventRecord(ce[6], sw));
 		if (n_pf) {
 			if (masked) launch_prefix_task(h, L, sw, NWP, (uint32_t)h->n_cu * 4u * (uint32_t)h->opt_sweep_blocks * (uint32_t)h->opt_oversub, L->tasks.as<uint2>(), &dc->n_tasks_cls[cls], qlist, L->wins.as<BhipWin>(), &dc->n_wins_cls[cls], dc, qmeta_cls);
@@ -636,7 +700,7 @@
 	return 0;
 }
 
-static void seed_next_batch(Handle *h, StageSlot *cur, hipEvent_t cur_done) {
+static void seed_next_batch(Handle *h, StageSlot *cur, hipEvent_t cur_done, bool allow_ahead, int all_hits) {
 	if (!h->opt_seed_ahead || !h->has_acx || !h->has_masks || !h->opt_lane_masks || h->opt_host_routing) return;
 	StageSlot *N = nullptr;
 	for (StageSlot &S : h->slots) if (&S != cur && S.state == 1 && (!N || S.seq < N->seq)) N = &S;
@@ -675,6 +739,25 @@
 			L->alt_ok = true; L->alt_seq = N->seq; L->alt_cls = only; L->alt_nwp = NWP; L->alt_n = n_list;
 		}
 	}
+	if (!allow_ahead || !h->opt_pf_ahead || N->st_lanes != 1 || h->lanes.empty() || !((N->seq ^ cur->seq) & 1)) return;
+	Lane *L = h->lanes[0];
+	L->ahead.ok = false;
+	PfAhead st;
+	if (!pf_stamp_for(h, L, N->seq, N->npf[0], N->nex[0], N->maxE[0], N->maxwords[0], N->seed_words[0], N->maxlen_lane[0], all_hits, &st)) return;
+	const int cls = st.cls;
+	if (!(L->seeded_ok[cls] && L->seeded_seq[cls] == N->seq && L->seeded_n[cls] == st.n_list && L->seeded_W16[cls] == st.W16)) return;
+	if (L->tasks.cap < L->task_cap * sizeof(uint2) || L->tasks2.cap < L->task_cap * sizeof(uint2) || L->cand.cap < L->cand_cap * sizeof(uint2) ||
+	    L->fb_list.cap < (size_t)st.n_list * 8 + 64 || L->gcnt.cap < dense_gcnt_bytes(h, N, st.n_list)) return;
+	hipStream_t pf = h->pf_stream;
+	Counters *dc = L->ctr(N->seq);
+	hipEvent_t *pe = L->ev_pfx[N->seq & 1][cls];
+	int kind = 0;
+	if (hipStreamWaitEvent(pf, cur_done, 0) != hipSuccess) { (void)hipGetLastError(); return; }
+	L->ahead_pending = true; L->ahead_call = h->call_no;
+	if (hipMemsetAsync(dc, 0, sizeof(Counters), pf) != hipSuccess || hipEventRecord(pe[0], pf) != hipSuccess ||
+	    launch_prefilter_mask(h, L, pf, N, cls, N->idx_sorted.as<uint32_t>() + N->qlist_off[0][cls], st.n_list, N->maxwords[0][cls], N->seed_words[0][cls], dc, bhip_pf_algo(h->opt_pf_algo, L->pf_algo), st.prune, true, &kind) ||
+	    hipEventRecord(pe[3], pf) != hipSuccess) { (void)hipGetLastError(); return; }
+	L->ahead = st; L->ahead.ok = true; L->ahead_kind = kind;
 }
 
 extern "C" int bhip_set_enqueued_hook(void *handle, void (*fn)(void *), void *ctx) {
@@ -728,15 +811,19 @@
 		HIPCHK(hipGetLastError());
 		return 0;
 	};
+	const bool prev_retried = h->last_call_retried;
+	h->last_call_retried = false;
 	for (int attempt = 0; attempt < 24; ++attempt) {
 		int rc;
 		sorted_ahead = false;
+		if (attempt > 0) { ahead_drain(h); h->last_call_retried = true; }
 		if (h->res_valid && h->res_seq == slot->seq && h->res_all_hits == all_hits_arg) { hsc.n_out = h->res_n_raw; hsc.err = 0; h->stats = h->res_stats; n_deliver = h->res_n; *n_hits = n_deliver; }
 		else {
 		h->res_valid = false;
 		if ((rc = h->best.reserve((size_t)(n_shared + 1) * 4))) return rc;
 		if ((rc = h->out.reserve(h->out_cap * sizeof(BhipHit)))) return rc;
 		if ((rc = h->shared_ctr.reserve(sizeof(SharedCtr)))) return rc;
+		++h->call_no;
 		HIPCHK(hipEventRecord(h->ev[0], h->stream));
 		HIPCHK(hipMemsetAsync(h->best.p, 0xFF, (size_t)n_shared * 4, h->stream));
 		HIPCHK(hipMemsetAsync(h->shared_ctr.p, 0, 2 * sizeof(uint32_t), h->stream));
@@ -773,9 +860,10 @@
 		if (!h->hsc_pinned) HIPCHK(hipHostMalloc((void **)&h->hsc_pinned, sizeof(SharedCtr), hipHostMallocDefault));
 		HIPCHK(hipMemcpyAsync(h->hsc_pinned, h->shared_ctr.p, 2 * sizeof(uint32_t), hipMemcpyDeviceToHost, h->post_stream));
 		HIPCHK(hipEventRecord(h->ev[3], h->post_stream));
-		seed_next_batch(h, slot, h->ev[3]);
+		seed_next_batch(h, slot, h->ev[3], attempt == 0 && !prev_retried, all_hits);
 		if (h->enqueued_hook && attempt == 0) h->enqueued_hook(h->enqueued_ctx);
 		HIPCHK(hipEventSynchronize(h->ev[2]));
+		for (Lane *L : h->lanes) if (L->ahead_pending && L->ahead_call < h->call_no) L->ahead_pending = false;
 		HIPCHK(hipStreamSynchronize(h->sweep_stream));
 		HIPCHK(hipStreamSynchronize(h->post_stream));
 		for (uint32_t l = 0; l < nl; ++l) if (h->lanes[l]->n_entries) h->lanes[l]->hc = *h->lanes[l]->hc_pinned;
@@ -784,13 +872,14 @@
 			const bool cq_min_only = !all_hits && h->opt_pf_cw == 2 && L->pf_algo_used == 3;
 			if (L->n_entries && L->pf_algo == 0 && !cq_min_only && L->hc.ent_read > 100000 && (double)L->hc.surv_sum > (all_hits ? 0.20 : 0.50) * (double)L->hc.ent_read) L->pf_algo = 1;
 		}
-		if (getenv("BHIP_DEBUG")) for (uint32_t l = 0; l < nl; ++l) {
+		if (h->dbg) for (uint32_t l = 0; l < nl; ++l) {
 			const Lane *L = h->lanes[l];
 			if (!L->n_entries) continue;
 			fprintf(stderr, "[bhip] lane %u: %llu list records, %llu survived the counting filter, next prefilter algorithm %d\n", l, (unsigned long long)L->hc.ent_read, (unsigned long long)L->hc.surv_sum, L->pf_algo);
 			for (int cls = 0; cls < kNumClasses; ++cls) if (L->npf[cls] + L->nex[cls])
 				fprintf(stderr, "[bhip] lane %u class NW=%d: prefiltered %u exhaustive %u maxE %u maxwords %u | tasks %u + deferred %u (kept %u) clump pairs %u windows %u + %u | fallback queries(last class) %u raw %u\n",
 					l, kClasses[cls], L->npf[cls], L->nex[cls], L->maxE[cls], L->maxwords[cls], L->hc.n_tasks_cls[cls], L->hc.n_tasks2_cls[cls], L->hc.n_tasks2k_cls[cls], L->hc.n_cand_cls[cls], L->hc.n_wins_cls[cls], L->hc.n_wins2_cls[cls], L->hc.n_fb, L->hc.n_raw);
+			if (L->hc.n_wide) fprintf(stderr, "[bhip] lane %u: %u hits go to the wide-band re-scorer behind the chain\n", l, L->hc.n_wide);
 			if (L->hc.n_fb) fprintf(stderr, "[bhip] lane %u: %u queries overflowed the first prefilter pass, %u the second (dense fallback)\n", l, L->hc.n_fb, L->hc.n_fb2);
 		}
 		bool retry = false;
@@ -813,7 +902,7 @@
 			Lane *L = h->lanes[l];
 			if (!L->n_entries || !L->hc.n_wide) continue;
 			sorted_ahead = false;
-			Counters *dc = L->counters.as<Counters>();
+			Counters *dc = L->ctr(h->cur->seq);
 			SharedCtr *sc = h->shared_ctr.as<SharedCtr>();
 			hipLaunchKernelGGL(k_rescore<true>, dim3(std::min<uint32_t>((L->hc.n_wide + 63) / 64, (uint32_t)h->n_cu * 16)), dim3(64), 256, h->post_stream,
 				L->raw.as<BhipRawHit>(), &dc->n_raw, (uint32_t)L->raw_cap, L->wide.as<uint32_t>(), &dc->n_wide, h->best.as<uint32_t>(), all_hits,
@@ -849,8 +938,9 @@
 				if (!(L->npf[cls] + L->nex[cls])) continue;
 				hipEvent_t *ce = L->ev_cls[cls];
 				S.ms_peq += L->peq_ahead[cls] ? ev_ms(L->ev_peq_cur[0], L->ev_peq_cur[1]) : ev_ms(ce[0], ce[1]);
-				if (L->npf[cls]) S.ms_prefilter += ev_ms(ce[7], ce[2]);
-				if (L->npf[cls] && L->pf_masked[cls]) { { hipEvent_t *es = L->ev_seed[h->cur->seq & 1][cls]; S.ms_seed += ev_ms(es[0], es[1]); } S.ms_prefilter_hash += ev_ms(L->ev_pf[cls][1], L->ev_pf[cls][2]); S.n_seed_words += L->seed_words[cls]; }
+				hipEvent_t *pe = L->ev_pfx[h->cur->seq & 1][cls];
+				if (L->npf[cls]) S.ms_prefilter += ev_ms(pe[0], pe[3]);
+				if (L->npf[cls] && L->pf_masked[cls]) { { hipEvent_t *es = L->ev_seed[h->cur->seq & 1][cls]; S.ms_seed += ev_ms(es[0], es[1]); } S.ms_prefilter_hash += ev_ms(pe[1], pe[2]); S.n_seed_words += L->seed_words[cls]; }
 				float sweep = ev_ms(ce[6], ce[4]), win = ev_ms(ce[4], ce[5]);
 				if (L->pruned[cls]) { const float second = ev_ms(L->ev_ph[cls][0], L->ev_ph[cls][1]); sweep += second; win -= second; }
 				S.ms_myers += sweep + win;
@@ -864,7 +954,7 @@
 		BhipStats &S = h->stats;
 		if (hits && n_deliver > cap) return fail(BHIP_E_CAPACITY, "hit buffer holds %llu records, %u needed", (unsigned long long)cap, n_deliver);
 		HIPCHK(hipEventRecord(h->ev[8], h->stream));
-		const bool dbg_t = getenv("BHIP_DEBUG_TIMES") != nullptr;
+		const bool dbg_t = h->dbg_times;
 		const auto tq0 = std::chrono::steady_clock::now();
 		auto tq = [&]() { return std::chrono::duration<double, std::milli>(std::chrono::steady_clock::now() - tq0).count(); };
 		double tq1 = 0, tq2 = 0, tq3 = 0, tq4 = 0;
@@ -957,6 +1047,7 @@
 	Handle *h = (Handle *)handle;
 	if (!h || !q_codes || !q_off || !q_emac || !pair_q || !pair_clump || !mins) return fail(BHIP_E_ARG, "null argument");
 	memset(&h->stats, 0, sizeof h->stats);
+	ahead_drain(h);
 	for (StageSlot &S : h->slots) { S.state = 0; S.st_valid = false; }
 	h->cur = &h->slots[0];
 	if (!n_pairs || !n_q) return BHIP_OK;
@@ -1007,6 +1098,7 @@
 	if (!h || !q_codes || !q_off || !q_emac || !n_out) return fail(BHIP_E_ARG, "null argument");
 	if (!h->has_acx) return fail(BHIP_E_ARG, "handle has no accelerator");
 	*n_out = 0;
+	ahead_drain(h);
 	for (StageSlot &S : h->slots) { S.state = 0; S.st_valid = false; }
 	h->cur = &h->slots[0];
 	if (!n_q) return BHIP_OK;
diff --git a/burst_amd/csrc/bhip_handle.h b/burst_amd/csrc/bhip_handle.h
--- a/burst_amd/csrc/bhip_handle.h
+++ b/burst_amd/csrc/bhip_handle.h
@@ -16,6 +16,7 @@
 #include <thread>
 #include "burst_hip.h"
 #include "bhip_internal.h"
+#include "bhip_pf_select.h"
 
 __global__ void k_acx_offsets(const uint32_t *, uint64_t, int, uint32_t *, unsigned long long *);
 __global__ void k_acx_lines(const uint32_t *, uint64_t, int, unsigned long long *, uint4 *);
@@ -252,12 +253,28 @@
 	}
 };
 
+struct PfAhead {
+	bool ok = false;
+	uint64_t seq = 0;
+	int cls = 0;
+	uint32_t n_list = 0, W16 = 0;
+	BhipPfChoice choice = {};
+	int prune = 0;
+	uint64_t task_cap = 0, cand_cap = 0, raw_cap = 0, win_cap = 0, scratch_cap = 0;
+	bool same(const PfAhead &o) const {
+		return seq == o.seq && cls == o.cls && n_list == o.n_list && W16 == o.W16 && prune == o.prune && choice.kind == o.choice.kind && choice.htb == o.choice.htb &&
+			choice.rb == o.choice.rb && choice.cw_mode == o.choice.cw_mode && choice.legacy == o.choice.legacy && choice.two_pass == o.choice.two_pass &&
+			task_cap == o.task_cap && cand_cap == o.cand_cap && raw_cap == o.raw_cap && win_cap == o.win_cap && scratch_cap == o.scratch_cap;
+	}
+};
+
 struct Lane {
 	hipStream_t stream = nullptr;
 	hipEvent_t ev_cls[kNumClasses][8];
 	hipEvent_t ev_rs[2];
 	hipEvent_t ev_ph[kNumClasses][2];
 	hipEvent_t ev_pf[kNumClasses][3];
+	hipEvent_t ev_pfx[2][kNumClasses][4];
 	uint64_t seed_words[kNumClasses] = {0};
 	uint32_t pf_launches = 0;
 	bool fb_dirty = false;
@@ -282,6 +299,11 @@
 	uint64_t cand_cap = 1 << 18, raw_cap = 1 << 18, win_cap = 1 << 20, scratch_cap = 1 << 18;
 	uint32_t npf[kNumClasses] = {0}, nex[kNumClasses] = {0}, maxE[kNumClasses] = {0}, maxwords[kNumClasses] = {0}, maxlen = 0, n_entries = 0;
 	Counters *hc_pinned = nullptr;
+	Counters *ctr(uint64_t seq) const { return counters.as<Counters>() + (seq & 1); }
+	PfAhead ahead;
+	bool ahead_pending = false;
+	uint64_t ahead_call = 0;
+	int ahead_kind = 0;
 	Counters hc;
 	uint32_t launches = 0, prefix_words = 0;
 	uint64_t n_pairs_ex = 0;
@@ -357,6 +379,11 @@
 	int opt_pf_bytes = 1;
 	int opt_pf_rb = 0;
 	int opt_seed_ahead = 1;
+	int opt_pf_ahead = 1;
+	uint64_t call_no = 0;
+	bool last_call_retried = false;
+	uint64_t test_lane_caps = 0;
+	bool dbg = false, dbg_times = false;
 	int opt_seed_ahead_blocks = 2;
 	int opt_peq_ahead_blocks = 16;
 	void (*enqueued_hook)(void *) = nullptr; void *enqueued_ctx = nullptr;
@@ -368,6 +395,11 @@
 static inline float ev_ms(hipEvent_t a, hipEvent_t b) { float ms = 0; (void)hipEventElapsedTime(&ms, a, b); return ms; }
 
 int  ensure_lanes(Handle *h, uint32_t n);
+static inline void ahead_drain(Handle *h) {
+	bool pending = false;
+	for (Lane *L : h->lanes) { pending |= L->ahead_pending; L->ahead_pending = false; L->ahead.ok = false; }
+	if (pending && h->pf_stream) { (void)hipSetDevice(h->device); (void)hipStreamSynchronize(h->pf_stream); }
+}
 uint32_t make_seed_plan(const uint8_t *s, uint32_t len, uint32_t E, uint32_t K, int stride_opt, const BhipAlt &A);
 int  slot_init(StageSlot *S);
 int  resolve_slot(Handle *h, StageSlot *S);
diff --git a/burst_amd/csrc/bhip_init.hip b/burst_amd/csrc/bhip_init.hip
--- a/burst_amd/csrc/bhip_init.hip
+++ b/burst_amd/csrc/bhip_init.hip
@@ -34,23 +34,26 @@
 	for (auto &e : L->ev_rs) if (e) (void)hipEventDestroy(e);
 	for (auto &ce : L->ev_pf) for (auto &e : ce) if (e) (void)hipEventDestroy(e);
 	for (auto &ce : L->ev_ph) for (auto &e : ce) if (e) (void)hipEventDestroy(e);
+	for (auto &pe : L->ev_pfx) for (auto &ce : pe) for (auto &e : ce) if (e) (void)hipEventDestroy(e);
 	if (L->hc_pinned) (void)hipHostFree(L->hc_pinned);
 	delete L;
 }
 
 static int lane_create(Handle *h, Lane **out) {
 	Lane *L = new Lane();
-	memset(L->ev_cls, 0, sizeof L->ev_cls); memset(L->ev_rs, 0, sizeof L->ev_rs); memset(L->ev_pf, 0, sizeof L->ev_pf); memset(L->ev_ph, 0, sizeof L->ev_ph); memset(L->ev_seed, 0, sizeof L->ev_seed); memset(L->ev_peq_alt, 0, sizeof L->ev_peq_alt); memset(L->ev_peq_cur, 0, sizeof L->ev_peq_cur);
+	memset(L->ev_pfx, 0, sizeof L->ev_pfx); memset(L->ev_cls, 0, sizeof L->ev_cls); memset(L->ev_rs, 0, sizeof L->ev_rs); memset(L->ev_pf, 0, sizeof L->ev_pf); memset(L->ev_ph, 0, sizeof L->ev_ph); memset(L->ev_seed, 0, sizeof L->ev_seed); memset(L->ev_peq_alt, 0, sizeof L->ev_peq_alt); memset(L->ev_peq_cur, 0, sizeof L->ev_peq_cur);
 	L->stream = h->stream;
 	for (auto &ce : L->ev_cls) for (auto &e : ce) if (hipEventCreate(&e) != hipSuccess) { lane_destroy(L); return fail(BHIP_E_DEVICE, "hipEventCreate failed"); }
 	for (auto &e : L->ev_rs) if (hipEventCreate(&e) != hipSuccess) { lane_destroy(L); return fail(BHIP_E_DEVICE, "hipEventCreate failed"); }
 	for (auto &ce : L->ev_pf) for (auto &e : ce) if (hipEventCreate(&e) != hipSuccess) { lane_destroy(L); return fail(BHIP_E_DEVICE, "hipEventCreate failed"); }
 	for (auto &ce : L->ev_ph) for (auto &e : ce) if (hipEventCreate(&e) != hipSuccess) { lane_destroy(L); return fail(BHIP_E_DEVICE, "hipEventCreate failed"); }
+	for (auto &pe : L->ev_pfx) for (auto &ce : pe) for (auto &e : ce) if (hipEventCreate(&e) != hipSuccess) { lane_destroy(L); return fail(BHIP_E_DEVICE, "hipEventCreate failed"); }
 	for (auto &pe : L->ev_seed) for (auto &ce : pe) for (auto &e : ce) if (hipEventCreate(&e) != hipSuccess) { lane_destroy(L); return fail(BHIP_E_DEVICE, "hipEventCreate failed"); }
 	for (auto &e : L->ev_peq_alt) if (hipEventCreate(&e) != hipSuccess) { lane_destroy(L); return fail(BHIP_E_DEVICE, "hipEventCreate failed"); }
 	for (auto &e : L->ev_peq_cur) if (hipEventCreate(&e) != hipSuccess) { lane_destroy(L); return fail(BHIP_E_DEVICE, "hipEventCreate failed"); }
-	int rc = L->counters.reserve(sizeof(Counters));
+	int rc = L->counters.reserve(2 * sizeof(Counters));
 	if (rc) { lane_destroy(L); return rc; }
+	if (h->test_lane_caps) L->task_cap = L->cand_cap = L->raw_cap = L->win_cap = L->scratch_cap = h->test_lane_caps;
 	if (hipHostMalloc((void **)&L->hc_pinned, sizeof(Counters), hipHostMallocDefault) != hipSuccess) { lane_destroy(L); return fail(BHIP_E_DEVICE, "hipHostMalloc failed"); }
 	(void)h;
 	*out = L;
@@ -61,6 +64,7 @@
 	Handle *h = (Handle *)handle;
 	if (!h) return;
 	(void)hipSetDevice(h->device);
+	ahead_drain(h);
 	if (h->stream) (void)hipStreamSynchronize(h->stream);
 	if (h->sweep_stream) (void)hipStreamSynchronize(h->sweep_stream);
 	if (h->pf_stream) (void)hipStreamSynchronize(h->pf_stream);
@@ -107,6 +111,8 @@
 	memset(h->ev, 0, sizeof h->ev);
 	memset(&h->stats, 0, sizeof h->stats);
 	h->device = device;
+	if (const char *ev = getenv("BHIP_TEST_LANE_CAPS")) h->test_lane_caps = strtoull(ev, nullptr, 0);
+	h->dbg = getenv("BHIP_DEBUG") != nullptr; h->dbg_times = getenv("BHIP_DEBUG_TIMES") != nullptr;
 	hipDeviceProp_t prop;
 	if (hipGetDeviceProperties(&prop, device) == hipSuccess) {
 		h->n_cu = prop.multiProcessorCount; h->hbm = prop.totalGlobalMem;
@@ -166,7 +172,7 @@
 		h->peq_rows = any_other ? 16u : 5u;
 		d_src.release(); d_srcoff.release(); d_flag.release();
 	}
-	if (getenv("BHIP_DEBUG")) { size_t f_ = 0, t_ = 0; if (hipMemGetInfo(&f_, &t_) == hipSuccess) fprintf(stderr, "[bhip] references on the device (%.2f GB, upload buffer released): %.2f GB of the device's %.2f free\n", h->ref_lane.cap / 1e9, f_ / 1e9, t_ / 1e9); }
+	if (h->dbg) { size_t f_ = 0, t_ = 0; if (hipMemGetInfo(&f_, &t_) == hipSuccess) fprintf(stderr, "[bhip] references on the device (%.2f GB, upload buffer released): %.2f GB of the device's %.2f free\n", h->ref_lane.cap / 1e9, f_ / 1e9, t_ / 1e9); }
 	h->acx_z = score_lut[16 * 5 + 5] != 0;
 	if (acx_lens) INITRC(bhip_load_accelerator(h, acx_lens, acx_lists, acx_fmt, K, badlist, n_bad));
 	else if (K) INITRC(bhip_build_accelerator(h, K, h->acx_z));
@@ -200,6 +206,8 @@
 extern "C" int bhip_set_option(void *handle, const char *name, long long value) {
 	Handle *h = (Handle *)handle;
 	if (!h || !name) return fail(BHIP_E_ARG, "null argument");
+	if (strcmp(name, "async_d2h")) ahead_drain(h);
+	if (!strcmp(name, "prefilter_ahead")) { h->opt_pf_ahead = value != 0; return BHIP_OK; }
 	if (!strcmp(name, "prefilter_stride")) {
 		if (value < 0 || value > 64) return fail(BHIP_E_ARG, "prefilter_stride must be 0 (auto) .. 64");
 		h->opt_prefilter_stride = (int)value; return BHIP_OK;
diff --git a/burst_amd/csrc/bhip_stage.hip b/burst_amd/csrc/bhip_stage.hip
--- a/burst_amd/csrc/bhip_stage.hip
+++ b/burst_amd/csrc/bhip_stage.hip
@@ -338,12 +338,13 @@
 	if (I.junk || h->opt_host_routing) { int rc = host_route(h, S); if (rc) return rc; }
 	else slot_take_info(S, I);
 	S->resolved = true; S->st_valid = true;
-	if (getenv("BHIP_DEBUG")) fprintf(stderr, "[bhip] stage: %u entries, %s routing, copies + routing %.2f ms on the staging stream\n", S->st_nq,
+	if (h->dbg) fprintf(stderr, "[bhip] stage: %u entries, %s routing, copies + routing %.2f ms on the staging stream\n", S->st_nq,
 		(I.junk || h->opt_host_routing) ? "host" : "device", S->st_ms_h2d);
 	return 0;
 }
 
 void lane_capacity_floor(Handle *h, Lane *L, uint64_t n) {
+	if (h->test_lane_caps) return;
 	L->task_cap = std::max<uint64_t>(L->task_cap, 3 * n + 4096); L->win_cap = std::max<uint64_t>(L->win_cap, 2 * n + 4096);
 	L->raw_cap = std::max<uint64_t>(L->raw_cap, 2 * n + 4096); L->cand_cap = std::max<uint64_t>(L->cand_cap, n / 4 + 4096);
 	h->out_cap = std::max<uint64_t>(h->out_cap, 2 * n + 4096);
@@ -387,6 +388,7 @@
 	if (!h) return fail(BHIP_E_ARG, "null handle");
 	if (n_q && (!q_codes || !q_off || !q_emac)) return fail(BHIP_E_ARG, "null query arrays");
 	HIPCHK(hipSetDevice(h->device));
+	ahead_drain(h);
 	for (StageSlot &S : h->slots) if (S.state == 1) S.state = 0;
 	StageSlot *S = free_slot(h);
 	S->state = 0;
```

Measured after the change: 599.7 million. About the same (-1.0%).
